# ghnmqdtg/VM-ASR

Measured on AMD Instinct MI355X. Metric: audio clips/sec (train step) 48kHz n_fft=1024, higher is better.
Workload: dtype bf16 (autocast over G; scan/STFT f32; MPD f32/bf16x3 MFMA); 1 GPU; vm_asr_48k_MPD.yaml full train step, DIMS 16 d_state 1 n_fft 1024 clip 122640@48k; per_gpu_batch=4, global_batch=4, parallelism=dp1, execution=hipGraph replay, 2 streams, generator_streams=2

## Files before the change

include/vmasr_hip.h:

```cpp
#ifndef VMASR_HIP_H
#define VMASR_HIP_H

#include <stddef.h>
#include <stdint.h>

#ifdef __cplusplus
extern "C" {
#endif

#define VMASR_ABI_VERSION 1

typedef void *vmasr_stream_t;

enum { VMASR_F32 = 0, VMASR_F16 = 1, VMASR_BF16 = 2 };

enum {
    VMASR_OK = 0,
    VMASR_EINVAL = -1,
    VMASR_EALIGN = -2,
    VMASR_ENOSPACE = -3
};

int vmasr_abi_version(void);
const char *vmasr_last_error(void);
// ... 95 lines not shown
    const float *h_down, *h_up;
    int64_t n_mid, mid_off;
    int32_t up, down, half_len, half_len_up;
} vmasr_degrade_item;
size_t vmasr_degrade_batch_workspace(const vmasr_degrade_item *items, int32_t B);
int vmasr_degrade_batch(const float *x, float *y, const vmasr_degrade_item *items, const vmasr_degrade_item *items_dev, int32_t B,
                        int64_t T, void *ws, size_t ws_bytes, vmasr_stream_t stream);

int vmasr_layer_norm_fwd(const void *x, const float *gamma, const float *beta, void *y, float *mean,
                         float *rstd, int32_t rows, int32_t C, float eps, int32_t dtype, int32_t y_dtype,
                         vmasr_stream_t stream);
size_t vmasr_layer_norm_bwd_workspace(int32_t rows, int32_t C);
int vmasr_layer_norm_bwd(const void *x, const void *gy, const float *gamma, const float *mean,
                         const float *rstd, void *dx, float *dgamma, float *dbeta, float *ws, int32_t rows,
                         int32_t C, int32_t dtype, int32_t gy_dtype, vmasr_stream_t stream);
int vmasr_layer_norm_bwd_res(const void *x, const void *gy, const float *gamma, const float *mean,
                             const float *rstd, const void *residual, void *dx, float *dgamma, float *dbeta, float *ws,
                             int32_t rows, int32_t C, int32_t dtype, int32_t gy_dtype, vmasr_stream_t stream);
int32_t vmasr_layer_norm_bwd_blocks(int32_t rows, int32_t C);
int vmasr_layer_norm_bwd_reduce_multi(const float *const *parts, float *const *dgammas, float *const *dbetas, const int32_t *nblks,
                                      const int32_t *Cs, int32_t n, vmasr_stream_t stream);

int vmasr_small_linear_supported(int32_t in_features, int32_t out_features);
int vmasr_small_linear_fwd(const void *x, const float *w, const float *bias, void *y, int64_t rows,
                           int32_t in_features, int32_t out_features, int32_t x_dtype, int32_t y_dtype,
                           vmasr_stream_t stream);
size_t vmasr_small_linear_bwd_workspace(int64_t rows, int32_t in_features, int32_t out_features);
int vmasr_small_linear_bwd(const void *x, const float *w, const void *gy, void *dx, float *dw, float *db,
                           float *ws, int64_t rows, int32_t in_features, int32_t out_features,
                           int32_t x_dtype, int32_t gy_dtype, vmasr_stream_t stream);

int vmasr_spectral_power_iter(const float *W, float *u, float *v, float *ws, int32_t R, int32_t C,
                              int32_t n_iter, float eps, vmasr_stream_t stream);

typedef struct vmasr_spectral_item {
    const float *W;
    float *u, *v, *t, *s;
    int32_t R, C, row_block_start, col_tile_start;
} vmasr_spectral_item;
int vmasr_spectral_power_iter_batched(const vmasr_spectral_item *items, int32_t n, int32_t total_row_blocks,
                                      int32_t total_col_tiles, int64_t weight_bytes, int32_t n_iter, float eps,
                                      float *sigma, vmasr_stream_t stream);

int vmasr_im2col_kx1(const void *x, void *cols, int64_t N, int32_t H, int32_t C, int32_t k, int32_t stride,
                     int32_t pad, int64_t rows_out, int32_t dtype, vmasr_stream_t stream);
int vmasr_im2col_kx1_split(const float *x, void *hi, void *lo, int64_t N, int32_t H, int32_t C, int32_t k, int32_t stride,
                           int32_t pad, int64_t rows_out, vmasr_stream_t stream);
int vmasr_col2im_kx1(const void *dcols, void *dx, int64_t N, int32_t H, int32_t C, int32_t k, int32_t stride,
                     int32_t pad, int32_t dtype, vmasr_stream_t stream);
int vmasr_im2col_kx1_split_multi(const float *const *xs, const int64_t *Ns, const int32_t *Hs, int32_t n, void *hi, void *lo,
                                 int32_t C, int32_t k, int32_t stride, int32_t pad, int64_t rows_out, vmasr_stream_t stream);
int vmasr_im2col_kx1_split3_multi(const float *const *xs, const int64_t *Ns, const int32_t *Hs, int32_t n, void *cat3, int32_t C,
                                  int32_t k, int32_t stride, int32_t pad, int64_t rows_out, vmasr_stream_t stream);
int vmasr_col2im_kx1_multi(const void *dcols, void *const *dxs, const int64_t *Ns, const int32_t *Hs, int32_t n, int32_t C,
                           int32_t k, int32_t stride, int32_t pad, int64_t rows, int32_t dtype, vmasr_stream_t stream);
int vmasr_col2im_kx1_stacked(const void *dcols, void *dx, const int64_t *Ns, const int32_t *Hs, int32_t n, int32_t C, int32_t k, int32_t stride,
                             int32_t pad, int64_t rows, int64_t dx_rows, int32_t dtype, vmasr_stream_t stream);
int vmasr_stack_rows(const void *const *srcs, const int64_t *Ms, int32_t n, void *full, int64_t rows, int64_t row_bytes,
                     vmasr_stream_t stream);


int vmasr_bias_gelu_fwd(float *acc, const float *bias, float *act, int32_t slots, int64_t M, int32_t N, int32_t parts,
                        vmasr_stream_t stream);
int vmasr_weight_prep_split(const float *w, void *out, int32_t n, int32_t N, int32_t K, vmasr_stream_t stream);
int vmasr_weight_transpose(const float *w, void *hi, void *lo, float *out32, int32_t n, int32_t N, int32_t Cin, int32_t k,
                           vmasr_stream_t stream);
int vmasr_sum_parts(const float *parts, float *out, int32_t P, int32_t n, int32_t S, int64_t NK, vmasr_stream_t stream);
int vmasr_gelu_bwd_split(const float *pre, const float *g, void *hi, void *lo, void *cat3, float *db, int32_t slots, int64_t M,
                         int32_t N, vmasr_stream_t stream);
int vmasr_gelu_bwd(const float *pre, const float *g, float *gx, float *db, int32_t slots, int64_t M, int32_t N, vmasr_stream_t stream);

typedef struct vmasr_cg_slot {
    const void *ah, *al;
    const void *bh, *bl;
    float *c0;
    float *c1;
    void *ch, *cl;
    const float *bias;
    int64_t nseq;
    int32_t H;
    int32_t reserved;
} vmasr_cg_slot;
int vmasr_conv_mfma_supported(int32_t Cin, int32_t Cout, int32_t k, int32_t stride);
int vmasr_conv_mfma_supported_launch(int32_t Cin, int32_t Cout, int32_t k, int32_t stride, int32_t n, int64_t rows);
int vmasr_conv_mfma_config(int32_t pass, int32_t Cin, int32_t Cout, int32_t ops, int32_t out[3]);
void vmasr_conv_set_cu_limit(int32_t cus);
int32_t vmasr_conv_get_cu_limit(void);
int vmasr_conv_mfma_fwd(const vmasr_cg_slot *slots, int32_t n, int32_t Cin, int32_t Cout, int32_t k, int32_t stride, int32_t pad,
                        int64_t rows_out, int32_t act, vmasr_stream_t stream);
int vmasr_conv_mfma_dgrad(const vmasr_cg_slot *slots, int32_t n, int32_t Cin, int32_t Cout, int32_t k, int32_t stride, int32_t pad,
                          int64_t rows_in, vmasr_stream_t stream);
int vmasr_conv_f32_fwd(const vmasr_cg_slot *slots, int32_t n, int32_t Cin, int32_t Cout, int32_t k, int32_t stride, int32_t pad,
                       int64_t rows_out, int32_t act, vmasr_stream_t stream);
int vmasr_conv_f32_dgrad(const vmasr_cg_slot *slots, int32_t n, int32_t Cin, int32_t Cout, int32_t k, int32_t stride, int32_t pad,
                         int64_t rows_in, vmasr_stream_t stream);
int vmasr_conv_mfma_wgrad(const vmasr_cg_slot *slots, int32_t n, int32_t Cin, int32_t Cout, int32_t k, int32_t stride, int32_t pad,
                          int32_t splits, vmasr_stream_t stream);
typedef struct vmasr_cg_gelu_bwd {
    const float *pre;
    const signed char *sgn;
    int64_t valid;
    float scale;
    int32_t reserved;
    float *db;
} vmasr_cg_gelu_bwd;
int vmasr_conv_mfma_dgrad_gelu(const vmasr_cg_slot *slots, const vmasr_cg_gelu_bwd *epi, const float *gtok, int32_t n, int32_t Cin, int32_t Cout,
                               int32_t k, int32_t stride, int32_t pad, int64_t rows_in, vmasr_stream_t stream);

int vmasr_wgrad_finish_multi(const float *const *parts, float *const *dws, float *const *dbs, float *const *e1s, float *const *e2s,
                             const int32_t *Ss, const int32_t *Ns, const int32_t *Ks, const int32_t *lds, int32_t n, vmasr_stream_t stream);

int vmasr_linear_f64acc(const float *x, const float *w, const float *bias, float *y, int64_t rows, int32_t out_features,
                        int32_t in_features, vmasr_stream_t stream);

typedef struct vmasr_adamw_item {
    float *p;
    const float *g;
    float *m;
    float *v;
    void *lp;
    int64_t n;
    float weight_decay;
    int32_t vec;
    void *lpt;
    int32_t rows, cols;
} vmasr_adamw_item;
int32_t vmasr_adamw_chunk(void);
int vmasr_adamw_step(const vmasr_adamw_item *items, const int32_t *chunks, int32_t nchunks, int64_t total_elems, const float *lr,
                     const float *step, float beta1, float beta2, float eps, vmasr_stream_t stream);

int32_t vmasr_sn_dot_blocks(void);
int vmasr_sn_stack_fwd(const void *const *weights, const void *const *sigmas, int32_t n, float *out, void *hi, void *lo, int32_t N, int32_t Cin,
                       int32_t k, vmasr_stream_t stream);
int vmasr_sn_stack_bwd(const float *dW, const float *Wn, void *const *gws, const void *const *sigmas, const void *const *us,
                       const void *const *vs, int32_t n, double *partials, int32_t N, int32_t Cin, int32_t k, vmasr_stream_t stream);

int vmasr_conv_post_supported(int32_t C, int32_t k);
int vmasr_conv_post_fwd(const float *x, const float *w, const float *b, float *y, const int64_t *Ms, const int32_t *Hs, int32_t n, int64_t rows,
                        int32_t C, int32_t k, vmasr_stream_t stream);
int vmasr_conv_post_bwd(const float *x, const float *w, const float *gy, float *dx, float *dw, float *db, const int64_t *Ms, const int32_t *Hs,
                        int32_t n, int64_t rows, int32_t C, int32_t k, vmasr_stream_t stream);
int vmasr_conv_post_bwd_gelu(const float *x, const float *w, const float *gy, const float *pre, const void *sgn, const float *gtok,
                             const int64_t *valid, const float *scale, void *gh, void *gl, float *g32, float *dw, float *db, float *dbcol,
                             const int64_t *Ms, const int32_t *Hs, int32_t n, int64_t rows, int32_t C, int32_t k, vmasr_stream_t stream);

int vmasr_conv_first_fwd(const void *const *xs, const int64_t *Ns, const int32_t *Hs, int32_t n, const float *w, const float *b, float *pre,
                         float *act, int64_t rows, vmasr_stream_t stream);
int vmasr_conv_first_bwd(const void *const *xs, const int64_t *Ns, const int32_t *Hs, int32_t n, const float *w, const float *pre,
                         const float *g, float *dcols, float *dw, float *db, int64_t rows, vmasr_stream_t stream);

int32_t vmasr_masked_l1_blocks(void);
int vmasr_masked_l1_fwd(const float *real, const float *gen, void *sgn, double *partials, const int64_t *valid, const float *scale,
                        int32_t n, int64_t rows_r, int64_t rows_g, int32_t N, vmasr_stream_t stream);
int vmasr_masked_l1_bwd(const void *sgn, const float *gout, float *dgen, const int64_t *valid, const float *scale, int32_t n,
                        int64_t rows_g, int32_t N, vmasr_stream_t stream);
int vmasr_masked_l1_bwd_add(const void *sgn, const float *gout, const float *add, float *dgen, const int64_t *valid, const float *scale,
                            int32_t n, int64_t rows_g, int32_t N, vmasr_stream_t stream);
int vmasr_lsgan_fwd(const void *const *xs, const int64_t *ns, const float *targets, int32_t count, float *out, vmasr_stream_t stream);
int vmasr_lsgan_bwd(const void *const *xs, void *const *ds, const int64_t *ns, const float *targets, int32_t count, const float *gout,
                    vmasr_stream_t stream);

#define VMASR_SS2D_PAIRS 1
typedef struct vmasr_ss2d_params {
    int32_t B, D, H, W, dtype, flags;
    const void *x;
    void *xT;
    const float *Wx, *Wdt, *dtb, *Alog, *Ds;
    float *state, *out02, *out13, *y;
    const float *dy;
    float *dyT, *adj, *part;
    void *dx;
    float *dWx, *dWdt, *ddtb, *dAlog, *dDs;
} vmasr_ss2d_params;
int vmasr_ss2d_supported(int32_t d_state, int32_t dt_rank, int32_t d_inner, int32_t H, int32_t W);
size_t vmasr_ss2d_part_floats(int32_t B, int32_t D, int32_t H, int32_t W);
int vmasr_ss2d_fwd(const vmasr_ss2d_params *p, vmasr_stream_t stream);
int vmasr_ss2d_bwd(const vmasr_ss2d_params *p, vmasr_stream_t stream);

typedef struct vmasr_ss2d_deep_params {
    int32_t B, D, H, W, R, dtype;
    const void *x;
    const float *WxT, *Wdt, *dtb, *Alog, *Ds;
    float *xdbl, *y;
    const float *dy;
    float *du;
    void *tp, *tb, *tc;
    float *pg, *g32;
    void *dx, *gpos;
} vmasr_ss2d_deep_params;
int vmasr_ss2d_deep_supported(int32_t d_state, int32_t dt_rank, int32_t d_inner, int32_t H, int32_t W);
int32_t vmasr_ss2d_deep_waves_per_row(int32_t H, int32_t W);
int vmasr_ss2d_deep_fwd(const vmasr_ss2d_deep_params *p, vmasr_stream_t stream);
int vmasr_ss2d_deep_bwd(const vmasr_ss2d_deep_params *p, vmasr_stream_t stream);

int vmasr_ss2d_glue_supported(int32_t D, int32_t L, int32_t dtype);
int vmasr_ss2d_pre_fwd(const void *xz, void *xT, void *sz, int32_t B, int32_t D, int32_t L, int32_t dtype, vmasr_stream_t stream);
int vmasr_ss2d_pre_bwd(const void *xz, const void *dxT, const void *dsz, void *dxz, int32_t B, int32_t D, int32_t L, int32_t dtype,
                       vmasr_stream_t stream);
int vmasr_ln_gate_fwd(const float *y, const void *sz, const float *gamma, const float *beta, void *out, float *mean, float *rstd,
                      int32_t B, int32_t D, int32_t L, float eps, int32_t dtype, vmasr_stream_t stream);
int vmasr_ln_gate_bwd(const float *y, const void *sz, const void *dout, const float *gamma, const float *beta, const float *mean,
                      const float *rstd, float *dy, void *dsz, float *dgamma, float *dbeta, int32_t B, int32_t D, int32_t L,
                      int32_t dtype, vmasr_stream_t stream);
int64_t vmasr_ln_gate_bwd_workspace(int32_t B, int32_t D, int32_t L, int32_t dtype);
int vmasr_ln_gate_bwd_ws(const float *y, const void *sz, const void *dout, const float *gamma, const float *beta, const float *mean,
                         const float *rstd, float *dy, void *dsz, float *dgamma, float *dbeta, float *ws, int32_t B, int32_t D,
                         int32_t L, int32_t dtype, vmasr_stream_t stream);
int vmasr_ln_gate_pair_supported(int32_t D, int32_t H, int32_t W);
int vmasr_ln_gate_pair_fwd(const float *y02, const float *y13, const void *sz, const float *gamma, const float *beta, void *out,
                           float *mean, float *rstd, int32_t B, int32_t D, int32_t H, int32_t W, float eps, int32_t dtype,
                           vmasr_stream_t stream);
int vmasr_ln_gate_pair_bwd(const float *y02, const float *y13, const void *sz, const void *dout, const float *gamma,
                           const float *beta, const float *mean, const float *rstd, float *dy02, float *dy13, void *dsz,
                           float *dgamma, float *dbeta, int32_t B, int32_t D, int32_t H, int32_t W, int32_t dtype,
                           vmasr_stream_t stream);

int vmasr_split_bf16(const float *x, void *hi, void *lo, int64_t n, vmasr_stream_t stream);

int vmasr_mlp_supported(int32_t d, int32_t hidden);
int vmasr_mlp_fwd(const void *x, const float *gamma, const float *beta, float eps, const void *w1, const float *b1,
                  const void *w2, const float *b2, const float *scale, int32_t rows_per_sample, void *y, int64_t rows,
                  int32_t d, int32_t x_dtype, vmasr_stream_t stream);
int vmasr_mlp_bwd(const void *x, const void *gy, const float *gamma, const float *beta, float eps, const void *w1,
                  const void *w1t, const float *b1, const void *w2t, const float *scale, int32_t rows_per_sample, void *dxn,
                  void *xn_aug, void *gys, void *act_aug, void *gpre, float *mean, float *rstd, int64_t rows, int32_t d,
                  int32_t x_dtype, vmasr_stream_t stream);

int vmasr_inproj_supported(int32_t d, int32_t d_proj, int64_t L);
int vmasr_inproj_fwd(const void *x, const float *gamma, const float *beta, float eps, const void *w, void *xT, void *sz, int64_t rows,
                     int32_t L, int32_t d, int32_t x_dtype, vmasr_stream_t stream);
int vmasr_inproj_bwd(const void *x, const float *gamma, const float *beta, float eps, const void *w, const void *wt, const void *dxT,
                     const void *dsz, void *dxn, void *xn, void *gpre, float *mean, float *rstd, int64_t rows, int32_t L, int32_t d,
                     int32_t x_dtype, vmasr_stream_t stream);

int vmasr_outproj_supported(int32_t d, int32_t d_inner);
int vmasr_outproj_fwd(const void *g, const void *w, const void *x, const float *scale, int32_t rows_per_sample, void *y, int64_t rows,
                      int32_t d, int32_t x_dtype, vmasr_stream_t stream);
int vmasr_outproj_bwd(const void *gy, const void *wt, const float *scale, int32_t rows_per_sample, void *dg, void *gys, int64_t rows,
                      int32_t d, int32_t x_dtype, vmasr_stream_t stream);

int32_t vmasr_stft_loss_blocks(void);
int vmasr_stft_loss_fwd(const float *re_x, const float *im_x, const float *re_y, const float *im_y, int64_t n, double *partials, float *out,
                        vmasr_stream_t stream);
int vmasr_stft_loss_bwd(const float *re_x, const float *im_x, const float *re_y, const float *im_y, int64_t n, const float *fin,
                        const float *g_sc, const float *g_ml, float *d_re, float *d_im, vmasr_stream_t stream);

int vmasr_gconv1d_supported(int32_t Cin, int32_t Cout, int32_t groups, int32_t k, int32_t stride);
int vmasr_gconv1d_supported_launch(int32_t Cin, int32_t Cout, int32_t groups, int32_t k, int32_t stride, int32_t pad, int32_t B, int64_t L);
size_t vmasr_gconv1d_wgrad_workspace(int32_t Cin, int32_t Cout, int32_t groups, int32_t k, int32_t stride, int32_t pad, int32_t B, int64_t L);
int vmasr_gconv1d_fwd(const float *x, const float *w, const float *bias, float *y, float *pre, int32_t B, int32_t Cin, int32_t Cout,
                      int32_t groups, int64_t L, int32_t k, int32_t stride, int32_t pad, int32_t act, vmasr_stream_t stream);
int vmasr_gconv1d_dgrad(const float *gy, const float *pre, const float *w, float *dx, int32_t B, int32_t Cin, int32_t Cout, int32_t groups,
                        int64_t L, int32_t k, int32_t stride, int32_t pad, vmasr_stream_t stream);
int vmasr_gconv1d_wgrad(const float *x, const float *gy, const float *pre, float *dw, float *db, void *ws, size_t ws_bytes, int32_t B,
                        int32_t Cin, int32_t Cout, int32_t groups, int64_t L, int32_t k, int32_t stride, int32_t pad, vmasr_stream_t stream);

int32_t vmasr_stem1d_time_tile(void);
int32_t vmasr_stem1d_channel_group(void);
int vmasr_stem1d_supported(int32_t Cout, int32_t k, int32_t stride, int32_t pad);
int vmasr_stem1d_supported_launch(int32_t Cout, int32_t k, int32_t stride, int32_t pad, int32_t B, int64_t L);
size_t vmasr_stem1d_bwd_workspace(int32_t Cout, int32_t k, int32_t stride, int32_t pad, int32_t B, int64_t L);
int vmasr_stem1d_fwd(const float *x, const float *w, const float *bias, float *y, int32_t B, int32_t Cout, int64_t L, int32_t k, int32_t stride,
                     int32_t pad, int32_t act, vmasr_stream_t stream);
int vmasr_stem1d_bwd(const float *gy, const float *x, const float *w, const float *bias, float *dx, float *dw, float *db, void *ws,
                     size_t ws_bytes, int32_t B, int32_t Cout, int64_t L, int32_t k, int32_t stride, int32_t pad, int32_t act,
                     vmasr_stream_t stream);

int vmasr_stem1d_fm_supported_launch(int32_t Cout, int32_t k, int32_t stride, int32_t pad, int32_t B, int64_t L);
size_t vmasr_stem1d_fm_workspace(int32_t Cout, int32_t k, int32_t stride, int32_t pad, int32_t B, int64_t L);
int vmasr_stem1d_fm_fwd(const float *x, const float *w, const float *bias, const float *y_real, float *y, double *partials, size_t ws_bytes,
                        int32_t B, int32_t Cout, int64_t L, int32_t k, int32_t stride, int32_t pad, vmasr_stream_t stream);
int vmasr_stem1d_fm_bwd(const float *gy, const float *x, const float *w, const float *bias, const float *y_real, const float *gterm, float coef,
                        float *dx, int32_t B, int32_t Cout, int64_t L, int32_t k, int32_t stride, int32_t pad, vmasr_stream_t stream);

enum {
    VMASR_K_SSCAN_FWD = 0,
    VMASR_K_SSCAN_FWD_AGG,
    VMASR_K_SSCAN_FWD_CARRY,
    VMASR_K_SSCAN_FWD_APPLY,
    VMASR_K_SSCAN_BWD,
    VMASR_K_SSCAN_BWD_AGG,
    VMASR_K_SSCAN_BWD_CARRY,
    VMASR_K_SSCAN_BWD_APPLY,
    VMASR_K_CROSS_SCAN,
    VMASR_K_CROSS_MERGE,
    VMASR_K_DWCONV_FWD,
    VMASR_K_DWCONV_BWD_A,
    VMASR_K_DWCONV_BWD_B,
    VMASR_K_STFT,
    VMASR_K_ISTFT_FRAMES,
    VMASR_K_ISTFT_OLA,
    VMASR_K_ISTFT_BWD,
    VMASR_K_LN_FWD,
    VMASR_K_LN_BWD,
    VMASR_K_LN_BWD_REDUCE,
    VMASR_K_SMALL_LINEAR_FWD,
    VMASR_K_SMALL_LINEAR_BWD,
    VMASR_K_SMALL_LINEAR_REDUCE,
    VMASR_K_XPROJ_FWD,
    VMASR_K_XPROJ_BWD_A,
    VMASR_K_XPROJ_BWD_B,
    VMASR_K_SPECTRAL,
    VMASR_K_IM2COL,
    VMASR_K_COL2IM,
    VMASR_K_SPLIT_BF16,
    VMASR_K_BIAS_GELU,
// ... 67 lines not shown
```

vm_asr_amd/_lib.py:

```python
import ctypes
import os

from . import knobs

_HERE = os.path.dirname(os.path.abspath(__file__))
LIB_PATH = knobs.get("VMASR_LIB") or os.path.join(_HERE, "libvmasr_hip.so")

c_i32, c_i64, c_vp, c_sz = ctypes.c_int32, ctypes.c_int64, ctypes.c_void_p, ctypes.c_size_t

F32, F16, BF16 = 0, 1, 2


class SScanParams(ctypes.Structure):
    _fields_ = (
        [(n, c_i32) for n in ("batch", "dim", "seqlen", "dstate", "n_groups", "n_chunks", "dtype",
                              "delta_softplus")]
        + [(n, c_i64) for n in ("A_d_stride", "A_dstate_stride",
                                "B_batch_stride", "B_group_stride", "B_dstate_stride",
                                "C_batch_stride", "C_group_stride", "C_dstate_stride",
                                "u_batch_stride", "u_d_stride", "delta_batch_stride", "delta_d_stride",
                                "out_batch_stride", "out_d_stride")]
        + [(n, c_vp) for n in ("A_ptr", "B_ptr", "C_ptr", "D_ptr", "u_ptr", "delta_ptr",
                               "delta_bias_ptr", "out_ptr", "x_ptr")]
    )


class SScanBwdParams(ctypes.Structure):
    _fields_ = (
        [("f", SScanParams)]
        + [(n, c_i64) for n in ("dout_batch_stride", "dout_d_stride", "du_batch_stride", "du_d_stride",
                                "ddelta_batch_stride", "ddelta_d_stride", "dA_d_stride", "dA_dstate_stride")]
        + [(n, c_vp) for n in ("dout_ptr", "du_ptr", "ddelta_ptr", "dA_ptr", "dB_ptr", "dC_ptr", "dD_ptr",
                               "ddelta_bias_ptr", "ws_ptr")]
        + [("ws_bytes", c_sz)]
    )


class SS2DParams(ctypes.Structure):
    _fields_ = ([(n, c_i32) for n in ("B", "D", "H", "W", "dtype", "flags")]
                + [(n, c_vp) for n in ("x", "xT", "Wx", "Wdt", "dtb", "Alog", "Ds", "state", "out02", "out13", "y",
                                       "dy", "dyT", "adj", "part", "dx", "dWx", "dWdt", "ddtb", "dAlog", "dDs")])


class CgSlot(ctypes.Structure):
    _fields_ = ([(n, c_vp) for n in ("ah", "al", "bh", "bl", "c0", "c1", "ch", "cl", "bias")]
                + [("nseq", c_i64), ("H", c_i32), ("reserved", c_i32)])


class CgGeluBwd(ctypes.Structure):
    _fields_ = [("pre", c_vp), ("sgn", c_vp), ("valid", c_i64), ("scale", ctypes.c_float), ("reserved", c_i32), ("db", c_vp)]


class SS2DDeepParams(ctypes.Structure):
    _fields_ = ([(n, c_i32) for n in ("B", "D", "H", "W", "R", "dtype")]
                + [(n, c_vp) for n in ("x", "WxT", "Wdt", "dtb", "Alog", "Ds", "xdbl", "y", "dy", "du", "tp", "tb", "tc", "pg",
                                       "g32", "dx", "gpos")])


SYMBOLS = {
    "vmasr_abi_version": (ctypes.c_int, []),
    "vmasr_last_error": (ctypes.c_char_p, []),
    "vmasr_sscan_chunk": (ctypes.c_int, []),
    "vmasr_sscan_fwd": (ctypes.c_int, [ctypes.POINTER(SScanParams), c_vp]),
    "vmasr_sscan_bwd_workspace": (c_sz, [ctypes.POINTER(SScanBwdParams)]),
    "vmasr_sscan_bwd": (ctypes.c_int, [ctypes.POINTER(SScanBwdParams), c_vp]),
    "vmasr_sscan_tune": (None, [ctypes.c_int, ctypes.c_int]),
    "vmasr_layer_norm_fwd": (ctypes.c_int, [c_vp, c_vp, c_vp, c_vp, c_vp, c_vp, c_i32, c_i32, ctypes.c_float, c_i32, c_i32, c_vp]),
    "vmasr_layer_norm_bwd_workspace": (c_sz, [c_i32, c_i32]),
    "vmasr_layer_norm_bwd": (ctypes.c_int, [c_vp, c_vp, c_vp, c_vp, c_vp, c_vp, c_vp, c_vp, c_vp, c_i32, c_i32, c_i32, c_i32, c_vp]),
    "vmasr_layer_norm_bwd_res": (ctypes.c_int, [c_vp, c_vp, c_vp, c_vp, c_vp, c_vp, c_vp, c_vp, c_vp, c_vp, c_i32, c_i32, c_i32, c_i32, c_vp]),
    "vmasr_layer_norm_bwd_blocks": (c_i32, [c_i32, c_i32]),
    "vmasr_layer_norm_bwd_reduce_multi": (ctypes.c_int, [c_vp, c_vp, c_vp, c_vp, c_vp, c_i32, c_vp]),
    "vmasr_mlp_supported": (ctypes.c_int, [c_i32, c_i32]),
    "vmasr_mlp_fwd": (ctypes.c_int, [c_vp, c_vp, c_vp, ctypes.c_float, c_vp, c_vp, c_vp, c_vp, c_vp, c_i32, c_vp, c_i64, c_i32, c_i32, c_vp]),
    "vmasr_mlp_bwd": (ctypes.c_int, [c_vp, c_vp, c_vp, c_vp, ctypes.c_float, c_vp, c_vp, c_vp, c_vp, c_vp, c_i32,
                                     c_vp, c_vp, c_vp, c_vp, c_vp, c_vp, c_vp, c_i64, c_i32, c_i32, c_vp]),
    "vmasr_stft_loss_blocks": (c_i32, []),
    "vmasr_stft_loss_fwd": (ctypes.c_int, [c_vp, c_vp, c_vp, c_vp, c_i64, c_vp, c_vp, c_vp]),
    "vmasr_stft_loss_bwd": (ctypes.c_int, [c_vp, c_vp, c_vp, c_vp, c_i64, c_vp, c_vp, c_vp, c_vp, c_vp, c_vp]),
    "vmasr_outproj_supported": (ctypes.c_int, [c_i32, c_i32]),
    "vmasr_outproj_fwd": (ctypes.c_int, [c_vp, c_vp, c_vp, c_vp, c_i32, c_vp, c_i64, c_i32, c_i32, c_vp]),
    "vmasr_outproj_bwd": (ctypes.c_int, [c_vp, c_vp, c_vp, c_i32, c_vp, c_vp, c_i64, c_i32, c_i32, c_vp]),
    "vmasr_inproj_supported": (ctypes.c_int, [c_i32, c_i32, c_i64]),
    "vmasr_inproj_fwd": (ctypes.c_int, [c_vp, c_vp, c_vp, ctypes.c_float, c_vp, c_vp, c_vp, c_i64, c_i32, c_i32, c_i32, c_vp]),
    "vmasr_inproj_bwd": (ctypes.c_int, [c_vp, c_vp, c_vp, ctypes.c_float, c_vp, c_vp, c_vp, c_vp, c_vp, c_vp, c_vp, c_vp, c_vp,
                                        c_i64, c_i32, c_i32, c_i32, c_vp]),
    "vmasr_small_linear_supported": (ctypes.c_int, [c_i32, c_i32]),
    "vmasr_small_linear_fwd": (ctypes.c_int, [c_vp, c_vp, c_vp, c_vp, c_i64, c_i32, c_i32, c_i32, c_i32, c_vp]),
    "vmasr_small_linear_bwd_workspace": (c_sz, [c_i64, c_i32, c_i32]),
    "vmasr_small_linear_bwd": (ctypes.c_int, [c_vp, c_vp, c_vp, c_vp, c_vp, c_vp, c_vp, c_i64, c_i32, c_i32, c_i32, c_i32, c_vp]),
    "vmasr_cross_scan_cvt": (ctypes.c_int, [c_vp, c_vp, c_i32, c_i32, c_i32, c_i32, c_i32, c_i32, c_vp]),
    "vmasr_cross_merge_cvt": (ctypes.c_int, [c_vp, c_vp, c_i32, c_i32, c_i32, c_i32, c_i32, c_i32, c_vp]),
    "vmasr_xproj_supported": (ctypes.c_int, [c_i32, c_i32, c_i32]),
    "vmasr_xproj_fwd": (ctypes.c_int, [c_vp] * 7 + [c_i32] * 7 + [c_vp]),
    "vmasr_xproj_bwd": (ctypes.c_int, [c_vp] * 12 + [c_i32] * 7 + [c_vp]),
    "vmasr_xproj_n_supported": (ctypes.c_int, [c_i32, c_i32, c_i32]),
    "vmasr_xproj_n_ws_floats": (c_sz, [c_i32, c_i32, c_i32, c_i32]),
    "vmasr_xproj_n_fwd": (ctypes.c_int, [c_vp] * 7 + [c_i32] * 7 + [c_vp]),
    "vmasr_xproj_n_bwd": (ctypes.c_int, [c_vp] * 12 + [c_i32] * 7 + [c_vp]),
    "vmasr_spectral_power_iter": (ctypes.c_int, [c_vp, c_vp, c_vp, c_vp, c_i32, c_i32, c_i32, ctypes.c_float, c_vp]),
    "vmasr_spectral_power_iter_batched": (ctypes.c_int, [c_vp, c_i32, c_i32, c_i32, c_i64, c_i32, ctypes.c_float, c_vp, c_vp]),
    "vmasr_im2col_kx1": (ctypes.c_int, [c_vp, c_vp, c_i64, c_i32, c_i32, c_i32, c_i32, c_i32, c_i64, c_i32, c_vp]),
    "vmasr_im2col_kx1_split": (ctypes.c_int, [c_vp, c_vp, c_vp, c_i64, c_i32, c_i32, c_i32, c_i32, c_i32, c_i64, c_vp]),
    "vmasr_im2col_kx1_split3_multi": (ctypes.c_int, [c_vp, c_vp, c_vp, c_i32, c_vp, c_i32, c_i32, c_i32, c_i32, c_i64, c_vp]),
    "vmasr_col2im_kx1": (ctypes.c_int, [c_vp, c_vp, c_i64, c_i32, c_i32, c_i32, c_i32, c_i32, c_i32, c_vp]),
    "vmasr_im2col_kx1_split_multi": (ctypes.c_int, [c_vp, c_vp, c_vp, c_i32, c_vp, c_vp, c_i32, c_i32, c_i32, c_i32, c_i64, c_vp]),
    "vmasr_col2im_kx1_multi": (ctypes.c_int, [c_vp, c_vp, c_vp, c_vp, c_i32, c_i32, c_i32, c_i32, c_i32, c_i64, c_i32, c_vp]),
    "vmasr_col2im_kx1_stacked": (ctypes.c_int, [c_vp, c_vp, c_vp, c_vp, c_i32, c_i32, c_i32, c_i32, c_i32, c_i64, c_i64, c_i32, c_vp]),
    "vmasr_stack_rows": (ctypes.c_int, [c_vp, c_vp, c_i32, c_vp, c_i64, c_i64, c_vp]),
    "vmasr_split_bf16": (ctypes.c_int, [c_vp, c_vp, c_vp, c_i64, c_vp]),
    "vmasr_bias_gelu_fwd": (ctypes.c_int, [c_vp, c_vp, c_vp, c_i32, c_i64, c_i32, c_i32, c_vp]),
    "vmasr_gelu_bwd": (ctypes.c_int, [c_vp, c_vp, c_vp, c_vp, c_i32, c_i64, c_i32, c_vp]),
    "vmasr_sn_dot_blocks": (c_i32, []),
    "vmasr_sn_stack_fwd": (ctypes.c_int, [c_vp, c_vp, c_i32, c_vp, c_vp, c_vp, c_i32, c_i32, c_i32, c_vp]),
    "vmasr_sn_stack_bwd": (ctypes.c_int, [c_vp, c_vp, c_vp, c_vp, c_vp, c_vp, c_i32, c_vp, c_i32, c_i32, c_i32, c_vp]),
    "vmasr_conv_post_supported": (ctypes.c_int, [c_i32, c_i32]),
    "vmasr_conv_post_fwd": (ctypes.c_int, [c_vp, c_vp, c_vp, c_vp, c_vp, c_vp, c_i32, c_i64, c_i32, c_i32, c_vp]),
    "vmasr_conv_post_bwd": (ctypes.c_int, [c_vp, c_vp, c_vp, c_vp, c_vp, c_vp, c_vp, c_vp, c_i32, c_i64, c_i32, c_i32, c_vp]),
    "vmasr_conv_post_bwd_gelu": (ctypes.c_int, [c_vp] * 16 + [c_i32, c_i64, c_i32, c_i32, c_vp]),
    "vmasr_conv_first_fwd": (ctypes.c_int, [c_vp, c_vp, c_vp, c_i32, c_vp, c_vp, c_vp, c_vp, c_i64, c_vp]),
    "vmasr_conv_first_bwd": (ctypes.c_int, [c_vp, c_vp, c_vp, c_i32, c_vp, c_vp, c_vp, c_vp, c_vp, c_vp, c_i64, c_vp]),
    "vmasr_adamw_chunk": (c_i32, []),
    "vmasr_adamw_step": (ctypes.c_int, [c_vp, c_vp, c_i32, c_i64, c_vp, c_vp, ctypes.c_float, ctypes.c_float, ctypes.c_float, c_vp]),
    "vmasr_masked_l1_blocks": (c_i32, []),
    "vmasr_masked_l1_fwd": (ctypes.c_int, [c_vp, c_vp, c_vp, c_vp, c_vp, c_vp, c_i32, c_i64, c_i64, c_i32, c_vp]),
    "vmasr_masked_l1_bwd": (ctypes.c_int, [c_vp, c_vp, c_vp, c_vp, c_vp, c_i32, c_i64, c_i32, c_vp]),
    "vmasr_lsgan_fwd": (ctypes.c_int, [c_vp, c_vp, c_vp, c_i32, c_vp, c_vp]),
    "vmasr_lsgan_bwd": (ctypes.c_int, [c_vp, c_vp, c_vp, c_vp, c_i32, c_vp, c_vp]),
    "vmasr_masked_l1_bwd_add": (ctypes.c_int, [c_vp, c_vp, c_vp, c_vp, c_vp, c_vp, c_i32, c_i64, c_i32, c_vp]),
    "vmasr_sum_parts": (ctypes.c_int, [c_vp, c_vp, c_i32, c_i32, c_i32, c_i64, c_vp]),
    "vmasr_weight_prep_split": (ctypes.c_int, [c_vp, c_vp, c_i32, c_i32, c_i32, c_vp]),
    "vmasr_weight_transpose": (ctypes.c_int, [c_vp, c_vp, c_vp, c_vp, c_i32, c_i32, c_i32, c_i32, c_vp]),
    "vmasr_gelu_bwd_split": (ctypes.c_int, [c_vp, c_vp, c_vp, c_vp, c_vp, c_vp, c_i32, c_i64, c_i32, c_vp]),
    "vmasr_conv_mfma_supported": (ctypes.c_int, [c_i32, c_i32, c_i32, c_i32]),
    "vmasr_conv_mfma_supported_launch": (ctypes.c_int, [c_i32, c_i32, c_i32, c_i32, c_i32, ctypes.c_int64]),
    "vmasr_conv_mfma_config": (ctypes.c_int, [c_i32, c_i32, c_i32, c_i32, ctypes.POINTER(c_i32)]),
    "vmasr_mark_time": (ctypes.c_int, [c_vp, c_vp]),
    "vmasr_im2col2d_rows": (ctypes.c_int, [c_vp, c_vp] + [c_i32] * 10 + [c_vp, c_i32, c_i32, c_vp]),
    "vmasr_col2im2d_rows": (ctypes.c_int, [c_vp, c_vp] + [c_i32] * 10 + [c_vp, c_i32, c_i32, c_vp]),
    "vmasr_skinny_linear_supported": (ctypes.c_int, [c_i64, c_i32, c_i32]),
    "vmasr_skinny_linear": (ctypes.c_int, [c_vp, c_vp, c_vp, c_vp, c_i64, c_i32, c_i32, c_i64, c_i64, c_i32, c_i32, c_vp]),
    "vmasr_conv_set_cu_limit": (None, [c_i32]),
    "vmasr_conv_get_cu_limit": (c_i32, []),
    "vmasr_conv_mfma_fwd": (ctypes.c_int, [ctypes.POINTER(CgSlot), c_i32, c_i32, c_i32, c_i32, c_i32, c_i32, c_i64, c_i32, c_vp]),
    "vmasr_conv_mfma_dgrad": (ctypes.c_int, [ctypes.POINTER(CgSlot), c_i32, c_i32, c_i32, c_i32, c_i32, c_i32, c_i64, c_vp]),
    "vmasr_conv_f32_fwd": (ctypes.c_int, [ctypes.POINTER(CgSlot), c_i32, c_i32, c_i32, c_i32, c_i32, c_i32, c_i64, c_i32, c_vp]),
    "vmasr_conv_f32_dgrad": (ctypes.c_int, [ctypes.POINTER(CgSlot), c_i32, c_i32, c_i32, c_i32, c_i32, c_i32, c_i64, c_vp]),
    "vmasr_conv_mfma_wgrad": (ctypes.c_int, [ctypes.POINTER(CgSlot), c_i32, c_i32, c_i32, c_i32, c_i32, c_i32, c_i32, c_vp]),
    "vmasr_conv_mfma_dgrad_gelu": (ctypes.c_int, [ctypes.POINTER(CgSlot), ctypes.POINTER(CgGeluBwd), c_vp, c_i32, c_i32, c_i32, c_i32, c_i32,
                                                  c_i32, c_i64, c_vp]),
    "vmasr_wgrad_finish_multi": (ctypes.c_int, [c_vp, c_vp, c_vp, c_vp, c_vp, c_vp, c_vp, c_vp, c_vp, c_i32, c_vp]),
    "vmasr_linear_f64acc": (ctypes.c_int, [c_vp, c_vp, c_vp, c_vp, c_i64, c_i32, c_i32, c_vp]),
    "vmasr_ss2d_glue_supported": (ctypes.c_int, [c_i32, c_i32, c_i32]),
    "vmasr_ss2d_pre_fwd": (ctypes.c_int, [c_vp, c_vp, c_vp, c_i32, c_i32, c_i32, c_i32, c_vp]),
    "vmasr_ss2d_pre_bwd": (ctypes.c_int, [c_vp, c_vp, c_vp, c_vp, c_i32, c_i32, c_i32, c_i32, c_vp]),
    "vmasr_ln_gate_fwd": (ctypes.c_int, [c_vp] * 7 + [c_i32, c_i32, c_i32, ctypes.c_float, c_i32, c_vp]),
    "vmasr_ln_gate_bwd": (ctypes.c_int, [c_vp] * 11 + [c_i32, c_i32, c_i32, c_i32, c_vp]),
    "vmasr_ln_gate_bwd_workspace": (c_i64, [c_i32, c_i32, c_i32, c_i32]),
    "vmasr_ln_gate_bwd_ws": (ctypes.c_int, [c_vp] * 12 + [c_i32, c_i32, c_i32, c_i32, c_vp]),
    "vmasr_ln_gate_pair_supported": (ctypes.c_int, [c_i32, c_i32, c_i32]),
    "vmasr_ln_gate_pair_fwd": (ctypes.c_int, [c_vp] * 8 + [c_i32, c_i32, c_i32, c_i32, ctypes.c_float, c_i32, c_vp]),
    "vmasr_ln_gate_pair_bwd": (ctypes.c_int, [c_vp] * 13 + [c_i32, c_i32, c_i32, c_i32, c_i32, c_vp]),
    "vmasr_ss2d_supported": (ctypes.c_int, [c_i32] * 5),
    "vmasr_ss2d_part_floats": (c_sz, [c_i32] * 4),
    "vmasr_ss2d_fwd": (ctypes.c_int, [ctypes.POINTER(SS2DParams), c_vp]),
    "vmasr_ss2d_bwd": (ctypes.c_int, [ctypes.POINTER(SS2DParams), c_vp]),
    "vmasr_ss2d_deep_supported": (ctypes.c_int, [c_i32] * 5),
    "vmasr_ss2d_deep_waves_per_row": (c_i32, [c_i32, c_i32]),
    "vmasr_ss2d_deep_fwd": (ctypes.c_int, [ctypes.POINTER(SS2DDeepParams), c_vp]),
    "vmasr_ss2d_deep_bwd": (ctypes.c_int, [ctypes.POINTER(SS2DDeepParams), c_vp]),
    "vmasr_set_deterministic": (None, [ctypes.c_int]),
    "vmasr_get_deterministic": (ctypes.c_int, []),
    "vmasr_det_timeouts": (ctypes.c_int64, []),
    "vmasr_prof_enable": (None, [ctypes.c_int]),
    "vmasr_prof_reset": (None, []),
    "vmasr_prof_name": (ctypes.c_char_p, [ctypes.c_int]),
    "vmasr_prof_collect": (ctypes.c_int, [ctypes.c_int, ctypes.POINTER(ctypes.c_int64),
                                          ctypes.POINTER(ctypes.c_double), ctypes.POINTER(ctypes.c_double)]),
    "vmasr_prof_collect_shapes": (ctypes.c_int, [ctypes.c_int, ctypes.c_int, ctypes.POINTER(ctypes.c_double), ctypes.POINTER(ctypes.c_int64),
                                                 ctypes.POINTER(ctypes.c_double)]),
    "vmasr_cross_scan": (ctypes.c_int, [c_vp, c_vp, c_i32, c_i32, c_i32, c_i32, c_i32, c_vp]),
    "vmasr_cross_merge": (ctypes.c_int, [c_vp, c_vp, c_i32, c_i32, c_i32, c_i32, c_i32, c_vp]),
    "vmasr_dwconv_silu_fwd": (ctypes.c_int, [c_vp, c_vp, c_vp, c_vp, c_i32, c_i32, c_i32, c_i32, c_i32, c_vp]),
    "vmasr_dwconv_silu_bwd": (ctypes.c_int, [c_vp, c_vp, c_vp, c_vp, c_vp, c_vp, c_vp, c_vp,
                                             c_i32, c_i32, c_i32, c_i32, c_i32, c_vp]),
    "vmasr_stft": (ctypes.c_int, [c_vp, c_vp, c_vp, c_i32, c_i32, c_i32, c_i32, c_i32, c_i32, c_i32, c_vp]),
    "vmasr_stft_bwd_workspace": (c_sz, [c_i32, c_i32, c_i32, c_i32]),
    "vmasr_stft_bwd": (ctypes.c_int, [c_vp, c_vp, c_vp, c_i32, c_i32, c_i32, c_i32, c_i32, c_i32, c_vp, c_sz, c_vp]),
    "vmasr_istft_workspace": (c_sz, [c_i32, c_i32, c_i32, c_i32]),
    "vmasr_istft": (ctypes.c_int, [c_vp, c_vp, c_vp, c_i32, c_i32, c_i32, c_i32, c_i32, c_vp, c_sz, c_vp]),
    "vmasr_istft_bwd": (ctypes.c_int, [c_vp, c_vp, c_vp, c_vp, c_vp, c_i32, c_i32, c_i32, c_i32, c_i32, c_vp]),
    "vmasr_metrics_workspace": (c_sz, [c_i32, c_i32, c_i32, c_i32]),
    "vmasr_metrics": (ctypes.c_int, [c_vp, c_vp, c_vp, c_vp, c_vp, c_i32, c_i32, c_i32, c_i32, c_vp, c_sz, c_vp]),
    "vmasr_gconv1d_supported": (ctypes.c_int, [c_i32] * 5),
    "vmasr_gconv1d_supported_launch": (ctypes.c_int, [c_i32] * 7 + [c_i64]),
    "vmasr_gconv1d_wgrad_workspace": (c_sz, [c_i32] * 7 + [c_i64]),
    "vmasr_gconv1d_fwd": (ctypes.c_int, [c_vp] * 5 + [c_i32] * 4 + [c_i64] + [c_i32] * 4 + [c_vp]),
    "vmasr_gconv1d_dgrad": (ctypes.c_int, [c_vp] * 4 + [c_i32] * 4 + [c_i64] + [c_i32] * 3 + [c_vp]),
    "vmasr_gconv1d_wgrad": (ctypes.c_int, [c_vp] * 6 + [c_sz] + [c_i32] * 4 + [c_i64] + [c_i32] * 3 + [c_vp]),
    "vmasr_stem1d_time_tile": (c_i32, []),
    "vmasr_stem1d_channel_group": (c_i32, []),
    "vmasr_stem1d_supported": (ctypes.c_int, [c_i32] * 4),
    "vmasr_stem1d_supported_launch": (ctypes.c_int, [c_i32] * 5 + [c_i64]),
    "vmasr_stem1d_bwd_workspace": (c_sz, [c_i32] * 5 + [c_i64]),
    "vmasr_stem1d_fwd": (ctypes.c_int, [c_vp] * 4 + [c_i32] * 2 + [c_i64] + [c_i32] * 4 + [c_vp]),
    "vmasr_stem1d_bwd": (ctypes.c_int, [c_vp] * 8 + [c_sz] + [c_i32] * 2 + [c_i64] + [c_i32] * 4 + [c_vp]),
    "vmasr_stem1d_fm_supported_launch": (ctypes.c_int, [c_i32] * 5 + [c_i64]),
    "vmasr_stem1d_fm_workspace": (c_sz, [c_i32] * 5 + [c_i64]),
    "vmasr_stem1d_fm_fwd": (ctypes.c_int, [c_vp] * 6 + [c_sz] + [c_i32] * 2 + [c_i64] + [c_i32] * 3 + [c_vp]),
    "vmasr_stem1d_fm_bwd": (ctypes.c_int, [c_vp] * 6 + [ctypes.c_float] + [c_vp] + [c_i32] * 2 + [c_i64] + [c_i32] * 3 + [c_vp]),
    "vmasr_resample_poly": (ctypes.c_int, [c_vp, c_vp, c_vp, c_i32, c_i64, c_i64, c_i32, c_i32, c_i32, c_vp]),
    "vmasr_resample_design_workspace": (c_sz, [c_i32]),
    "vmasr_resample_design": (ctypes.c_int, [c_vp, c_i32, c_i32, c_i32, c_vp, c_sz, c_vp]),
    "vmasr_degrade_batch_workspace": (c_sz, [c_vp, c_i32]),
    "vmasr_degrade_batch": (ctypes.c_int, [c_vp, c_vp, c_vp, c_vp, c_i32, c_i64, c_vp, c_sz, c_vp]),
}

_lib = None


def lib():
    global _lib
    if _lib is None:
        if not os.path.exists(LIB_PATH):
            raise RuntimeError(
                f"{LIB_PATH} is missing: build it with `make -C vm_asr_amd/csrc` "
                "(or __graft_entry__.build()). vm_asr_amd has no CPU fallback.")
        import torch
        l = ctypes.CDLL(LIB_PATH)
        for name, (res, args) in SYMBOLS.items():
            fn = getattr(l, name)
            fn.restype, fn.argtypes = res, args
        if l.vmasr_abi_version() != 1:
            raise RuntimeError("libvmasr_hip.so ABI version mismatch")
        if knobs.get("VMASR_DETERMINISTIC"):
            l.vmasr_set_deterministic(1)
        knobs.warn_undeclared()
        _lib = l
    return _lib


def check(code, what):
    if code != 0:
        msg = lib().vmasr_last_error().decode() or "unknown error"
        raise RuntimeError(f"{what} failed ({code}): {msg}")


def torch_dtype_code(dt):
    import torch
    try:
        return {torch.float32: F32, torch.float16: F16, torch.bfloat16: BF16}[dt]
    except KeyError:
        raise RuntimeError(f"unsupported dtype {dt}: expected float32 / float16 / bfloat16")


def det_mode():
    if knobs.get("VMASR_DETERMINISTIC"):
        return True
    try:
        return bool(lib().vmasr_get_deterministic())
    except (OSError, RuntimeError, AttributeError):
        return False


def current_stream(device):
    import torch
    return ctypes.c_void_p(torch.cuda.current_stream(device).cuda_stream)


def ptr(t):
    return None if t is None else ctypes.c_void_p(t.data_ptr())


def call(fn, *args, device=None):
    import torch
    what = fn.__name__[len("vmasr_"):]
    conv = list(args)
    for i, a in enumerate(conv):
# ... 85 lines not shown
```

vm_asr_amd/convgemm.py:

```python
import ctypes

import torch

from . import _lib
from .mpd_ops import need as _need, sum_parts


def supported(Cin, Cout, k, stride):
    return bool(_lib.lib().vmasr_conv_mfma_supported(int(Cin), int(Cout), int(k), int(stride)))


def config(what, Cin, Cout, f32=False):
    out = (ctypes.c_int32 * 3)()
    _lib.check(_lib.lib().vmasr_conv_mfma_config(("fwd", "dgrad", "wgrad").index(what), int(Cin), int(Cout), int(bool(f32)), out), "conv_mfma_config")
    return tuple(out)


_LIMIT = {"cus": 0, "min_channels": 0}


class cu_limit:

    def __init__(self, cus, min_channels=0):
        self.new = {"cus": int(cus or 0), "min_channels": int(min_channels or 0)}

    def __enter__(self):
        self.prev = dict(_LIMIT)
        _LIMIT.update(self.new)
        return self

    def __exit__(self, *exc):
        _LIMIT.update(self.prev)
        _lib.lib().vmasr_conv_set_cu_limit(0)
        return False


def _apply_limit(Cin, Cout):
    lim = _LIMIT["cus"] if max(Cin, Cout) >= _LIMIT["min_channels"] else 0
    _lib.lib().vmasr_conv_set_cu_limit(lim)


def _slots(geom, **operands):
    sl = (_lib.CgSlot * len(geom))()
    steps = [(f, t.data_ptr(), t.stride(0) * t.element_size()) for f, t in operands.items() if t is not None]
    for i, (nseq, H) in enumerate(geom):
        for f, base, step in steps:
            setattr(sl[i], f, base + i * step)
        sl[i].nseq, sl[i].H = int(nseq), int(H)
    return sl


def _ptr(t, i, step):
    return ctypes.c_void_p(t.data_ptr() + i * step) if t is not None else None


def out_positions(H, k, stride, pad):
    return (H + 2 * pad - k) // stride + 1


def _fwd(fn, xh, xl, wh, wl, bias, geom, k, stride, pad, rows_out, act, want_pair):
    _need(xh, xl, wh, wl, bias)
    (n, _, Cin), Cout, dev = xh.shape, wh.shape[1], xh.device
    pre = torch.empty((n, rows_out, Cout), dtype=torch.float32, device=dev)
    y = torch.empty_like(pre) if act else None
    yh = torch.empty((n, rows_out, Cout), dtype=torch.bfloat16, device=dev) if act and want_pair else None
    yl = torch.empty_like(yh) if yh is not None else None
    sl = _slots(geom, ah=xh, al=xl, bh=wh, bl=wl, c0=pre, c1=y, ch=yh, cl=yl, bias=bias)
    _apply_limit(Cin, Cout)
    _lib.call(fn, sl, n, Cin, Cout, k, stride, pad, rows_out, int(bool(act)), device=dev)
    return pre, y, yh, yl


def _dgrad(fn, gh, gl, wth, wtl, geom, k, stride, pad, rows_in):
    _need(gh, gl, wth, wtl)
    (n, _, Cout), Cin, dev = gh.shape, wth.shape[1], gh.device
    dx = torch.empty((n, rows_in, Cin), dtype=torch.float32, device=dev)
    sl = _slots(geom, ah=gh, al=gl, bh=wth, bl=wtl, c0=dx)
    _apply_limit(Cin, Cout)
    _lib.call(fn, sl, n, Cin, Cout, k, stride, pad, rows_in, device=dev)
    return dx


def conv_fwd(xh, xl, wh, wl, bias, geom, k, stride, pad, rows_out, act=True, want_pair=True):
    return _fwd(_lib.lib().vmasr_conv_mfma_fwd, xh, xl, wh, wl, bias, geom, k, stride, pad, rows_out, act, want_pair)


def conv_dgrad(gh, gl, wth, wtl, geom, k, stride, pad, rows_in):
    return _dgrad(_lib.lib().vmasr_conv_mfma_dgrad, gh, gl, wth, wtl, geom, k, stride, pad, rows_in)


def conv_fwd_f32(x, w, bias, geom, k, stride, pad, rows_out, act=True, want_pair=True):
    assert x.dtype == torch.float32 and w.dtype == torch.float32
    return _fwd(_lib.lib().vmasr_conv_f32_fwd, x, None, w, None, bias, geom, k, stride, pad, rows_out, act, want_pair)


def conv_dgrad_f32(g, wt, geom, k, stride, pad, rows_in):
    assert g.dtype == torch.float32 and wt.dtype == torch.float32
    return _dgrad(_lib.lib().vmasr_conv_f32_dgrad, g, None, wt, None, geom, k, stride, pad, rows_in)


def conv_dgrad_gelu(gh, gl, wth, wtl, geom, k, stride, pad, rows_in, pre, want_f32=False, want_pair=True, sgn=None, gtok=None,
                    scale=None, valid=None, db=None):
    _need(gh, gl, wth, wtl, pre, sgn, gtok, db)
    assert db is None or (db.shape == (gh.shape[0], wth.shape[1]) and db.dtype == torch.float32)
    (n, _, Cout), Cin, dev = gh.shape, wth.shape[1], gh.device
    assert pre.shape == (n, rows_in, Cin) and pre.dtype == torch.float32 and (want_f32 or want_pair)
    assert sgn is None or (sgn.shape == pre.shape and sgn.dtype == torch.int8 and gtok is not None and gtok.dtype == torch.float32)
    g32 = torch.empty((n, rows_in, Cin), dtype=torch.float32, device=dev) if want_f32 else None
    oh = torch.empty((n, rows_in, Cin), dtype=torch.bfloat16, device=dev) if want_pair else None
    ol = torch.empty_like(oh) if want_pair else None
    sl = _slots(geom, ah=gh, al=gl, bh=wth, bl=wtl, c0=g32, ch=oh, cl=ol)
    ep = (_lib.CgGeluBwd * n)()
    for i in range(n):
        ep[i].pre = _ptr(pre, i, rows_in * Cin * 4)
        ep[i].sgn = _ptr(sgn, i, rows_in * Cin)
        ep[i].valid = int(valid[i]) if (sgn is not None and valid is not None) else 0
        ep[i].scale = float(scale[i]) if (sgn is not None and scale is not None) else 0.0
        ep[i].db = _ptr(db, i, Cin * 4)
    _apply_limit(Cin, Cout)
    _lib.call(_lib.lib().vmasr_conv_mfma_dgrad_gelu, sl, ep, gtok if sgn is not None else None, n, Cin, Cout, k, stride, pad, rows_in,
              device=dev)
    return g32, ((oh, ol) if want_pair else None)


def wgrad_splits(n, Cin, Cout, k, M):
    if Cin % 256 == 0 and Cout % 256 == 0:
        return 1
    T = 128
    tiles = n * (Cout // T) * (k * Cin // T)
    s = 1
    while tiles * s < 768 and s < 16 and M // (2 * s) >= 1024:
        s *= 2
    return s


def conv_wgrad(gh, gl, xh, xl, geom, k, stride, pad, splits=None):
    _need(gh, gl, xh, xl)
    (n, _, Cout), Cin, dev = gh.shape, xh.shape[2], gh.device
    if splits is None:
        M = max(nseq * out_positions(H, k, stride, pad) for nseq, H in geom)
        splits = wgrad_splits(n, Cin, Cout, k, M)
    parts = torch.empty((n, splits, Cout, k * Cin), dtype=torch.float32, device=dev)
    sl = _slots(geom, ah=gh, al=gl, bh=xh, bl=xl, c0=parts)
    _apply_limit(Cin, Cout)
    _lib.call(_lib.lib().vmasr_conv_mfma_wgrad, sl, n, Cin, Cout, k, stride, pad, splits, device=dev)
    if splits == 1:
        return parts.view(n, Cout, k * Cin)
    return sum_parts(parts, 1, n, splits, (Cout, k * Cin))
```

vm_asr_amd/csrc/convgemm.hip:

```cpp
#include <algorithm>
#include <cstdlib>
#include <type_traits>

#include "common.h"

namespace vmasr {
namespace {

typedef __bf16 bf16x8 __attribute__((ext_vector_type(8)));
typedef float f32x16 __attribute__((ext_vector_type(16)));
typedef float f32x4 __attribute__((ext_vector_type(4)));
typedef unsigned u32x4 __attribute__((ext_vector_type(4)));
typedef __attribute__((address_space(1))) const void *cg_gptr;
typedef __attribute__((address_space(3))) void *cg_lptr;
__device__ uint4 cg_zero_page[4];

constexpr int CG_BM = 128, CG_BN = 128, CG_BK = 32;
constexpr int CG_TILE = CG_BM * CG_BK * 2;
constexpr int CG_STAGE = 4 * CG_TILE;
constexpr int CG_MAXP = 24;

struct CgProb {
    const bf16_t *ah, *al, *bh, *bl;
    float *c0, *c1;
    bf16_t *ch, *cl;
    const float *bias;
    int M, Q;
    int HA;
    int HC;
    int hq_mul, hq_add;
    int crow_mul, crow_add;
    int ntaps, tap0, tap_step, dstep;
    int tile_start, mtiles;
    int zero_rows;
    float fscale;
    int fvalid;
    float *db;
};

struct CgParams {
    CgProb prob[CG_MAXP];
    int nprob, ntiles_n, total_tiles;
    int CA;
    int NB;
    int KB;
    const float *gtok;
};
static_assert(sizeof(CgParams) <= 4096, "CgParams is passed by value as the kernel's argument block");

__device__ __forceinline__ int cg_swz(const int row) { return (0 - (row >> 2)) & 3; }
__device__ __forceinline__ int cg_off(const int row, const int chunk) { return row * 64 + ((chunk ^ cg_swz(row)) << 4); }

__device__ __forceinline__ float cg_gelu(float x) { return 0.5f * x * (1.f + erff(x * 0.70710678118654752f)); }
__device__ __forceinline__ float cg_gelu_grad(float x) {
    return 0.5f * (1.f + erff(x * 0.70710678118654752f)) + x * 0.3989422804014327f * __expf(-0.5f * x * x);
}

__device__ __forceinline__ f32x16 cg_mfma(const bf16x8 a, const bf16x8 b, const f32x16 c) {
    return __builtin_amdgcn_mfma_f32_32x32x16_bf16(a, b, c, 0, 0, 0);
}

template <int BM, int BN, int WM, int WN, int EPI, int MF, int OPS = 0>
__global__ __launch_bounds__(64 * WM * WN, 2) void conv_mfma_nt_kernel(const CgParams P) {
    static_assert(OPS == 0 || MF == 32, "the f32 form uses the 32-row fragment layout");
    constexpr bool ACT = EPI == 1;
    constexpr int NT = 64 * WM * WN;
    constexpr int WTM = BM / WM, WTN = BN / WN;
    constexpr int TI = WTM / MF, TJ = WTN / MF;
    constexpr int TILE_A = BM * 64, TILE_B = BN * 64;
    constexpr int STAGE = 2 * TILE_A + 2 * TILE_B;
    constexpr int RPP = NT / 4;
    constexpr int PA = BM / RPP, PB = (BN + RPP - 1) / RPP;
    constexpr bool B_PART = BN < RPP;
    static_assert(BM % RPP == 0 && (BN % RPP == 0 || (B_PART && BN % 16 == 0)) && BM % 128 == 0, "tile / thread geometry");
    extern __shared__ __attribute__((aligned(16))) unsigned char smem[];
    int *crow_tab = reinterpret_cast<int *>(smem + 2 * STAGE);

    const int tid = threadIdx.x, lane = tid & 63, wave = tid >> 6;
    const int wm = wave / WN, wn = wave % WN, lr = lane & 31, lh = lane >> 5;

#pragma unroll 1
    for (int tile = blockIdx.x; tile < P.total_tiles; tile += gridDim.x) {
    const int t = xcd_remap(tile, P.total_tiles);
    int pi = 0;
#pragma unroll 1
    for (int i = 1; i < P.nprob; ++i) pi = (t >= P.prob[i].tile_start) ? i : pi;
    const CgProb &pr = P.prob[pi];
    const int local = t - pr.tile_start;
    const int nt = local % P.ntiles_n, mt = local / P.ntiles_n;
    const int m0 = mt * BM, n0 = nt * BN;
    const int M = pr.M, Q = pr.Q, HA = pr.HA, CA = P.CA, NB = P.NB;
    constexpr int UPK = OPS ? 64 : 32;
    const int LDA = OPS ? 2 * CA : CA;
    const int KB = OPS ? 2 * P.KB : P.KB;

    if (tid < BM) {
        const int m = m0 + tid;
        int cr = -1;
        if (m < M) {
            const int seq = m / Q, q = m - seq * Q;
            cr = seq * pr.HC + q * pr.crow_mul + pr.crow_add;
        } else if (m < pr.zero_rows) {
            cr = m;
        }
        crow_tab[tid] = cr;
    }

    const int srow = tid >> 2, chunk = (tid & 3) ^ cg_swz(srow);
    int a_base[PA], a_hq[PA];
    bool a_ok[PA];
#pragma unroll
    for (int i = 0; i < PA; ++i) {
        const int m = m0 + srow + RPP * i;
        a_ok[i] = m < M;
        const int mm = a_ok[i] ? m : 0;
        const int seq = mm / Q, q = mm - seq * Q;
        a_base[i] = seq * HA;
        a_hq[i] = q * pr.hq_mul + pr.hq_add;
    }
    const bf16_t *bsrc_h[PB], *bsrc_l[PB];
#pragma unroll
    for (int i = 0; i < PB; ++i) {
        const size_t o = (size_t)(n0 + ((B_PART && srow >= BN) ? 0 : srow + RPP * i)) * KB + chunk * 8;
        bsrc_h[i] = pr.bh + o;
        bsrc_l[i] = pr.bl + o;
    }
    const int cpk = CA / CG_BK;
    const int nk = (m0 < M) ? pr.ntaps * cpk : 0;
    const int wbase = wave * 16 * 64;
    const bf16_t *zp = reinterpret_cast<const bf16_t *>(cg_zero_page);

#define CG_DMA(src, dst) __builtin_amdgcn_global_load_lds((cg_gptr)(src), (cg_lptr)(dst), 16, 0, 0)
    auto stage_tile = [&](const int kt, const int buf) {
        const int j = kt / cpk, c0 = (kt - j * cpk) * UPK;
        const int koff = (pr.tap0 + j * pr.tap_step) * LDA + c0;
        unsigned char *d = smem + buf * STAGE + wbase;
#pragma unroll
        for (int i = 0; i < PA; ++i) {
            const int pos = a_hq[i] + j * pr.dstep;
            const bool ok = a_ok[i] && pos >= 0 && pos < HA;
            const size_t o = (size_t)(a_base[i] + pos) * LDA + c0 + chunk * 8;
            CG_DMA(ok ? pr.ah + o : zp, d + i * RPP * 64);
            CG_DMA(ok ? (OPS ? pr.ah + o + 32 : pr.al + o) : zp, d + TILE_A + i * RPP * 64);
        }
#pragma unroll
        for (int i = 0; i < PB; ++i) {
            if (B_PART && srow >= BN) break;
            CG_DMA(bsrc_h[i] + koff, d + 2 * TILE_A + i * RPP * 64);
            CG_DMA((OPS ? bsrc_h[i] + 32 : bsrc_l[i]) + koff, d + 2 * TILE_A + TILE_B + i * RPP * 64);
        }
    };

    using acc_t = typename std::conditional<MF == 32, f32x16, f32x4>::type;
    constexpr int NR = MF == 32 ? 16 : 4;
    acc_t acc[TI][TJ];
#pragma unroll
    for (int i = 0; i < TI; ++i)
#pragma unroll
        for (int j = 0; j < TJ; ++j)
#pragma unroll
            for (int r = 0; r < NR; ++r) acc[i][j][r] = 0.f;

    if (nk > 0) stage_tile(0, 0);
    asm volatile("s_waitcnt vmcnt(0)" ::: "memory");
    __syncthreads();

    for (int kt = 0; kt < nk; ++kt) {
        const int buf = kt & 1;
        if (kt + 1 < nk) stage_tile(kt + 1, buf ^ 1);
        const unsigned char *s = smem + buf * STAGE;
        if constexpr (OPS == 1) {
#pragma unroll
            for (int ks = 0; ks < 2; ++ks) {
                f32x4 a0[TI], a1[TI], b0[TJ], b1[TJ];
#pragma unroll
                for (int i = 0; i < TI; ++i) {
                    const int oa = cg_off(wm * WTM + i * 32 + lr, ks * 2 + lh);
                    a0[i] = *reinterpret_cast<const f32x4 *>(s + oa);
                    a1[i] = *reinterpret_cast<const f32x4 *>(s + TILE_A + oa);
                }
#pragma unroll
                for (int j = 0; j < TJ; ++j) {
                    const int ob = cg_off(wn * WTN + j * 32 + lr, ks * 2 + lh);
                    b0[j] = *reinterpret_cast<const f32x4 *>(s + 2 * TILE_A + ob);
                    b1[j] = *reinterpret_cast<const f32x4 *>(s + 2 * TILE_A + TILE_B + ob);
                }
#pragma unroll
                for (int i = 0; i < TI; ++i)
#pragma unroll
                    for (int j = 0; j < TJ; ++j) {
#pragma unroll
                        for (int e = 0; e < 4; ++e) acc[i][j] = __builtin_amdgcn_mfma_f32_32x32x2f32(a0[i][e], b0[j][e], acc[i][j], 0, 0, 0);
#pragma unroll
                        for (int e = 0; e < 4; ++e) acc[i][j] = __builtin_amdgcn_mfma_f32_32x32x2f32(a1[i][e], b1[j][e], acc[i][j], 0, 0, 0);
                    }
            }
        } else if constexpr (MF == 32) {
#pragma unroll
            for (int ks = 0; ks < 2; ++ks) {
                bf16x8 ah[TI], al[TI], bh[TJ], bl[TJ];
#pragma unroll
                for (int i = 0; i < TI; ++i) {
                    const int oa = cg_off(wm * WTM + i * 32 + lr, ks * 2 + lh);
                    ah[i] = *reinterpret_cast<const bf16x8 *>(s + oa);
                    al[i] = *reinterpret_cast<const bf16x8 *>(s + TILE_A + oa);
                }
// ... 358 lines not shown
int cg_grid(int tiles, size_t smem) {
    if (g_cg_cu_limit <= 0) return tiles;
    const int per_cu = std::max(1, (int)((160 * 1024) / std::max<size_t>(smem, 1)));
    static const int slack = [] { const char *e = getenv("VMASR_CONV_CU_SLACK"); return e ? atoi(e) : 24; }();
    const int cap = std::min(256, g_cg_cu_limit + slack) * per_cu;
    const int rounds = (tiles + cap - 1) / cap;
    const int g = ((tiles + rounds - 1) / rounds + 7) / 8 * 8;
    return std::min(tiles, std::min(g, cap));
}

template <int BM, int BN, int WM, int WN, int MF, int OPS = 0>
int cg_launch_cfg(CgParams &P, int epi, hipStream_t st, int kid, double bytes) {
    int tiles = 0;
    P.ntiles_n = P.NB / BN;
    for (int i = 0; i < P.nprob; ++i) {
        P.prob[i].tile_start = tiles;
        P.prob[i].mtiles = (std::max(P.prob[i].M, P.prob[i].zero_rows) + BM - 1) / BM;
        tiles += P.prob[i].mtiles * P.ntiles_n;
    }
    P.total_tiles = tiles;
    if (tiles == 0) return 0;
    constexpr size_t smem = 2 * (2 * BM * 64 + 2 * BN * 64) + BM * sizeof(int);
    constexpr bool HAS_EPI2 = BN >= 128 && OPS == 0;
    static bool attr_done = false;
    if (!attr_done && smem > 65536) {
        (void)hipFuncSetAttribute(reinterpret_cast<const void *>(&conv_mfma_nt_kernel<BM, BN, WM, WN, 1, MF, OPS>), hipFuncAttributeMaxDynamicSharedMemorySize, (int)smem);
        (void)hipFuncSetAttribute(reinterpret_cast<const void *>(&conv_mfma_nt_kernel<BM, BN, WM, WN, 0, MF, OPS>), hipFuncAttributeMaxDynamicSharedMemorySize, (int)smem);
        if constexpr (HAS_EPI2)
            (void)hipFuncSetAttribute(reinterpret_cast<const void *>(&conv_mfma_nt_kernel<BM, BN, WM, WN, 2, MF, OPS>), hipFuncAttributeMaxDynamicSharedMemorySize, (int)smem);
        attr_done = true;
    }
    if (epi == 1) {
        VMASR_LAUNCH(kid, bytes, (conv_mfma_nt_kernel<BM, BN, WM, WN, 1, MF, OPS>), dim3(cg_grid(tiles, smem)), dim3(64 * WM * WN), smem, st, P);
    } else if (epi == 2) {
        if constexpr (HAS_EPI2) {
            VMASR_LAUNCH(kid, bytes, (conv_mfma_nt_kernel<BM, BN, WM, WN, 2, MF, OPS>), dim3(cg_grid(tiles, smem)), dim3(64 * WM * WN), smem, st, P);
        } else {
            set_error("conv_mfma: no fused activation backward for this tile");
            return VMASR_EINVAL;
        }
    } else {
        VMASR_LAUNCH(kid, bytes, (conv_mfma_nt_kernel<BM, BN, WM, WN, 0, MF, OPS>), dim3(cg_grid(tiles, smem)), dim3(64 * WM * WN), smem, st, P);
    }
    return check_launch("conv_mfma");
}

int env_conv_tile() {
    static const int v = [] { const char *e = getenv("VMASR_CONV_TILE"); return e ? atoi(e) : 0; }();
    return v;
}
int env_conv_mfma() {
    static const int v = [] { const char *e = getenv("VMASR_CONV_MFMA"); return e ? atoi(e) : 16; }();
    return v;
}

struct CgConfig {
    int BM, BN, MF;
};
enum { CG_PASS_FWD = 0, CG_PASS_DGRAD = 1, CG_PASS_WGRAD = 2 };

CgConfig cg_config_nt(int NB, int CA, int ops, bool fwd) {
    if (ops) {
        static const int tile = [] { const char *e = getenv("VMASR_CONV_F32_TILE"); return e ? atoi(e) : 128; }();
        if (!fwd) return {256, 32, 32};
        return tile == 256 ? CgConfig{256, 128, 32} : CgConfig{128, 128, 32};
    }
    const int forced = env_conv_tile();
    const int mf = env_conv_mfma() == 16 ? 16 : 32;
    if (NB % 256 == 0 && forced != 128) return {256, 256, mf};
    if (NB % 128 == 0 && CA == 32 && forced != 128) return {256, 128, 16};
    if (NB == 32) return {256, 32, 16};
    return {128, 128, mf};
}

CgConfig cg_config_wgrad(int Cin, int Cout) {
    if (Cout % 256 == 0 && Cin % 256 == 0 && env_conv_tile() != 128) return {256, 256, 16};
    if (Cin == 32) return {128, 32, 16};
    return {128, 128, env_conv_mfma() == 32 ? 32 : 16};
}

CgConfig cg_config(int pass, int Cin, int Cout, int ops) {
    if (pass == CG_PASS_WGRAD) return cg_config_wgrad(Cin, Cout);
    return pass == CG_PASS_FWD ? cg_config_nt(Cout, Cin, ops, true) : cg_config_nt(Cin, Cout, ops, false);
}

int cg_launch(CgParams &P, int epi, hipStream_t st, int kid, double bytes, int ops = 0, bool fwd = true) {
    const CgConfig c = cg_config_nt(P.NB, P.CA, ops, fwd);
    const int key = c.BM * 1000000 + c.BN * 1000 + c.MF;
    if (ops) {
        switch (key) {
            case 256128032: return cg_launch_cfg<256, 128, 4, 2, 32, 1>(P, epi, st, kid, bytes);
            case 256032032: return cg_launch_cfg<256, 32, 8, 1, 32, 1>(P, epi, st, kid, bytes);
            default: return cg_launch_cfg<128, 128, 2, 2, 32, 1>(P, epi, st, kid, bytes);
        }
    }
    switch (key) {
        case 256256016: return cg_launch_cfg<256, 256, 2, 4, 16>(P, epi, st, kid, bytes);
        case 256256032: return cg_launch_cfg<256, 256, 2, 4, 32>(P, epi, st, kid, bytes);
        case 256128016: return cg_launch_cfg<256, 128, 4, 2, 16>(P, epi, st, kid, bytes);
        case 256032016: return cg_launch_cfg<256, 32, 8, 1, 16>(P, epi, st, kid, bytes);
        case 128128032: return cg_launch_cfg<128, 128, 2, 2, 32>(P, epi, st, kid, bytes);
        default: return cg_launch_cfg<128, 128, 2, 2, 16>(P, epi, st, kid, bytes);
    }
}

int64_t cg_fwd_row_bound(int Cin, int Cout, int k, int ops) { return ((int64_t)1 << (ops ? 30 : 31)) / std::max(Cout, k * Cin); }
int64_t cg_dgrad_row_bound(int Cin, int Cout, int k) { return ((int64_t)1 << 31) / std::max(Cin, k * Cout); }
int64_t cg_wgrad_grow_bound(int Cin, int Cout) { return ((int64_t)1 << 31) / std::max(Cout, Cin); }
int64_t cg_wgrad_xrow_bound(int Cin) { return ((int64_t)1 << 31) / Cin; }

}

VMASR_EXPORT void vmasr_conv_set_cu_limit(int32_t cus) { g_cg_cu_limit = cus < 0 ? 0 : cus; }
VMASR_EXPORT int32_t vmasr_conv_get_cu_limit(void) { return g_cg_cu_limit; }

VMASR_EXPORT int vmasr_conv_mfma_supported(int32_t Cin, int32_t Cout, int32_t k, int32_t stride) {
    const bool in_ok = Cin > 0 && (Cin % 128 == 0 || Cin == 32), out_ok = Cout > 0 && Cout % 128 == 0;
    return in_ok && out_ok && k >= 1 && k <= 8 && stride >= 1 && stride <= 3;
}

VMASR_EXPORT int vmasr_conv_mfma_supported_launch(int32_t Cin, int32_t Cout, int32_t k, int32_t stride, int32_t n, int64_t rows) {
    if (!vmasr_conv_mfma_supported(Cin, Cout, k, stride)) return 0;
    if (n < 1 || n > 8 || n * (stride + 1) > CG_MAXP) return 0;
    int64_t bound = std::min(cg_fwd_row_bound(Cin, Cout, k, 0), cg_dgrad_row_bound(Cin, Cout, k));
    bound = std::min(bound, std::min(cg_wgrad_grow_bound(Cin, Cout), cg_wgrad_xrow_bound(Cin)));
    if (Cin == 32) bound = std::min(bound, cg_fwd_row_bound(Cin, Cout, k, 1));
    return rows >= 1 && rows < bound ? 1 : 0;
}

VMASR_EXPORT int vmasr_conv_mfma_config(int32_t pass, int32_t Cin, int32_t Cout, int32_t ops, int32_t out[3]) {
    VMASR_REQUIRE(out && pass >= CG_PASS_FWD && pass <= CG_PASS_WGRAD && (ops == 0 || (ops == 1 && Cin == 32 && pass != CG_PASS_WGRAD)), VMASR_EINVAL,
                  "conv_mfma_config: pass 0..2, ops 0 or 1 (Cin 32, forward / input gradient), out");
    VMASR_REQUIRE(vmasr_conv_mfma_supported(Cin, Cout, 1, 1), VMASR_EINVAL, "conv_mfma_config: unsupported channel counts (Cin %d, Cout %d)", Cin, Cout);
    const CgConfig c = cg_config(pass, Cin, Cout, ops);
    out[0] = c.BM; out[1] = c.BN; out[2] = c.MF;
    return VMASR_OK;
}

namespace {
int cg_fwd(const vmasr_cg_slot *slots, int32_t n, int32_t Cin, int32_t Cout, int32_t k, int32_t stride, int32_t pad, int64_t rows_out,
           int32_t act, vmasr_stream_t stream, int ops) {
    const char *what = ops ? "conv_f32_fwd" : "conv_mfma_fwd";
    VMASR_REQUIRE(slots && n >= 1 && n <= CG_MAXP, VMASR_EINVAL, "%s: 1..%d slots", what, CG_MAXP);
    VMASR_REQUIRE(vmasr_conv_mfma_supported(Cin, Cout, k, stride) && (!ops || Cin == 32), VMASR_EINVAL,
                  "%s: unsupported shape (Cin %d, Cout %d, k %d, stride %d)", what, Cin, Cout, k, stride);
    VMASR_REQUIRE(rows_out % 256 == 0, VMASR_EINVAL, "%s: rows_out must be a multiple of 256", what);
    CgParams P = {};
    P.nprob = n;
    P.CA = Cin; P.NB = Cout; P.KB = k * Cin;
    double bytes = 0;
    for (int i = 0; i < n; ++i) {
        const vmasr_cg_slot &s = slots[i];
        VMASR_REQUIRE(s.ah && s.bh && s.c0 && (ops || (s.al && s.bl)), VMASR_EINVAL, "%s: null tensor in slot %d", what, i);
        VMASR_REQUIRE(!ops || (aligned_to(s.ah, 16) && aligned_to(s.bh, 16)), VMASR_EALIGN, "%s: slot %d: operands must be 16-byte aligned", what, i);
        const int64_t H1 = ((int64_t)s.H + 2 * pad - k) / stride + 1;
        const int64_t M = s.nseq * H1;
        VMASR_REQUIRE(H1 >= 1 && M <= rows_out && rows_out < cg_fwd_row_bound(Cin, Cout, k, ops), VMASR_EINVAL,
                      "%s: slot %d: %lld rows do not fit rows_out %lld (or 32-bit offsets)", what, i, (long long)M, (long long)rows_out);
        CgProb &p = P.prob[i];
        p.ah = (const bf16_t *)s.ah; p.al = (const bf16_t *)s.al; p.bh = (const bf16_t *)s.bh; p.bl = (const bf16_t *)s.bl;
        p.c0 = s.c0; p.c1 = s.c1; p.ch = (bf16_t *)s.ch; p.cl = (bf16_t *)s.cl; p.bias = s.bias;
        p.M = (int)M; p.Q = (int)H1; p.HA = s.H; p.HC = (int)H1;
        p.hq_mul = stride; p.hq_add = -pad; p.crow_mul = 1; p.crow_add = 0;
        p.ntaps = k; p.tap0 = 0; p.tap_step = 1; p.dstep = 1;
        p.zero_rows = (int)rows_out;
        bytes += (double)s.nseq * s.H * Cin * 4 + (double)Cout * k * Cin * 4 + (double)M * Cout * (act ? 12 : 4);
    }
    hipStream_t st = static_cast<hipStream_t>(stream);
    if (ops) VMASR_REQUIRE(Cout % 128 == 0, VMASR_EINVAL, "%s: Cout %% 128", what);
    return cg_launch(P, act != 0 ? 1 : 0, st, VMASR_K_CONV_MFMA_FWD, bytes, ops, true);
}
}

VMASR_EXPORT int vmasr_conv_mfma_fwd(const vmasr_cg_slot *slots, int32_t n, int32_t Cin, int32_t Cout, int32_t k, int32_t stride,
                                     int32_t pad, int64_t rows_out, int32_t act, vmasr_stream_t stream) {
    return cg_fwd(slots, n, Cin, Cout, k, stride, pad, rows_out, act, stream, 0);
}

VMASR_EXPORT int vmasr_conv_f32_fwd(const vmasr_cg_slot *slots, int32_t n, int32_t Cin, int32_t Cout, int32_t k, int32_t stride,
                                    int32_t pad, int64_t rows_out, int32_t act, vmasr_stream_t stream) {
    return cg_fwd(slots, n, Cin, Cout, k, stride, pad, rows_out, act, stream, 1);
}

namespace {

int cg_dgrad(const vmasr_cg_slot *slots, const vmasr_cg_gelu_bwd *epi, const float *gtok, int32_t n, int32_t Cin, int32_t Cout, int32_t k,
             int32_t stride, int32_t pad, int64_t rows_in, vmasr_stream_t stream, int ops = 0) {
    const char *what = ops ? "conv_f32_dgrad" : epi ? "conv_mfma_dgrad_gelu" : "conv_mfma_dgrad";
    VMASR_REQUIRE(!ops || (!epi && Cin == 32), VMASR_EINVAL, "%s: the f32 form serves Cin = 32 without a fused activation backward", what);
    VMASR_REQUIRE(slots && n >= 1 && n * (stride + 1) <= CG_MAXP, VMASR_EINVAL, "%s: too many slots", what);
    VMASR_REQUIRE(vmasr_conv_mfma_supported(Cin, Cout, k, stride), VMASR_EINVAL, "%s: unsupported shape (Cin %d, Cout %d, k %d, stride %d)", what,
                  Cin, Cout, k, stride);
    VMASR_REQUIRE(!epi || Cin % 128 == 0, VMASR_EINVAL, "%s: the fused activation backward needs Cin %% 128 == 0", what);
    CgParams P = {};
    P.CA = Cout; P.NB = Cin; P.KB = k * Cout;
    P.gtok = gtok;
    double bytes = 0;
    int np = 0;
    for (int i = 0; i < n; ++i) {
        const vmasr_cg_slot &s = slots[i];
        VMASR_REQUIRE(s.ah && s.bh && (ops || (s.al && s.bl)) && (epi ? (s.c0 || (s.ch && s.cl)) && (!s.ch == !s.cl) : s.c0 != nullptr), VMASR_EINVAL,
                      "%s: null tensor in slot %d", what, i);
        VMASR_REQUIRE(!ops || (aligned_to(s.ah, 16) && aligned_to(s.bh, 16)), VMASR_EALIGN, "%s: slot %d: operands must be 16-byte aligned", what, i);
        VMASR_REQUIRE(!epi || (epi[i].pre && epi[i].valid >= 0 && (!epi[i].sgn || gtok)), VMASR_EINVAL,
                      "%s: slot %d: pre-activation missing (or a sign map without the loss gradient)", what, i);
        const int64_t H = s.H, H1 = (H + 2 * pad - k) / stride + 1;
        VMASR_REQUIRE(H1 >= 1 && s.nseq * H <= rows_in && rows_in < cg_dgrad_row_bound(Cin, Cout, k), VMASR_EINVAL,
                      "%s: slot %d: %lld rows do not fit rows_in %lld (or 32-bit offsets)", what, i, (long long)(s.nseq * H), (long long)rows_in);
        auto outputs = [&](CgProb &p) {
            p.c0 = s.c0; p.c1 = nullptr; p.ch = nullptr; p.cl = nullptr; p.bias = nullptr;
            if (epi) {
                p.ch = (bf16_t *)s.ch; p.cl = (bf16_t *)s.cl;
                p.bias = epi[i].pre;
                p.c1 = reinterpret_cast<float *>(const_cast<signed char *>(epi[i].sgn));
                p.fscale = epi[i].scale;
                p.fvalid = (int)std::min<int64_t>(epi[i].valid, rows_in);
                p.db = epi[i].db;
            }
        };
        for (int r = 0; r < stride; ++r) {
            const int r0 = ((r - pad) % stride + stride) % stride;
            const int64_t Q = H > r0 ? (H - r0 + stride - 1) / stride : 0;
            if (Q == 0) continue;
            CgProb &p = P.prob[np++];
            p.ah = (const bf16_t *)s.ah; p.al = (const bf16_t *)s.al; p.bh = (const bf16_t *)s.bh; p.bl = (const bf16_t *)s.bl;
            outputs(p);
            p.M = (int)(s.nseq * Q); p.Q = (int)Q; p.HA = (int)H1; p.HC = (int)H;
            p.hq_mul = 1; p.hq_add = (r0 + pad - r) / stride;
            p.crow_mul = stride; p.crow_add = r0;
            p.ntaps = r < k ? (k - r + stride - 1) / stride : 0;
            p.tap0 = r; p.tap_step = stride; p.dstep = -1;
            p.zero_rows = 0;
        }
        if (s.nseq * H < rows_in) {
            CgProb &p = P.prob[np++];
            p.ah = (const bf16_t *)s.ah; p.al = (const bf16_t *)s.al; p.bh = (const bf16_t *)s.bh; p.bl = (const bf16_t *)s.bl;
            outputs(p);
            p.M = (int)(rows_in - s.nseq * H); p.Q = p.M; p.HA = 1; p.HC = 0;
            p.hq_mul = 0; p.hq_add = 0; p.crow_mul = 1; p.crow_add = (int)(s.nseq * H);
            p.ntaps = 0; p.tap0 = 0; p.tap_step = 1; p.dstep = 0;
            p.zero_rows = 0;
            p.db = nullptr;
        }
        bytes += (double)s.nseq * H1 * Cout * 4 + (double)Cout * k * Cin * 4 + (double)s.nseq * H * Cin * 4;
        if (epi) bytes += (double)s.nseq * H * Cin * ((s.c0 && s.ch ? 4.0 : 0.0) + 4.0 + (epi[i].sgn ? 1.0 : 0.0));
    }
    P.nprob = np;
    return cg_launch(P, epi ? 2 : 0, static_cast<hipStream_t>(stream), VMASR_K_CONV_MFMA_DGRAD, bytes, ops, false);
}

}

VMASR_EXPORT int vmasr_conv_mfma_dgrad(const vmasr_cg_slot *slots, int32_t n, int32_t Cin, int32_t Cout, int32_t k, int32_t stride,
                                       int32_t pad, int64_t rows_in, vmasr_stream_t stream) {
    return cg_dgrad(slots, nullptr, nullptr, n, Cin, Cout, k, stride, pad, rows_in, stream);
}

VMASR_EXPORT int vmasr_conv_f32_dgrad(const vmasr_cg_slot *slots, int32_t n, int32_t Cin, int32_t Cout, int32_t k, int32_t stride,
                                      int32_t pad, int64_t rows_in, vmasr_stream_t stream) {
    return cg_dgrad(slots, nullptr, nullptr, n, Cin, Cout, k, stride, pad, rows_in, stream, 1);
}

VMASR_EXPORT int vmasr_conv_mfma_dgrad_gelu(const vmasr_cg_slot *slots, const vmasr_cg_gelu_bwd *epi, const float *gtok, int32_t n, int32_t Cin,
                                            int32_t Cout, int32_t k, int32_t stride, int32_t pad, int64_t rows_in, vmasr_stream_t stream) {
    VMASR_REQUIRE(epi, VMASR_EINVAL, "conv_mfma_dgrad_gelu: epi is required");
    return cg_dgrad(slots, epi, gtok, n, Cin, Cout, k, stride, pad, rows_in, stream);
}

VMASR_EXPORT int vmasr_conv_mfma_wgrad(const vmasr_cg_slot *slots, int32_t n, int32_t Cin, int32_t Cout, int32_t k, int32_t stride,
                                       int32_t pad, int32_t splits, vmasr_stream_t stream) {
    VMASR_REQUIRE(slots && n >= 1 && n <= 8, VMASR_EINVAL, "conv_mfma_wgrad: 1..8 slots");
    VMASR_REQUIRE(vmasr_conv_mfma_supported(Cin, Cout, k, stride) && splits >= 1 && splits <= 64, VMASR_EINVAL,
                  "conv_mfma_wgrad: unsupported shape (Cin %d, Cout %d, k %d, stride %d, splits %d)", Cin, Cout, k, stride, splits);
    CwParams P = {};
    const CgConfig cfg = cg_config_wgrad(Cin, Cout);
    const bool big = cfg.BM == 256, narrow = cfg.BN == 32;
    const int T = cfg.BM, TK = cfg.BN;
    P.nslots = n; P.splits = splits; P.tiles_co = Cout / T; P.tiles_kc = k * Cin / TK;
    P.Cin = Cin; P.Cout = Cout; P.k = k; P.stride = stride; P.pad = pad;
    double bytes = 0;
    for (int i = 0; i < n; ++i) {
        const vmasr_cg_slot &s = slots[i];
        VMASR_REQUIRE(s.ah && s.al && s.bh && s.bl && s.c0, VMASR_EINVAL, "conv_mfma_wgrad: null tensor in slot %d", i);
        const int64_t H1 = ((int64_t)s.H + 2 * pad - k) / stride + 1, M = s.nseq * H1;
        VMASR_REQUIRE(H1 >= 1 && M < cg_wgrad_grow_bound(Cin, Cout) && s.nseq * (int64_t)s.H < cg_wgrad_xrow_bound(Cin), VMASR_EINVAL,
                      "conv_mfma_wgrad: slot %d too large for 32-bit row offsets", i);
        CwProb &p = P.prob[i];
        p.gh = (const bf16_t *)s.ah; p.gl = (const bf16_t *)s.al; p.xh = (const bf16_t *)s.bh; p.xl = (const bf16_t *)s.bl;
        p.dw = s.c0; p.M = (int)M; p.Q = (int)H1; p.H = s.H;
        const int64_t per = (M + splits - 1) / splits;
        p.mchunk = (int)((per + CW_BR - 1) / CW_BR * CW_BR);
        bytes += (double)M * Cout * 4 + (double)s.nseq * s.H * Cin * 4 + (double)splits * Cout * k * Cin * 4;
    }
    const int tiles = n * splits * P.tiles_co * P.tiles_kc;
    hipStream_t st = static_cast<hipStream_t>(stream);
    if (big) {
        constexpr size_t smem = 2 * 4 * CW_BR * 512;
        static bool attr_done = false;
        if (!attr_done) {
            (void)hipFuncSetAttribute(reinterpret_cast<const void *>(&conv_mfma_wgrad_kernel<256, 256, 2, 4, 16>), hipFuncAttributeMaxDynamicSharedMemorySize, (int)smem);
            attr_done = true;
        }
        VMASR_LAUNCH(VMASR_K_CONV_MFMA_WGRAD, bytes, (conv_mfma_wgrad_kernel<256, 256, 2, 4, 16>), dim3(cg_grid(tiles, smem)), dim3(512), smem, st, P);
    } else if (narrow) {
        VMASR_LAUNCH(VMASR_K_CONV_MFMA_WGRAD, bytes, (conv_mfma_wgrad_kernel<128, 32, 4, 1, 16>), dim3(cg_grid(tiles, 2 * (2 * CW_BR * 256 + 2 * CW_BR * 64))), dim3(256), 2 * (2 * CW_BR * 256 + 2 * CW_BR * 64), st, P);
    } else if (cfg.MF == 32) {
        VMASR_LAUNCH(VMASR_K_CONV_MFMA_WGRAD, bytes, (conv_mfma_wgrad_kernel<128, 128, 2, 2, 32>), dim3(cg_grid(tiles, 2 * 4 * CW_BR * 256)), dim3(256), 2 * 4 * CW_BR * 256, st, P);
    } else {
        VMASR_LAUNCH(VMASR_K_CONV_MFMA_WGRAD, bytes, (conv_mfma_wgrad_kernel<128, 128, 2, 2, 16>), dim3(cg_grid(tiles, 2 * 4 * CW_BR * 256)), dim3(256), 2 * 4 * CW_BR * 256, st, P);
    }
    return check_launch("conv_mfma_wgrad");
}
```

vm_asr_amd/csrc/featloss.hip:

```cpp
#include <algorithm>

#include "common.h"

namespace vmasr {
namespace {

constexpr int kMaxSlots = 8;

struct L1Slots {
    long valid_elems[kMaxSlots];
    float scale[kMaxSlots];
};

__device__ __forceinline__ signed char sgn1(float d) { return (signed char)((d > 0.f) - (d < 0.f)); }

__global__ __launch_bounds__(256) void masked_l1_fwd_kernel(const float *__restrict__ real, const float *__restrict__ gen,
                                                            signed char *__restrict__ sgn, double *__restrict__ partials,
                                                            const L1Slots t, const size_t stride_r, const size_t stride_g) {
    const int s = blockIdx.y;
    const float *__restrict__ r = real + (size_t)s * stride_r;
    const float *__restrict__ g = gen + (size_t)s * stride_g;
    signed char *__restrict__ o = sgn ? sgn + (size_t)s * stride_g : nullptr;
    const long n = t.valid_elems[s], n4 = n / 4;
    double acc = 0.0;
    for (long i = (long)blockIdx.x * blockDim.x + threadIdx.x; i < n4; i += (long)gridDim.x * blockDim.x) {
        const float4 a = reinterpret_cast<const float4 *>(g)[i], b = reinterpret_cast<const float4 *>(r)[i];
        const float d0 = a.x - b.x, d1 = a.y - b.y, d2 = a.z - b.z, d3 = a.w - b.w;
        acc += (double)((fabsf(d0) + fabsf(d1)) + (fabsf(d2) + fabsf(d3)));
        if (o) {
            char4 q;
            q.x = sgn1(d0); q.y = sgn1(d1); q.z = sgn1(d2); q.w = sgn1(d3);
            reinterpret_cast<char4 *>(o)[i] = q;
        }
    }
    if (blockIdx.x == 0 && (int)threadIdx.x < (int)(n - n4 * 4)) {
        const long i = n4 * 4 + threadIdx.x;
        const float d = g[i] - r[i];
        acc += (double)fabsf(d);
        if (o) o[i] = sgn1(d);
    }
    for (int off = 32; off > 0; off >>= 1) acc += __shfl_down(acc, off, 64);
    __shared__ double wsum[4];
    if ((threadIdx.x & 63) == 0) wsum[threadIdx.x >> 6] = acc;
    __syncthreads();
    if (threadIdx.x == 0) partials[(size_t)s * gridDim.x + blockIdx.x] = (wsum[0] + wsum[1] + wsum[2] + wsum[3]) * (double)t.scale[s];
}

__global__ __launch_bounds__(256) void masked_l1_bwd_kernel(const signed char *__restrict__ sgn, const float *__restrict__ gout,
                                                            const float *__restrict__ add, float *__restrict__ dgen, const L1Slots t,
                                                            const size_t stride_g) {
    const int s = blockIdx.y;
    const signed char *__restrict__ q = sgn + (size_t)s * stride_g;
    const float *__restrict__ a = add ? add + (size_t)s * stride_g : nullptr;
    float *__restrict__ o = dgen + (size_t)s * stride_g;
    const float k = gout[0] * t.scale[s];
    const long n = t.valid_elems[s], total4 = (long)(stride_g / 4);
    for (long i = (long)blockIdx.x * blockDim.x + threadIdx.x; i < total4; i += (long)gridDim.x * blockDim.x) {
        float4 v = a ? reinterpret_cast<const float4 *>(a)[i] : make_float4(0.f, 0.f, 0.f, 0.f);
        const long e = i * 4;
        if (e + 3 < n) {
            const char4 c = reinterpret_cast<const char4 *>(q)[i];
            v.x = fmaf(k, (float)c.x, v.x); v.y = fmaf(k, (float)c.y, v.y); v.z = fmaf(k, (float)c.z, v.z); v.w = fmaf(k, (float)c.w, v.w);
        } else if (e < n) {
            float w[4] = {v.x, v.y, v.z, v.w};
            for (int j = 0; j < 4 && e + j < n; ++j) w[j] = fmaf(k, (float)q[e + j], w[j]);
            v = make_float4(w[0], w[1], w[2], w[3]);
        }
        reinterpret_cast<float4 *>(o)[i] = v;
    }
}

int fill_slots(L1Slots &t, const int64_t *valid, const float *scale, int n, int N, int64_t rows_g, int64_t rows_r, const char *what) {
    for (int s = 0; s < n; ++s) {
        if (valid[s] < 0 || valid[s] > rows_g || valid[s] > rows_r) {
            set_error("%s: slot %d has %ld valid rows of %ld / %ld", what, s, (long)valid[s], (long)rows_g, (long)rows_r);
            return VMASR_EINVAL;
        }
        t.valid_elems[s] = (long)valid[s] * N;
        t.scale[s] = scale[s];
    }
    return 0;
}

}
}

using namespace vmasr;

VMASR_EXPORT int32_t vmasr_masked_l1_blocks(void) { return 256 * 4; }

VMASR_EXPORT int vmasr_masked_l1_fwd(const float *real, const float *gen, void *sgn, double *partials, const int64_t *valid,
                                     const float *scale, int32_t n, int64_t rows_r, int64_t rows_g, int32_t N, vmasr_stream_t stream) {
    VMASR_REQUIRE(real && gen && partials && valid && scale, VMASR_EINVAL, "masked_l1_fwd: null argument");
    VMASR_REQUIRE(n > 0 && n <= kMaxSlots && rows_r > 0 && rows_g > 0 && N > 0, VMASR_EINVAL, "masked_l1_fwd: bad shape");
    VMASR_REQUIRE(((size_t)rows_r * N) % 4 == 0 && ((size_t)rows_g * N) % 4 == 0 && aligned_to(real, 16) && aligned_to(gen, 16) &&
                      (!sgn || aligned_to(sgn, 4)),
                  VMASR_EINVAL, "masked_l1_fwd: slots must be 16-byte aligned (rows * N %% 4 == 0)");
    L1Slots t{};
    if (int e = fill_slots(t, valid, scale, n, N, rows_g, rows_r, "masked_l1_fwd")) return e;
    double bytes = 0;
    for (int s = 0; s < n; ++s) bytes += (double)t.valid_elems[s] * (sgn ? 9.0 : 8.0);
    hipStream_t st = static_cast<hipStream_t>(stream);
    VMASR_LAUNCH(VMASR_K_FEAT_L1, bytes, masked_l1_fwd_kernel, dim3(vmasr_masked_l1_blocks(), n), dim3(256), 0, st, real, gen,
                 static_cast<signed char *>(sgn), partials, t, (size_t)rows_r * N, (size_t)rows_g * N);
    return check_launch("masked_l1_fwd");
}

VMASR_EXPORT int vmasr_masked_l1_bwd_add(const void *sgn, const float *gout, const float *add, float *dgen, const int64_t *valid,
                                         const float *scale, int32_t n, int64_t rows_g, int32_t N, vmasr_stream_t stream) {
    VMASR_REQUIRE(sgn && gout && dgen && valid && scale, VMASR_EINVAL, "masked_l1_bwd: null argument");
    VMASR_REQUIRE(n > 0 && n <= kMaxSlots && rows_g > 0 && N > 0, VMASR_EINVAL, "masked_l1_bwd: bad shape");
    VMASR_REQUIRE(((size_t)rows_g * N) % 4 == 0 && aligned_to(dgen, 16) && aligned_to(sgn, 4) && (!add || aligned_to(add, 16)), VMASR_EINVAL,
                  "masked_l1_bwd: slots must be 16-byte aligned (rows * N %% 4 == 0)");
    L1Slots t{};
    if (int e = fill_slots(t, valid, scale, n, N, rows_g, rows_g, "masked_l1_bwd")) return e;
    const long total4 = (long)rows_g * N / 4;
    const int blocks = (int)std::min<long>((total4 + 255) / 256, 256L * 8);
    hipStream_t st = static_cast<hipStream_t>(stream);
    VMASR_LAUNCH(VMASR_K_FEAT_L1, (add ? 9.0 : 5.0) * n * (double)rows_g * N, masked_l1_bwd_kernel, dim3(blocks, n), dim3(256), 0, st,
                 static_cast<const signed char *>(sgn), gout, add, dgen, t, (size_t)rows_g * N);
    return check_launch("masked_l1_bwd");
}

VMASR_EXPORT int vmasr_masked_l1_bwd(const void *sgn, const float *gout, float *dgen, const int64_t *valid, const float *scale, int32_t n,
                                     int64_t rows_g, int32_t N, vmasr_stream_t stream) {
    return vmasr_masked_l1_bwd_add(sgn, gout, nullptr, dgen, valid, scale, n, rows_g, N, stream);
}

namespace vmasr {
namespace {

constexpr int kGanMax = 16;
struct GanItems {
    const float *x[kGanMax];
    float *d[kGanMax];
    long n[kGanMax];
    float c[kGanMax];
    int count;
};

__global__ __launch_bounds__(1024) void lsgan_fwd_kernel(const GanItems t, float *__restrict__ out) {
    __shared__ double ws[16];
    double total = 0.0;
    for (int it = 0; it < t.count; ++it) {
        const float *__restrict__ x = t.x[it];
        const float c = t.c[it];
        double acc = 0.0;
        for (long i = threadIdx.x; i < t.n[it]; i += blockDim.x) {
            const float d = x[i] - c;
            acc += (double)(d * d);
        }
        for (int off = 32; off > 0; off >>= 1) acc += __shfl_down(acc, off, 64);
        if ((threadIdx.x & 63) == 0) ws[threadIdx.x >> 6] = acc;
        __syncthreads();
        if (threadIdx.x == 0) {
            double s = 0.0;
            for (int w = 0; w < 16; ++w) s += ws[w];
            total += s / (double)t.n[it];
        }
        __syncthreads();
    }
    if (threadIdx.x == 0) out[0] = (float)total;
}

__global__ __launch_bounds__(256) void lsgan_bwd_kernel(const GanItems t, const float *__restrict__ gout) {
    const int it = blockIdx.y;
    const float *__restrict__ x = t.x[it];
    float *__restrict__ d = t.d[it];
    const float c = t.c[it], k = 2.f * gout[0] / (float)t.n[it];
    for (long i = (long)blockIdx.x * blockDim.x + threadIdx.x; i < t.n[it]; i += (long)gridDim.x * blockDim.x) d[i] = k * (x[i] - c);
}

int gan_fill(GanItems &t, const void *const *xs, void *const *ds, const int64_t *ns, const float *cs, int count, const char *what) {
    VMASR_REQUIRE(xs && ns && cs && count > 0 && count <= kGanMax, VMASR_EINVAL, "%s: 1..%d tensors", what, kGanMax);
    t.count = count;
    for (int i = 0; i < count; ++i) {
        VMASR_REQUIRE(xs[i] && ns[i] > 0 && (!ds || ds[i]), VMASR_EINVAL, "%s: tensor %d null / empty", what, i);
        t.x[i] = static_cast<const float *>(xs[i]);
        t.d[i] = ds ? static_cast<float *>(ds[i]) : nullptr;
        t.n[i] = ns[i];
        t.c[i] = cs[i];
    }
    return 0;
}

}
}

VMASR_EXPORT int vmasr_lsgan_fwd(const void *const *xs, const int64_t *ns, const float *targets, int32_t count, float *out,
                                 vmasr_stream_t stream) {
    VMASR_REQUIRE(out, VMASR_EINVAL, "lsgan_fwd: null output");
    GanItems t{};
    if (int e = gan_fill(t, xs, nullptr, ns, targets, count, "lsgan_fwd")) return e;
    double bytes = 0;
    for (int i = 0; i < count; ++i) bytes += 4.0 * ns[i];
    VMASR_LAUNCH(VMASR_K_FEAT_L1, bytes, lsgan_fwd_kernel, dim3(1), dim3(1024), 0, static_cast<hipStream_t>(stream), t, out);
    return check_launch("lsgan_fwd");
}

VMASR_EXPORT int vmasr_lsgan_bwd(const void *const *xs, void *const *ds, const int64_t *ns, const float *targets, int32_t count,
                                 const float *gout, vmasr_stream_t stream) {
    VMASR_REQUIRE(gout && ds, VMASR_EINVAL, "lsgan_bwd: null argument");
    GanItems t{};
    if (int e = gan_fill(t, xs, ds, ns, targets, count, "lsgan_bwd")) return e;
    long nmax = 0;
    double bytes = 0;
    for (int i = 0; i < count; ++i) { nmax = std::max<long>(nmax, ns[i]); bytes += 8.0 * ns[i]; }
    const int blocks = (int)std::min<long>((nmax + 255) / 256, 64);
    VMASR_LAUNCH(VMASR_K_FEAT_L1, bytes, lsgan_bwd_kernel, dim3(blocks, count), dim3(256), 0, static_cast<hipStream_t>(stream), t, gout);
    return check_launch("lsgan_bwd");
}
```

vm_asr_amd/discriminator.py:

```python

import torch
import torch.nn as nn
import torch.nn.functional as F
from torch.nn.utils import parametrize
from torch.nn.utils.parametrizations import weight_norm

from . import _lib, knobs, mpd_ops as bind
from .linear import linear as _linear, weight_grad as _weight_grad
from .mpd_featloss import StackedFeatures, _FeatTapFn, _MaskedL1Fn, _masked_l1_ok, feature_loss_stacked
from .mpd_layers import (_BatchedLinearFn, _BatchedLinearSplitFn, _StackedConvFirstFn, _StackedConvMfmaFn, _StackedConvPostFn,
                         _StackedConvSplitFn, _StackedIm2ColFn, _UnstackRowsFn, _bmm3, _dw3, _l1_mode, _poison, _round_up, _split_k,
                         _split_mode, scores_only, skip_weight_grads)
from .mpd_link import _Link, _Tap
from .mpd_ops import SpectralBatch, _slot_arrays, geom_of as _geom, split_bf16

__all__ = ["PeriodDiscriminator", "MultiPeriodDiscriminator", "spectral_norm", "plain_torch_ops"]

_PLAIN_OPS = [False]


class plain_torch_ops:

    def __enter__(self):
        self._saved = _PLAIN_OPS[0]
        _PLAIN_OPS[0] = True
        return self

    def __exit__(self, *exc):
        _PLAIN_OPS[0] = self._saved
        return False


class _SpectralNorm(nn.Module):

    def __init__(self, weight, n_power_iterations=1, eps=1e-12):
        super().__init__()
        self.n_power_iterations, self.eps = n_power_iterations, eps
        w = weight.detach().flatten(1)
        u = F.normalize(w.new_empty(w.size(0)).normal_(0, 1), dim=0, eps=eps)
        v = F.normalize(w.new_empty(w.size(1)).normal_(0, 1), dim=0, eps=eps)
        self.register_buffer("_u", u)
        self.register_buffer("_v", v)
        self._power_method(w, 15)

    @torch.autograd.no_grad()
    def _power_method(self, w, n):
        if w.is_cuda and n > 0 and w.dtype == torch.float32:
            bind.spectral_power_iter(w.contiguous(), self._u, self._v, n, self.eps)
            return
        for _ in range(n):
            self._u = F.normalize((w @ self._v.unsqueeze(1)).squeeze(1), dim=0, eps=self.eps, out=self._u)
            self._v = F.normalize((w.t() @ self._u.unsqueeze(1)).squeeze(1), dim=0, eps=self.eps, out=self._v)

    def forward(self, weight):
        with torch.autocast(device_type=weight.device.type, enabled=False):
            pre = getattr(self, "_sigma_pre", None)
            if pre is not None and self.training and self.n_power_iterations == 0 and weight.dtype == torch.float32:
                return _SNDivFn.apply(weight, self._u, self._v, pre)
            w = (weight if weight.dtype == torch.float64 else weight.float()).flatten(1)
            if self.training:
                self._power_method(w, self.n_power_iterations)
            u, v = self._u.clone(), self._v.clone()
            sigma = (u * (w @ v.unsqueeze(1)).squeeze(1)).sum()
            return weight / sigma


class _SNDivFn(torch.autograd.Function):

    @staticmethod
    def forward(ctx, weight, u, v, sigma):
        out = weight / sigma
        ctx.save_for_backward(out, u, v, sigma)
        return out

    @staticmethod
    def backward(ctx, g):
        out, u, v, sigma = ctx.saved_tensors
        g2, o2 = g.reshape(u.numel(), -1), out.reshape(u.numel(), -1)
        s = torch.dot(g2.reshape(-1), o2.reshape(-1))
        gw = torch.addcmul(g2, (u * (-s)).unsqueeze(1), v.unsqueeze(0)) / sigma
        return gw.view_as(out), None, None, None


class _SNStackFn(torch.autograd.Function):

    @staticmethod
    def forward(ctx, n, *args):
        sig, us, vs, ws = args[:n], args[n:2 * n], args[2 * n:3 * n], args[3 * n:4 * n]
        pair_out = args[4 * n] if len(args) > 4 * n else None
        out = bind.sn_stack_fwd([w.detach().contiguous() for w in ws], sig, want_pair=pair_out is not None)
        if pair_out is not None:
            out, pair_out["w"] = out
        ctx.save_for_backward(out, *sig, *us, *vs)
        ctx.geom = (n, [w.shape for w in ws], len(args) - 4 * n)
        return out

    @staticmethod
    def backward(ctx, dW):
        n, shapes, extra = ctx.geom
        out, *rest = ctx.saved_tensors
        gws = bind.sn_stack_bwd(dW.float().contiguous(), out, rest[:n], rest[n:2 * n], rest[2 * n:3 * n], shapes)
        return (None, *([None] * (3 * n)), *gws, *([None] * extra))


def _sn_stack(layers, pair_out=None):
    sns, origs = [], []
    for l in layers:
        if not (isinstance(l, nn.Conv2d) and parametrize.is_parametrized(l, "weight")):
            return None
        sn, w = l.parametrizations.weight[0], l.parametrizations.weight.original
        if not (isinstance(sn, _SpectralNorm) and getattr(sn, "_sigma_pre", None) is not None and sn.training and sn.n_power_iterations == 0
                and w.is_cuda and w.dtype == torch.float32 and w.dim() == 4 and w.shape[3] == 1):
            return None
        sns.append(sn); origs.append(w)
    n = len(layers)
    if n > 8 or any(w.shape != origs[0].shape for w in origs) or origs[0].shape[1] * origs[0].shape[2] * 4 > 60 * 1024:
        return None
    if n > 1 and (origs[0].numel() % 4):
        return None
    return _SNStackFn.apply(n, *[sn._sigma_pre for sn in sns], *[sn._u for sn in sns], *[sn._v for sn in sns], *origs,
                            *([pair_out] if pair_out is not None else []))


def spectral_norm(module, name="weight", n_power_iterations=1, eps=1e-12):
    parametrize.register_parametrization(module, name, _SpectralNorm(getattr(module, name), n_power_iterations, eps))
    return module


class _Im2ColFn(torch.autograd.Function):

    @staticmethod
    def forward(ctx, x, k, stride, pad):
        B, P, H, C = x.shape
        cols = bind.im2col_kx1([x.contiguous()], _geom([x]), C, k, stride, pad)
        ctx.geom = (tuple(x.shape), k, stride, pad)
        return cols.view(B, P, -1, k * C)

    @staticmethod
    def backward(ctx, g):
        shape, k, stride, pad = ctx.geom
        return bind.col2im_kx1(g.contiguous(), shape, k, stride, pad), None, None, None


def _conv_kx1_cl(x, weight, bias, stride, pad):
    k = weight.shape[2]
    if x.is_cuda and x.dtype in (torch.float32, torch.float16, torch.bfloat16) and x.shape[2] + 2 * pad >= k:
        cols = _Im2ColFn.apply(x, k, stride, pad)
        w = weight[:, :, :, 0].permute(0, 2, 1).reshape(weight.shape[0], -1)
        return _linear(cols, w, bias)
    if pad:
        x = F.pad(x, (0, 0, pad, pad))
    cols = x.unfold(2, k, stride)
    Bn, P, To, Cin, _ = cols.shape
    w = weight[:, :, :, 0].reshape(weight.shape[0], Cin * k)
    y = _linear(cols.reshape(Bn, P, To, Cin * k), w, bias)
    return y


class _ConvKx1Fn(torch.autograd.Function):

    @staticmethod
    def forward(ctx, x, weight, bias, stride, pad, cdt):
        B, P, H, C = x.shape
        Cout, _, k, _ = weight.shape
        N = B * P
        H1 = (H + 2 * pad - k) // stride + 1
# ... 26 lines not shown
            ctx.save_for_backward(xp, Wt)
            rows = Hp
        ctx.meta = (x.shape, x.dtype, weight.dtype, None if bias is None else bias.dtype, stride, pad, k, H1, rows)
        return Y.view(B, P, rows, Cout)[:, :, :H1]

    @staticmethod
    def backward(ctx, gy):
        (B, P, H, C), xdt, wdt, bdt, stride, pad, k, H1, rows = ctx.meta
        N = B * P
        Cout = gy.shape[-1]
        cdt = ctx.saved_tensors[0].dtype
        g = F.pad(gy.reshape(N, H1, Cout).to(cdt), (0, 0, 0, rows - H1)).view(N * rows, Cout)
        need_x, need_w, need_b = ctx.needs_input_grad[0], ctx.needs_input_grad[1], ctx.needs_input_grad[2]
        dx = dw = db = None
        if stride == 3:
            xp, Wa, Wb = ctx.saved_tensors
            V = xp.view(N * rows, 3 * C)
            if need_x:
                dV = g @ Wa
                dV[1:, :2 * C].addmm_(g[:-1], Wb)
                dxp = dV.view(N, 3 * rows, C)
            if need_w:
                dWa = _weight_grad(g, V).view(Cout, 3, C)
                dWb = _weight_grad(g[:-1], V[1:, :2 * C]).view(Cout, 2, C)
                dw = torch.cat((dWa, dWb), dim=1).permute(0, 2, 1).unsqueeze(-1).to(wdt)
            Hp = 3 * rows
        else:
            xp, Wt = ctx.saved_tensors
            Hp = rows
            R = N * Hp - (k - 1)
            if need_x:
                dX = torch.zeros((N * Hp, C), dtype=cdt, device=gy.device)
                for j in range(k):
                    dX[j:j + R].addmm_(g[:R], Wt[j])
                dxp = dX.view(N, Hp, C)
            if need_w:
                dw = torch.stack([_weight_grad(g[:R], xp[j:j + R]) for j in range(k)], dim=2).unsqueeze(-1).to(wdt)
        if need_x:
            avail = min(H, Hp - pad)
            dx = dxp[:, pad:pad + avail]
            if avail < H:
                dx = F.pad(dx, (0, 0, 0, H - avail))
            dx = dx.reshape(B, P, H, C).to(xdt)
        if need_b and bdt is not None:
            db = g.sum(0, dtype=torch.float32 if cdt in (torch.float16, torch.bfloat16) else None).to(bdt)
        return dx, dw, db, None, None, None


def _kx1_mode():
    return knobs.get("VMASR_MPD_CONV") or "unfold"


def _batched_conv_mode():
    return knobs.get("VMASR_MPD_CONV") or "mfma"


def conv_kx1(x, weight, bias, stride, pad):
    k = weight.shape[2]
    mode = _kx1_mode()
    ok = (stride == 3 and k == 5 and mode in ("gemm", "s3")) or (stride == 1 and mode == "gemm")
    if x.is_cuda and ok and x.shape[2] + 2 * pad >= k:
        cdt = _lib.autocast_dtype(x)
        return _ConvKx1Fn.apply(x, weight, bias, stride, pad, cdt)
    return _conv_kx1_cl(x, weight, bias, stride, pad)


def _layer_path(li, act, cdt, prev_dt, stacked, k, stride, pad, Cin, Cout, n, rows_out, rows_in):
    f32 = cdt == torch.float32
    if (not act and prev_dt is not None and f32 and k == 3 and stride == 1 and pad == 1 and Cout == 1
            and prev_dt == torch.float32 and knobs.get("VMASR_CONV_POST") and bind.conv_post_supported(Cin, k)):
        return "post"
    if (act and li == 0 and f32 and k == 5 and stride == 3 and pad == 2 and Cout == 32 and k * Cin == 5 and Cin == 1
            and knobs.get("VMASR_CONV_FIRST")):
        return "first"
    if (f32 and knobs.get("VMASR_MPD_GEMM") == "bf16x3" and act and stacked
            and _batched_conv_mode() == "mfma"
            and (Cin >= 128 or _l1_mode() != "0")
            and bind.conv_mfma_supported_launch(Cin, Cout, k, stride, n, max(_round_up(rows_out, 256), rows_in))):
        return "mfma"
    if _split_mode(k * Cin, Cout, cdt) and Cin % 4 == 0:
        return "split"
    return "gemm"


class PeriodDiscriminator(nn.Module):
    def __init__(self, period, kernel_size=5, stride=3, use_spectral_norm=False, hidden=32):
        super().__init__()
        self.period = period
        norm = weight_norm if use_spectral_norm else spectral_norm
        pad = (kernel_size - 1) // 2
        chans = [1, hidden, hidden * 4, hidden * 16, hidden * 32]
        layers = [norm(nn.Conv2d(chans[i], chans[i + 1], (kernel_size, 1), (stride, 1), padding=(pad, 0)))
                  for i in range(4)]
        layers.append(norm(nn.Conv2d(hidden * 32, hidden * 32, (kernel_size, 1), 1, padding=(2, 0))))
        self.layers = nn.ModuleList(layers)
        self.conv_post = norm(nn.Conv2d(hidden * 32, 1, (3, 1), 1, padding=(1, 0)))

    def forward(self, x, detach_weights=False):
        fmap = []
        b, c, t = x.shape
        if t % self.period != 0:
            n_pad = self.period - (t % self.period)
            x = F.pad(x, (0, n_pad), "reflect")
            t = t + n_pad
        wb = (lambda l: (l.weight.detach(), l.bias.detach())) if detach_weights else (lambda l: (l.weight, l.bias))
        if not x.is_cuda or _PLAIN_OPS[0]:
            x = x.view(b, c, t // self.period, self.period)
            for layer in list(self.layers) + [self.conv_post]:
                w, bias = wb(layer)
                x = F.conv2d(x, w, bias, layer.stride, layer.padding)
                if layer is not self.conv_post:
                    x = F.gelu(x)
                fmap.append(x)
            return torch.flatten(x, 1, -1), fmap
        x = x.view(b, c, t // self.period, self.period).permute(0, 3, 2, 1)
        for layer in self.layers:
            w, bias = wb(layer)
            x = F.gelu(conv_kx1(x, w, bias, layer.stride[0], layer.padding[0]))
            fmap.append(x)
        w, bias = wb(self.conv_post)
        x = conv_kx1(x, w, bias, 1, self.conv_post.padding[0])
        fmap.append(x)
        return torch.flatten(x, 1, -1), fmap


class MultiPeriodDiscriminator(nn.Module):
    def __init__(self, hidden=32, periods=(2, 3, 5, 7, 11)):
        super().__init__()
        self.discriminators = nn.ModuleList([PeriodDiscriminator(p, hidden=hidden) for p in periods])
        self._frozen = None

    def frozen_weights(self):
        import contextlib

        @contextlib.contextmanager
        def ctx():
            object.__setattr__(self, "_frozen", {})
            try:
                yield
            finally:
                object.__setattr__(self, "_frozen", None)
        return ctx()

    def _forward_batched(self, x, detach_weights=False):
        discs = list(self.discriminators)
        n, (B, _, T) = len(discs), x.shape
        cdt = _lib.autocast_dtype(x)
        cur = []
        for d in discs:
            xp, p = x, d.period
            if T % p:
                xp = F.pad(xp, (0, p - T % p), "reflect")
            cur.append(xp.view(B, 1, -1, p).permute(0, 3, 2, 1).to(cdt))
        fmaps, stacks, valid, taps = [[] for _ in discs], [], [], []
        next_pair = this_link = None
        for li in range(len(discs[0].layers) + 1):
            layers = [d.layers[li] if li < len(d.layers) else d.conv_post for d in discs]
            k, stride, pad = layers[0].kernel_size[0], layers[0].stride[0], layers[0].padding[0]
            P = [c.shape[1] for c in cur]
            H1 = [(c.shape[2] + 2 * pad - k) // stride + 1 for c in cur]
            Ms = [B * p * h for p, h in zip(P, H1)]
            act = li < len(discs[0].layers)
            sgeom, src = None, cur
            pair, next_pair = next_pair, None
            prev_link, this_link = this_link, None
            if stacks and stacks[-1].dtype == cdt and knobs.get("VMASR_STACK_INPUT"):
                sgeom, src = tuple((B * p, c.shape[2]) for c, p in zip(cur, P)), (stacks[-1],)
            rows = _round_up(max(Ms), 256)
            Cin = cur[0].shape[3]
            path = _layer_path(li, act, cdt, stacks[-1].dtype if stacks else None, sgeom is not None, k, stride, pad, Cin,
                               layers[0].out_channels, n, max(Ms), max(B * p * c.shape[2] for c, p in zip(cur, P)))
            wcache = wpair = None
            if path == "mfma" and self._frozen is not None:
                wcache = self._frozen.setdefault(("mfma_ops", li), {})
            W = None
            if knobs.get("VMASR_SN_STACK"):
                key = (li, bool(detach_weights))
                W = self._frozen.get(key) if self._frozen is not None else None
                if W is None:
                    got = {} if (path == "mfma" and not (Cin < 128 and _l1_mode() == "f32")
                                 and (wcache is None or "ops" not in wcache)) else None
                    W = _sn_stack(layers, got)
                    wpair = got.get("w") if got is not None else None
                    if W is not None and detach_weights:
                        W = W.detach()
                    if W is not None and self._frozen is not None:
                        self._frozen[key] = W
            if W is not None:
                ws = [(None, l.bias.detach() if detach_weights else l.bias) for l in layers]
            else:
                ws = [(l.weight.detach(), l.bias.detach()) if detach_weights else (l.weight, l.bias) for l in layers]
                W = torch.stack([w.squeeze(3).transpose(1, 2) for w, _ in ws])
                W = W.reshape(n, W.shape[1], -1)
            bstack = torch.stack([b for _, b in ws])
            if path == "post":
                y = _StackedConvPostFn.apply(tuple(valid[-1]), tuple(c.shape[2] for c in cur), W, bstack, stacks[-1], prev_link)
            elif path == "first":
                y = _StackedConvFirstFn.apply(rows, W, bstack, *cur)
            elif path == "mfma":
                xh, xl = pair if pair is not None else (None, None)
                this_link = _Link()
                y = _StackedConvMfmaFn.apply(k, stride, pad, rows, sgeom, wcache, W, bstack, src[0], xh, xl, this_link, prev_link, wpair)
                next_pair, this_link.pair = this_link.pair, None
            elif path == "split":
                y = _StackedConvSplitFn.apply(k, stride, pad, rows, act, sgeom, W, bstack, *src)
            else:
                cols = _StackedIm2ColFn.apply(k, stride, pad, rows, sgeom, *src)
                y = _BatchedLinearFn.apply(cols, W, bstack, cdt, act)
            tap = None
            if (act and y.requires_grad and y.dtype == torch.float32 and x.requires_grad
                    and knobs.get("VMASR_FEAT_TAP")):
                t = _Tap()
                y, token = _FeatTapFn.apply(y, t)
                tap = (token, t)
                if this_link is not None:
                    this_link.tap = t
            outs = _UnstackRowsFn.apply(y, *Ms)
            cur = [o.view(B, p, h, -1) for o, p, h in zip(outs, P, H1)]
            for f, c in zip(fmaps, cur):
                f.append(c)
            stacks.append(y)
            valid.append(tuple(Ms))
            taps.append(tap)
        return [torch.flatten(c, 1, -1) for c in cur], StackedFeatures(fmaps, stacks, valid, taps)

    def _use_batched(self, x):
        return (x.is_cuda and not _PLAIN_OPS[0] and knobs.get("VMASR_MPD_BATCHED")
                and len(self.discriminators) > 1)

    def forward_single(self, x, detach_weights=False):
        if self._use_batched(x):
            return self._forward_batched(x, detach_weights)
        res = [d(x, detach_weights) for d in self.discriminators]
        return [r[0] for r in res], [r[1] for r in res]

    def forward_pair(self, y, y_hat):
        n = y.shape[0]
        y_real, y_gen, fmap_real, fmap_gen = [], [], [], []
        both = torch.cat((y, y_hat), dim=0)
        if self._use_batched(both):
            scores, feats = self._forward_batched(both)
            y_real, y_gen = [s[:n] for s in scores], [s[n:] for s in scores]
            fmap_real = StackedFeatures([[t[:n] for t in f] for f in feats], feats.stacks, [tuple(m // 2 for m in v) for v in feats.valid])
            return y_real, y_gen, fmap_real, [[t[n:] for t in f] for f in feats]
        else:
            res = [d(both) for d in self.discriminators]
        for s, f in res:
            y_real.append(s[:n]); y_gen.append(s[n:])
            fmap_real.append([t[:n] for t in f]); fmap_gen.append([t[n:] for t in f])
        return y_real, y_gen, fmap_real, fmap_gen

    def spectral_norms(self):
        return [m for m in self.modules() if isinstance(m, _SpectralNorm)]

    def power_iterate_all(self, n_iter, with_sigma=False):
        pairs = [(mod.parametrizations.weight[0], mod.parametrizations.weight.original)
                 for mod in self.modules() if isinstance(mod, nn.Conv2d) and parametrize.is_parametrized(mod, "weight")
                 and isinstance(mod.parametrizations.weight[0], _SpectralNorm)]
        if not pairs or not all(w.is_cuda and w.dtype == torch.float32 for _, w in pairs) or len(pairs) > 64:
            return False
        weights = [w.detach() for _, w in pairs]
        batch = getattr(self, "_sn_batch", None)
        if batch is None or not batch.matches(weights):
            batch = SpectralBatch([m for m, _ in pairs], weights)
            object.__setattr__(self, "_sn_batch", batch)
        batch.run(n_iter, with_sigma)
        return True

    def clear_sigmas(self):
        batch = getattr(self, "_sn_batch", None)
        if batch is not None:
            batch.clear_sigma()

    def forward(self, y, y_hat):
        y_real, y_gen, fmap_real, fmap_gen = [], [], [], []
        for disc in self.discriminators:
            r, fr = disc(y)
            y_real.append(r)
            fmap_real.append(fr)
            if y_hat is not None:
                g, fg = disc(y_hat)
                y_gen.append(g)
                fmap_gen.append(fg)
            else:
                y_gen.append(0)
                fmap_gen.append(0)
        return y_real, y_gen, fmap_real, fmap_gen
```

vm_asr_amd/knobs.py:

```python
import os
import warnings
from collections import namedtuple

Knob = namedtuple("Knob", "name kind default values reader doc parse")


def _bad(k, raw, allowed):
    return ValueError(f"{k.name}={raw!r}: expected {allowed}")


def _flag(k, raw):
    if raw == "1":
        return True
    if raw == "0":
        return False
    raise _bad(k, raw, "0 or 1")


def _choice(k, raw):
    if raw in k.values:
        return raw
    raise _bad(k, raw, "one of " + " | ".join(k.values))


def _int(k, raw):
    try:
        return int(raw)
    except ValueError:
        raise _bad(k, raw, "an integer") from None


def _float(k, raw):
    try:
        return float(raw)
    except ValueError:
        raise _bad(k, raw, "a number") from None


def _str(k, raw):
    return raw or k.default


def _comma_list(k, raw):
    return tuple(raw.split(","))


def _step_variant(k, raw):
    if raw == "":
        return None
    if raw == "one":
        return (False, None)
    if raw == "lane":
        return (True, None)
    if raw.startswith("lane:"):
        try:
            share = float(raw[5:])
        except ValueError:
            share = 0.0
        if 0.0 < share < 1.0:
            return (True, share)
    raise _bad(k, raw, "one | lane | lane:<share> with 0 < share < 1")


_PARSE = {"flag": _flag, "choice": _choice, "int": _int, "float": _float, "str": _str}
_FLAG_VALUES = ("0", "1")


def _k(name, kind, default, doc, values=None, reader="python", parse=None):
    if kind == "flag":
        values, default = _FLAG_VALUES, bool(default)
    return Knob(name, kind, default, values, reader, doc, parse or _PARSE.get(kind))


def _csrc(name, default, doc):
    return Knob(name, "csrc", default, None, "csrc", doc, None)


def _external(name, doc):
    return Knob(name, "external", None, None, "external", doc, None)


KNOBS = {k.name: k for k in (
    _k("VMASR_LIB", "str", None, "path of the HIP library instead of vm_asr_amd/libvmasr_hip.so (A/B and sanitizer builds); read at import"),
    _k("VMASR_DETERMINISTIC", "flag", 0, "ordered fp32 accumulation everywhere; every stream-layout decision then keeps one stream (_lib.det_mode())"),
    _k("VMASR_LINEAR_F64ACC", "choice", "auto", "fp32 Linear with float64 accumulation: 1 always, 0 never, auto only where no gradient is recorded",
       values=("auto", "0", "1")),
    _k("VMASR_SKINNY", "choice", "1", "streaming kernel for Linear layers of many rows and few features: 1 where it beats the GEMM library, 0 off, "
       "all every supported shape", values=("1", "0", "all")),
    _k("VMASR_SPLITK_CHUNK", "int", 2048, "fewest rows of one K-split of a weight-gradient GEMM; read at import"),
    _k("VMASR_XPROJ_MAX_D", "int", 512, "largest d_inner that takes the x_proj row kernels instead of einsums; read at import"),
    _k("VMASR_FUSED_MLP", "flag", 1, "LayerNorm + Mlp + residual of a VSS block as one operator (mlp.py)"),
    _k("VMASR_FUSED_INPROJ", "flag", 1, "LayerNorm + in_proj + split + SiLU as one operator (inproj.py)"),
    _k("VMASR_FUSED_OUTPROJ", "flag", 1, "out_proj + DropPath + residual as one operator (outproj.py)"),
    _k("VMASR_SS2D_FUSED", "flag", 1, "the d_state-1 SS2D core (x_proj, dt_proj, four-direction scan, merge) as one operator (ss2d_core.py)"),
    _k("VMASR_SS2D_DEEP", "flag", 1, "the deep stages' SS2D core on the row-parallel kernels (ss2d_deep.py)"),
    _k("VMASR_SS2D_GLUE", "flag", 1, "the pre-scan and gated-LayerNorm glue kernels (ss2d_glue.py)"),
    _k("VMASR_SS2D_PAIRS", "flag", 1, "magnitude and phase blocks of equal shape through one gated-LayerNorm launch (ss2d_glue.py)"),
    _k("VMASR_IM2COL2D", "flag", 1, "the generator's 2-D convolutions through the row-major im2col kernel (model.py)"),
    _k("VMASR_STFT_LOSS", "flag", 1, "the multi-resolution STFT loss kernel (loss.py)"),
    _k("VMASR_LSGAN", "flag", 1, "the least-squares GAN loss kernel (loss.py)"),
    _k("VMASR_MPD_BATCHED", "flag", 1, "all period discriminators layer by layer on stacked operands"),
    _k("VMASR_MPD_GEMM", "choice", "bf16x3", "fp32 discriminator GEMMs as bf16x3 MFMA triples, or fp32 library GEMMs", values=("bf16x3", "fp32")),
    _k("VMASR_MPD_CONV", "choice", None, "ONE variable read at two sites.  conv_kx1 (one discriminator at a time; unset = unfold): gemm = the "
       "im2col-free GEMM form for stride 3 and stride 1, s3 = that form for the stride-3 layers only, unfold or mfma = unfold + GEMM.  "
       "Batched path (unset = mfma): mfma = the implicit-GEMM MFMA kernels for the compute-bound layers, gemm / s3 / unfold = not those",
       values=("mfma", "gemm", "s3", "unfold")),
    _k("VMASR_MPD_CONV_L1", "choice", "f32", "the 32 -> 128 layer: f32 exact-fp32 MFMA implicit GEMM, 1 bf16x3 pairs, 0 library GEMMs",
       values=("f32", "1", "0")),
    _k("VMASR_MPD_SPLIT_MIN", "int", 1 << 18, "smallest K * N of a stacked layer that takes the split (hi, lo) GEMM path"),
    _k("VMASR_MPD_KCAT", "flag", 0, "the split GEMM's three products as one GEMM over a concatenated K"),
    _k("VMASR_MPD_FUSE_GELU_BWD", "flag", 1, "the activation backward inside the input-gradient epilogue"),
    _k("VMASR_SN_STACK", "flag", 1, "spectral normalisation, stack and permutation of a layer's weights in one launch"),
    _k("VMASR_STACK_INPUT", "flag", 1, "a layer reads the previous layer's stacked output directly"),
    _k("VMASR_CONV_POST", "flag", 1, "the 1-channel output convolution straight on the stacked maps"),
    _k("VMASR_CONV_FIRST", "flag", 1, "the 1 -> 32 channel input convolution + GELU straight from the folded signals"),
    _k("VMASR_FEAT_TAP", "flag", 1, "a feature map's gradient (next layer's + feature-matching loss's) formed in one pass"),
    _k("VMASR_FEAT_L1", "flag", 1, "the feature-matching loss on the stacked maps in one kernel"),
    _k("VMASR_MSD_CONV", "choice", "hip", "the MSD's strided grouped 1-D convolutions: hip = the exact-fp32 MFMA kernels (csrc/gconv1d.hip), "
       "torch = F.conv1d (A/B measurements, double backward)", values=("hip", "torch"), reader="python:msd"),
    _k("VMASR_MSD_STEM", "choice", "hip", "the MSD's 1 -> hidden stem convolution + GELU: hip = one fused pass that keeps no pre-activation "
       "(csrc/stem1d.hip), torch = F.conv1d + F.gelu (A/B measurements, double backward)", values=("hip", "torch"), reader="python:msd"),
    _k("VMASR_MSD_FEAT", "choice", "hip", "the MSD's feature-matching loss in the generator's pass: hip = formed on the way (the stem's share inside "
       "the stem kernels, the other maps in the one-pass L1 kernel; msd_featmatch.py), torch = forward_single + the loop of sub, abs, mean",
       values=("hip", "torch"), reader="python:msd"),
    _k("VMASR_TWO_STREAM", "choice", "1", "the discriminator on a side stream: 1 on, 0 one stream, force also in deterministic mode (test hook)",
       values=("1", "0", "force")),
    _k("VMASR_SHARE_FAKE_PASS", "flag", 1, "one discriminator pass over the fake batch serves both phases of the step"),
    _k("VMASR_GEN_STREAMS", "choice", "auto", "the generator's phase branch on a stream of its own in captured steps: auto where the trainer says so, "
       "1 off, 2 on, 2eager on in eager steps too (debugging aid)", values=("auto", "1", "2", "2eager")),
    _k("VMASR_GEN_LANES", "list", None, "comma list of the segments that leave the main stream (pe,e0..e3,d0..d3,out,ia); unset = all (dev aid)",
       parse=_comma_list),
    _k("VMASR_STEP_VARIANT", "variant", None, "pins the captured step layout: one | lane | lane:<share of the CUs for the discriminator's backward>",
       values=("one", "lane", "lane:0.75"), parse=_step_variant),
    _k("VMASR_SIDE_CUS", "int", None, "CU limit of the discriminator's convolutions beside the generator's backward (and forward unless "
       "VMASR_SIDE_CUS_FWD is set); 0 = no limit; unset = Trainer.side_cu_limits()"),
    _k("VMASR_SIDE_CUS_FWD", "int", None, "the same beside the generator's forward"),
    _k("VMASR_SIDE_CUS_MINC", "int", 0, "the backward limit only for layers at least this wide"),
    _k("VMASR_GRAPH_GC_GUARD", "flag", 1, "no cyclic garbage collection between a graph capture and its first replays"),
    _k("VMASR_PHASE_EVENTS", "flag", 0, "device-clock marks at the step's phase boundaries (tools/phase_probe.py)"),
    _k("VMASR_LN_DEFER", "flag", 1, "LayerNorm's dgamma / dbeta of a whole backward pass reduced in one launch"),
    _k("VMASR_HIP_ADAMW", "flag", 1, "the multi-tensor AdamW kernel on the flat gradient buffers"),
    _k("VMASR_FUSED_ADAMW", "flag", 1, "torch's fused AdamW where the HIP kernel does not apply"),
    _k("VMASR_LP_SHADOWS", "flag", 1, "bf16 shadow copies of the parameters, refreshed by the optimiser kernel"),
    _k("VMASR_LP_SHADOWS_T", "flag", 1, "transposed bf16 shadows of the 2-D weights too"),
    _k("VMASR_RESUME_CONFIG_MISMATCH", "choice", "raise", "a checkpoint written under another configuration: raise or warn", values=("raise", "warn")),
    _k("VMASR_DIST_BACKEND", "str", None, "torch.distributed backend; unset = nccl on a GPU, else gloo"),
    _k("VMASR_DIST_TIMEOUT_S", "int", 600, "process-group timeout in seconds"),
    _k("VMASR_RCCL_TIMEOUT_S", "float", 300.0, "watchdog of a captured collective in seconds (rccl.py)"),
    _k("VMASR_RCCL_DIRECT", "flag", 0, "the trainer's own RCCL communicator outside captures too"),
    _k("VMASR_GRAPH_COLLECTIVES", "flag", 0, "capture the gradient all-reduces into the step's graph"),
    _k("VMASR_OVERLAP_REDUCE", "flag", 1, "asynchronous gradient all-reduces; 0 = strictly between the graphs"),
    _k("VMASR_GRAD_COMM", "choice", "fp32", "wire dtype of the gradient all-reduce: fp32, mpd-bf16 the discriminator's as bf16, bf16 both",
       values=("fp32", "mpd-bf16", "bf16")),
    _k("VMASR_GRAD_COMM_EMULATE", "choice", None, "one rank: the 16-bit wire's rounding applied to this rank's own gradient", values=("mpd-bf16", "bf16")),
    _csrc("VMASR_CONV_CU_SLACK", 24, "convgemm.hip: CUs by which the convolution CU limit is soft"),
    _csrc("VMASR_CONV_TILE", 0, "convgemm.hip: 128 forces the small tile"),
    _csrc("VMASR_CONV_MFMA", 16, "convgemm.hip: 16 = the 16x16x32 MFMA form, 32 = 32x32x16"),
    _csrc("VMASR_CONV_F32_TILE", 128, "convgemm.hip: tile of the exact-fp32 form, 128 or 256"),
    _csrc("VMASR_XPROJ_MFMA", 0, "xproj.hip: 1 = the MFMA kernels (measured slower)"),
    _csrc("VMASR_SSCAN_N_RB", 0, "sscan_n.hip: rows per workgroup; 0 = planned"),
    _csrc("VMASR_SSCAN_N_PP", 0, "sscan_n.hip: state pairs per wave; 0 = planned"),
    _csrc("VMASR_BWD_WAVES", 0, "sscan.hip: waves of the d_state-1 backward; 0 = 8"),
    _csrc("VMASR_SSCAN_N_LEGACY", 0, "sscan.hip: non-zero = the one-state-at-a-time kernels for general d_state (A/B)"),
    _external("VMASR_BENCH_WATCHDOG", "bench.py: seconds after which a wedged run dumps its stacks and exits"),
    _external("VMASR_PARITY_TABLE", "tests/conftest.py: path of the achieved-error table the session writes"),
    _external("VMASR_TEST_CLIPS", "tests/test_fullsize.py: clips of the full-size accuracy test"),
    _external("VMASR_ORACLE_LIB", "oracle/oracle.py: path of the oracle library (sanitizer build)"),
    _external("VMASR_REFERENCE", "tests/golden/_refload.py: checkout of the reference project that regenerates the goldens"),
)}


def get(name):
    k = KNOBS[name]
    raw = os.environ.get(name)
    return k.default if raw is None else k.parse(k, raw)


def undeclared():
    return sorted(n for n in os.environ if n.startswith("VMASR_") and n not in KNOBS)


def warn_undeclared():
    names = undeclared()
    if names:
        warnings.warn(f"unknown VMASR_* variables in the environment (ignored): {', '.join(names)}; vm_asr_amd/knobs.py lists the switches",
                      stacklevel=2)
```

vm_asr_amd/mpd_featloss.py:

```python
import torch

from . import knobs, mpd_ops as bind


class StackedFeatures(list):

    def __init__(self, per_disc, stacks, valid, taps=None):
        super().__init__(per_disc)
        self.stacks, self.valid = stacks, valid
        self.taps = taps if taps is not None else [None] * len(stacks)

    def detach(self):
        return StackedFeatures([[f.detach() for f in fs] for fs in self], [y.detach() for y in self.stacks], self.valid)


class _FeatTapFn(torch.autograd.Function):

    @staticmethod
    def forward(ctx, y, tap):
        ctx.tap = tap
        ctx.set_materialize_grads(False)
        return y.view_as(y), y.new_zeros(1)

    @staticmethod
    def backward(ctx, gy, gtok):
        t = ctx.tap
        sgn = t.sgn
        t.gtok = None
        consumed, t.consumed = t.consumed, False
        if consumed:
            return gy, None
        if gtok is None or sgn is None:
            return gy, None
        add = None if gy is None else gy.float().contiguous()
        return bind.masked_l1_bwd(sgn, gtok.float().contiguous(), t.valid, t.scale, add, tap=True), None


_FEAT_MASKS = {}


class _MaskedL1Fn(torch.autograd.Function):

    @staticmethod
    def forward(ctx, real, gen, valid, scale, token, tap):
        tapped = token is not None and ctx.needs_input_grad[4]
        partials, sgn = bind.masked_l1_fwd(real, gen, valid, scale, ctx.needs_input_grad[1] or tapped)
        ctx.meta = (valid, scale, gen.shape)
        ctx.tapped = tapped
        ctx.tap = tap if tapped else None
        if tapped:
            tap.offer(sgn, valid, scale)
        elif sgn is not None:
            ctx.save_for_backward(sgn)
        return partials.sum().float()

    @staticmethod
    def backward(ctx, g):
        if ctx.tapped:
            ctx.tap.gtok = g.detach().reshape(1).float().contiguous()
            return None, None, None, None, g.reshape(1), None
        (sgn,) = ctx.saved_tensors
        valid, scale, _ = ctx.meta
        return None, bind.masked_l1_bwd(sgn, g.float().contiguous(), valid, scale), None, None, None, None


def _masked_l1_ok(yr, yg):
    return (yg.is_cuda and yr.is_cuda and yg.dtype == torch.float32 and yr.dtype == torch.float32 and yg.is_contiguous()
            and yr.is_contiguous() and not yr.requires_grad and yg.shape[0] <= 8 and yg.shape[0] == yr.shape[0]
            and (yg.shape[1] * yg.shape[2]) % 4 == 0 and (yr.shape[1] * yr.shape[2]) % 4 == 0
            and knobs.get("VMASR_FEAT_L1"))


def feature_loss_stacked(real, gen):
    if not (isinstance(real, StackedFeatures) and isinstance(gen, StackedFeatures)) or real.valid != gen.valid:
        return None
    n_maps = sum(len(fs) for fs in gen)
    total = None
    for yr, yg, valid, tap in zip(real.stacks, gen.stacks, real.valid, gen.taps):
        R, N = min(yr.shape[1], yg.shape[1]), yg.shape[2]
        if max(valid) > R:
            return None
        if _masked_l1_ok(yr, yg):
            scale = tuple(1.0 / (m * N * n_maps) for m in valid)
            if tap is not None and tap[0].requires_grad and not tap[1].fed:
                term = _MaskedL1Fn.apply(yr, yg.detach(), tuple(valid), scale, *tap)
            else:
                term = _MaskedL1Fn.apply(yr, yg, tuple(valid), scale, None, None)
            total = term if total is None else total + term
            continue
        key = (yg.device, valid, R, N, n_maps)
        mask = _FEAT_MASKS.get(key)
        if mask is None:
            rows = torch.arange(R, device=yg.device).unsqueeze(0)
            m = torch.tensor(valid, device=yg.device).unsqueeze(1)
            mask = ((rows < m).float() / (m.float() * N * n_maps)).unsqueeze(2)
            _FEAT_MASKS[key] = mask
        term = ((yg[:, :R] - yr[:, :R]).abs() * mask).sum()
        total = term if total is None else total + term
    return total
```

vm_asr_amd/mpd_layers.py:

```python
import torch
import torch.nn.functional as F

from . import _lib, knobs, mpd_ops as bind
from .linear import _mm_acc
from .mpd_ops import geom_of as _geom, split_bf16



def _round_up(v, m):
    return -(-v // m) * m


class _StackedIm2ColFn(torch.autograd.Function):

    @staticmethod
    def forward(ctx, k, stride, pad, rows, geom, *xs):
        if geom is not None:
            src = xs[0].contiguous()
            ctx.geom = (k, stride, pad, None, tuple(geom), tuple(src.shape))
        else:
            src, geom = [x.contiguous() for x in xs], _geom(xs)
            ctx.geom = (k, stride, pad, [tuple(x.shape) for x in xs], None, None)
        return bind.im2col_kx1(src, geom, src[0].shape[-1], k, stride, pad, rows)

# ... 104 lines not shown
        return 1
    return max(d for d in range(1, want + 1) if blocks % d == 0)


def _dw3(gh, gl, ch, cl, wdt):
    n, M, N = gh.shape
    K = ch.shape[2]
    S = _split_k(n, N, K, M)
    v = (lambda t: t.view(n * S, M // S, t.shape[2])) if S > 1 else (lambda t: t)
    ght, glt = v(gh).transpose(1, 2), v(gl).transpose(1, 2)
    parts = torch.empty((3, n * S, N, K), dtype=torch.float32, device=gh.device)
    torch.bmm(ght, v(ch), out_dtype=torch.float32, out=parts[0])
    torch.bmm(glt, v(ch), out_dtype=torch.float32, out=parts[1])
    torch.bmm(ght, v(cl), out_dtype=torch.float32, out=parts[2])
    if (N * K) % 4 == 0 and n <= 65535:
        return bind.sum_parts(parts, 3, n, S, (N, K)).to(wdt)
    return parts.view(3, n, S, N, K).sum((0, 2)).to(wdt)


def _split_mode(K, N, cdt):
    return (cdt == torch.float32 and K * N >= knobs.get("VMASR_MPD_SPLIT_MIN")
            and knobs.get("VMASR_MPD_GEMM") == "bf16x3")


class _BatchedLinearSplitFn(torch.autograd.Function):

    @staticmethod
    def forward(ctx, cols, weight, bias):
        ch, cl = split_bf16(cols)
        w = weight.detach().float()
        wh, wl = split_bf16(w)
        wth, wtl = split_bf16(w.transpose(1, 2).contiguous())
        y = _bmm3(ch, cl, wth, wtl).add_(bias.detach().float().unsqueeze(1))
        ctx.save_for_backward(ch, cl, wh, wl)
        ctx.meta = (weight.dtype, bias.dtype)
        return y

    @staticmethod
    def backward(ctx, gy):
        ch, cl, wh, wl = ctx.saved_tensors
        wdt, bdt = ctx.meta
        gy = gy.float().contiguous()
        n, M, N = gy.shape
        K = ch.shape[2]
        gh, gl = split_bf16(gy)
        dcols = _bmm3(gh, gl, wh, wl) if ctx.needs_input_grad[0] else None
        if skip_weight_grads.on:
            return dcols, None, None
        dw = db = None
        if ctx.needs_input_grad[1]:
            dw = _dw3(gh, gl, ch, cl, wdt)
        if ctx.needs_input_grad[2]:
            db = gy.sum(1).to(bdt)
        return dcols, dw, db


class _StackedConvSplitFn(torch.autograd.Function):

    @staticmethod
    def forward(ctx, k, stride, pad, rows, act, geom, weight, bias, *xs):
        sgeom = tuple(geom) if geom is not None else None
        if geom is not None:
            src = xs[0].float().contiguous()
        else:
            src, geom = [x.float().contiguous() for x in xs], _geom(xs)
        C, dev = xs[0].shape[-1], xs[0].device
        n, K = len(geom), k * C
        w = weight.detach().float().contiguous()
        N = w.shape[1]
        fused = act and N % 4 == 0 and N <= 1024
        kcat = fused and knobs.get("VMASR_MPD_KCAT")
        if kcat:
            acat = bind.im2col_kx1_split(src, geom, C, k, stride, pad, rows, cat3=True)
            ch, cl = acat[:, :, :K], acat[:, :, K:2 * K]
        else:
            ch, cl = bind.im2col_kx1_split(src, geom, C, k, stride, pad, rows)
        wcat = bind.weight_prep_split(w)
        wth, wtl = wcat[:, :, :N], wcat[:, :, 2 * N:]
        b32 = bias.detach().float().contiguous()
        pre = None
        if kcat:
            f32 = torch.float32
            wk = torch.cat((wth, wth, wtl), dim=1)
            pre = torch.bmm(acat, wk, out_dtype=f32)
            y = bind.bias_gelu_fwd(pre, b32)
        elif fused:
            f32 = torch.float32
            parts = torch.empty((3, n, rows, N), dtype=f32, device=dev)
            torch.bmm(ch, wth, out_dtype=f32, out=parts[0])
            torch.bmm(cl, wth, out_dtype=f32, out=parts[1])
            torch.bmm(ch, wtl, out_dtype=f32, out=parts[2])
            pre = parts[0]
            y = bind.bias_gelu_fwd(parts, b32, 3)
        else:
            y = _bmm3(ch, cl, wth, wtl)
            y.add_(b32.unsqueeze(1))
            if act:
                pre = y
                y = F.gelu(pre)
        ctx.save_for_backward(ch, cl, wcat, *([pre] if pre is not None else []))
        ctx.geom = (k, stride, pad, [tuple(x.shape) for x in xs], weight.dtype, bias.dtype, [x.dtype for x in xs], act, fused, sgeom)
        return y

    @staticmethod
    def backward(ctx, gy):
        ch, cl, wcat, *rest = ctx.saved_tensors
        k, stride, pad, shapes, wdt, bdt, xdts, act, fused, sgeom = ctx.geom
        gy = gy.float().contiguous()
        n, M, N = gy.shape
        K = ch.shape[2]
        want_db = ctx.needs_input_grad[7] and not skip_weight_grads.on
        want_dx = any(ctx.needs_input_grad[8:])
        db32 = gcat = None
        if N % 4 == 0 and N <= 1024:
            db32, = _lib.zeros_f32(gy.device, (n, N) if want_db else None)
            gh, gl, gcat = bind.gelu_bwd_split(rest[0] if act else None, gy, db32, cat=want_dx)
        else:
            if act:
                gy = torch.ops.aten.gelu_backward(gy, rest[0])
            gh, gl = split_bf16(gy)
            db32 = gy.sum(1) if want_db else None
        dxs = [None] * len(shapes)
        if want_dx:
            if gcat is None:
                gcat = torch.cat((gh, gl, gh), dim=2)
            dcols = torch.bmm(gcat, wcat.transpose(1, 2), out_dtype=torch.float32)
            if sgeom is not None:
                dxs = [bind.col2im_kx1_stacked(dcols, sgeom, shapes[0], k, stride, pad).to(xdts[0])]
            else:
                outs = bind.col2im_kx1_multi(dcols, shapes, k, stride, pad, ctx.needs_input_grad[8:])
                dxs = [o.to(xdts[i]) if o is not None else None for i, o in enumerate(outs)]
        dw = db = None
        if not skip_weight_grads.on:
            if ctx.needs_input_grad[6]:
                dw = _dw3(gh, gl, ch, cl, wdt)
            if ctx.needs_input_grad[7]:
                db = db32.to(bdt)
        return (None, None, None, None, None, None, dw, db, *dxs)


def _dgrad_operand(ops, key, pair, w, k, n, N, C):
    if key not in ops:
        if bind.weight_transpose_supported(N, C):
            ops[key] = bind.weight_transpose(w, k, pair=pair)
        else:
            wt = w.view(n, N, k, C).permute(0, 3, 2, 1).reshape(n, C, k * N).contiguous()
            ops[key] = split_bf16(wt) if pair else wt
    return ops[key]


class _StackedConvMfmaFn(torch.autograd.Function):

    @staticmethod
    def forward(ctx, k, stride, pad, rows, geom, wcache, weight, bias, x, xh, xl, link, below=None, wpair=None):
        from . import convgemm as cg
        x_req = x.requires_grad
        x = x.float().contiguous()
        w = weight.detach().float().contiguous()
        f32 = x.shape[2] < 128 and _l1_mode() == "f32"
        ops = wcache.get("ops") if wcache is not None else None
        if ops is None:
            ops = {} if f32 else {"w": wpair if wpair is not None else split_bf16(w)}
            if wcache is not None:
                wcache["ops"] = ops
        if f32:
            pre, y, yh, yl = cg.conv_fwd_f32(x, w, bias.detach().float().contiguous(), geom, k, stride, pad, rows, act=True)
            xh = xl = x
        else:
            if xh is None:
                xh, xl = split_bf16(x)
            wh, wl = ops["w"]
            pre, y, yh, yl = cg.conv_fwd(xh, xl, wh, wl, bias.detach().float().contiguous(), geom, k, stride, pad, rows, act=True)
        ctx.save_for_backward(xh, xl, pre, w)
        ctx.f32 = f32
        ctx.meta = (k, stride, pad, tuple(geom), ops, weight.dtype, bias.dtype, x.shape)
        ctx.link, ctx.below = link, below
        link.fill(pre, x.shape[2], x_req, weight.requires_grad, bias.requires_grad, pair=(yh, yl))
        return y

    @staticmethod
    def _fuse_below(ctx, gh, gl, wth, wtl, geom, k, stride, pad, rows_in, skip_w):
        from . import convgemm as cg
        plan = ctx.below.plan(skip_w, scores_only.on) if ctx.below is not None else None
        if plan is None:
            return False
        db32 = _lib.zeros_f32(gh.device, (gh.shape[0], wth.shape[1]))[0] if plan.want_db else None
        g32, pair = cg.conv_dgrad_gelu(gh, gl, wth, wtl, geom, k, stride, pad, rows_in, ctx.below.pre, want_f32=plan.want_f32,
                                       want_pair=plan.want_pair, db=db32, **(plan.loss or {}))
        ctx.below.put(g32, pair, db32)
        return True

    @staticmethod
    def backward(ctx, gy):
        from . import convgemm as cg
        xh, xl, pre, w = ctx.saved_tensors
        k, stride, pad, geom, ops, wdt, bdt, xshape = ctx.meta
        n, M, N = gy.shape
        C = xshape[2]
        skip_w = skip_weight_grads.on
        want_db = ctx.needs_input_grad[7] and not skip_w
        fp32_dgrad = C < 128 and ctx.needs_input_grad[8]
        need_pair = (not fp32_dgrad and ctx.needs_input_grad[8]) or (ctx.needs_input_grad[6] and not skip_w)
        gh = gl = gx = None
        stash = ctx.link.take()
        if stash is not None:
            gx, pair_, db32 = stash
            gh, gl = pair_ if pair_ is not None else (None, None)
            if (want_db and db32 is None) or (need_pair and gh is None) or (fp32_dgrad and gx is None):
                raise RuntimeError("MPD: the fused activation backward left less than this layer's backward needs")
        if stash is None:
            gy = gy.float().contiguous()
            db32, = _lib.zeros_f32(gy.device, (n, N) if want_db else None)
            if need_pair:
                gh, gl, _ = bind.gelu_bwd_split(pre, gy, db32)
            if fp32_dgrad:
                gx, _ = bind.gelu_bwd(pre, gy, None if need_pair else db32)
        dx = dw = db = None
        if fp32_dgrad and ctx.f32:
            dx = cg.conv_dgrad_f32(gx, _dgrad_operand(ops, "wt32", False, w, k, n, N, C), geom, k, stride, pad, xshape[1])
        elif fp32_dgrad:
            dx = bind.col2im_kx1_stacked(torch.bmm(gx, w), geom, xshape, k, stride, pad)
        elif ctx.needs_input_grad[8]:
            wth, wtl = _dgrad_operand(ops, "wt", True, w, k, n, N, C)
            if _StackedConvMfmaFn._fuse_below(ctx, gh, gl, wth, wtl, geom, k, stride, pad, xshape[1], skip_w):
                dx = _poison(gy.device).expand(xshape)
            else:
                dx = cg.conv_dgrad(gh, gl, wth, wtl, geom, k, stride, pad, xshape[1])
        if not skip_w:
            if ctx.needs_input_grad[6]:
                if ctx.f32:
                    xh, xl = split_bf16(xh)
                dw = cg.conv_wgrad(gh, gl, xh, xl, geom, k, stride, pad).to(wdt)
            if want_db:
                db = db32.to(bdt)
        return (None, None, None, None, None, None, dw, db, dx, None, None, None, None, None)


_POISON = {}


def _poison(device):
    t = _POISON.get(device)
    if t is None:
        t = _POISON[device] = torch.full((), float("nan"), dtype=torch.float32, device=device)
    return t


def _l1_mode():
    return knobs.get("VMASR_MPD_CONV_L1")


class _StackedConvFirstFn(torch.autograd.Function):

    @staticmethod
    def forward(ctx, rows, W, bias, *xs):
        xcs = [x.float().contiguous() for x in xs]
        w32, b32 = W.detach().float().contiguous(), bias.detach().float().contiguous()
        pre, act = bind.conv_first_fwd(xcs, _geom(xcs), w32, b32, rows)
        ctx.save_for_backward(pre, w32, *xcs)
        ctx.meta = (W.dtype, bias.dtype, [x.dtype for x in xs], [tuple(x.shape) for x in xs])
        return act

    @staticmethod
    def backward(ctx, gy):
        pre, w32, *xcs = ctx.saved_tensors
        wdt, bdt, xdts, shapes = ctx.meta
        gy = gy.float().contiguous()
        skip_w = skip_weight_grads.on
        want_dw, want_db = ctx.needs_input_grad[1] and not skip_w, ctx.needs_input_grad[2] and not skip_w
        want_dx = any(ctx.needs_input_grad[3:])
        dxs = [None] * len(xcs)
        dcols, dw, db = bind.conv_first_bwd(xcs, _geom(shapes), w32, pre, gy, want_dx, want_dw, want_db)
        if want_dx:
            outs = bind.col2im_kx1_multi(dcols, shapes, 5, 3, 2, ctx.needs_input_grad[3:])
            dxs = [o.to(xdts[i]) if o is not None else None for i, o in enumerate(outs)]
        return (None, dw.to(wdt) if want_dw else None, db.to(bdt) if want_db else None, *dxs)


class _StackedConvPostFn(torch.autograd.Function):

    @staticmethod
    def forward(ctx, Ms, Hs, W, bias, x, below=None):
        xc, w32, b32 = x.contiguous(), W.detach().float().contiguous(), bias.detach().float().contiguous()
        y = bind.conv_post_fwd(xc, w32, b32, Ms, Hs)
        ctx.save_for_backward(xc, w32)
        ctx.meta = (tuple(Ms), tuple(Hs), W.dtype, bias.dtype, tuple(bias.shape))
        ctx.below = below
        return y

    @staticmethod
    def _fuse_below(ctx, xc, w32, gy, Ms, Hs, want_dw, want_db, skip_w):
        plan = ctx.below.plan(skip_w, scores_only.on, map_shape=xc.shape) if ctx.below is not None else None
        if plan is None:
            return None
        g32, pair, dbcol, dw, db = bind.conv_post_bwd_gelu(xc, w32, gy, ctx.below.pre, Ms, Hs, plan.want_pair, plan.want_f32, want_dw, want_db,
                                                           plan.want_db, **(plan.loss or {}))
        ctx.below.put(g32, pair, dbcol)
        return dw, db

    @staticmethod
    def backward(ctx, gy):
        xc, w32 = ctx.saved_tensors
        Ms, Hs, wdt, bdt, bshape = ctx.meta
        gy = gy.float().contiguous()
        skip_w = skip_weight_grads.on
        want_dx, want_dw, want_db = ctx.needs_input_grad[4], ctx.needs_input_grad[2] and not skip_w, ctx.needs_input_grad[3] and not skip_w
        fused = _StackedConvPostFn._fuse_below(ctx, xc, w32, gy, Ms, Hs, want_dw, want_db, skip_w) if want_dx else None
        if fused is not None:
            (dw, db), dx = fused, _poison(gy.device).expand(xc.shape)
        else:
            dx, dw, db = bind.conv_post_bwd(xc, w32, gy, Ms, Hs, want_dx, want_dw, want_db)
        return (None, None, dw.to(wdt) if want_dw else None, db.view(bshape).to(bdt) if want_db else None, dx, None)


class _UnstackRowsFn(torch.autograd.Function):

    @staticmethod
    def forward(ctx, y, *Ms):
        ctx.shape = tuple(y.shape)
        ctx.Ms = Ms
        return tuple(y[i, :m] for i, m in enumerate(Ms))

    @staticmethod
    def backward(ctx, *gs):
        ref = next(g for g in gs if g is not None)
        if ref.is_cuda and len(gs) <= 8:
            return (bind.stack_rows(gs, ctx.Ms, ctx.shape, ref), *([None] * len(ctx.Ms)))
        full = torch.empty(ctx.shape, dtype=ref.dtype, device=ref.device)
        for i, (g, m) in enumerate(zip(gs, ctx.Ms)):
            if g is None:
                full[i].zero_()
            else:
                full[i, :m].copy_(g)
                if m < ctx.shape[1]:
                    full[i, m:].zero_()
        return (full, *([None] * len(ctx.Ms)))
```

vm_asr_amd/mpd_link.py:

```python
from collections import namedtuple

Plan = namedtuple("Plan", "want_f32 want_pair want_db loss")


class _Tap:
    __slots__ = ("sgn", "valid", "scale", "gtok", "consumed")

    def __init__(self):
        self.sgn = self.valid = self.scale = self.gtok = None
        self.consumed = False

    def offer(self, sgn, valid, scale):
        self.sgn, self.valid, self.scale = sgn, valid, scale

    @property
    def fed(self):
        return self.sgn is not None

    def loss_term(self):
        if self.sgn is None or self.gtok is None:
            return None
        return dict(sgn=self.sgn, gtok=self.gtok, scale=self.scale, valid=self.valid)


class _Link:
    __slots__ = ("pre", "C", "x_req", "w_req", "b_req", "tap", "pair", "_stash")

    def __init__(self):
        self.pre = self.C = self.tap = self.pair = self._stash = None
        self.x_req = self.w_req = self.b_req = False

    def fill(self, pre, C, x_req, w_req, b_req, pair):
        self.pre, self.C, self.x_req, self.w_req, self.b_req, self.pair = pre, C, x_req, w_req, b_req, pair

    def put(self, g32, pair, db):
        if self._stash is not None:
            raise RuntimeError("MPD: the fused activation backward of an earlier pass was never taken by the layer below")
        self._stash = (g32, pair, db)

    def take(self):
        stash, self._stash = self._stash, None
        return stash

    def plan(self, skip_w, scores_only, map_shape=None):
        from . import _lib, knobs
        if (self.pre is None or not knobs.get("VMASR_MPD_FUSE_GELU_BWD") or _lib.det_mode()
                or (map_shape is not None and self.pre.shape != map_shape)):
            return None
        want_db = bool(self.b_req and not skip_w)
        want_f32 = bool(self.C < 128 and self.x_req)
        want_pair = bool((not want_f32 and self.x_req) or (self.w_req and not skip_w))
        if not (want_f32 or want_pair):
            return None
        loss = self.tap.loss_term() if self.tap is not None else None
        if loss is not None and map_shape is not None and self.tap.sgn.shape != map_shape:
            loss = None
        if loss is not None:
            self.tap.consumed = True
        elif not scores_only:
            return None
        return Plan(want_f32, want_pair, want_db, loss)
```

vm_asr_amd/mpd_ops.py:

```python
import ctypes

import torch

from . import _lib
from ._lib import ptr as _p

_F32, _BF16 = torch.float32, torch.bfloat16


def need(*ts):
    for t in ts:
        if t is not None and not (t.is_cuda and t.is_contiguous()):
            raise RuntimeError("vm_asr_amd: tensors must be contiguous CUDA tensors (there is no CPU path)")


def _call(fn, *args):
    need(*[a for a in args if torch.is_tensor(a)])
    _lib.call(fn, *args)


def _new(like, shape, dtype=None):
    return torch.empty(shape, dtype=dtype or like.dtype, device=like.device)


# ... 28 lines not shown
    x0, (nseq0, H0), src = xs[0], geom[0], _ptrs(xs, len(geom))
    cols = _new(x0, (len(geom), rows or nseq0 * ((H0 + 2 * pad - k) // stride + 1), k * C))
    for i, (nseq, H) in enumerate(geom):
        _lib.call(_lib.lib().vmasr_im2col_kx1, src[i], cols[i], nseq, H, C, k, stride, pad, rows, _lib.torch_dtype_code(x0.dtype))
    return cols


def col2im_kx1(g, shape, k, stride, pad):
    B, P, H, C = shape
    dx = _new(g, shape)
    _call(_lib.lib().vmasr_col2im_kx1, g, dx, B * P, H, C, k, stride, pad, _lib.torch_dtype_code(g.dtype))
    return dx


def im2col_kx1_split(xs, geom, C, k, stride, pad, rows, cat3=False):
    n, x0 = len(geom), xs[0]
    ptrs, Ns, Hs = _slots(xs, geom)
    if cat3:
        acat = _new(x0, (n, rows, 3 * k * C), _BF16)
        _call(_lib.lib().vmasr_im2col_kx1_split3_multi, ptrs, Ns, Hs, n, acat, C, k, stride, pad, rows)
        return acat
    ch, cl = _new(x0, (n, rows, k * C), _BF16), _new(x0, (n, rows, k * C), _BF16)
    _call(_lib.lib().vmasr_im2col_kx1_split_multi, ptrs, Ns, Hs, n, ch, cl, C, k, stride, pad, rows)
    return ch, cl


def col2im_kx1_multi(dcols, shapes, k, stride, pad, want=None):
    dxs = [_new(dcols, shp) if want is None or want[i] else None for i, shp in enumerate(shapes)]
    ptrs, Ns, Hs = _slots(dxs, geom_of(shapes))
    _call(_lib.lib().vmasr_col2im_kx1_multi, dcols, ptrs, Ns, Hs, len(shapes), shapes[0][3], k, stride, pad, dcols.shape[1],
          _lib.torch_dtype_code(dcols.dtype))
    return dxs


def col2im_kx1_stacked(dcols, geom, shape, k, stride, pad):
    n, rows_in, C = shape
    dx = _new(dcols, shape)
    _, Ns, Hs = _slot_arrays([0] * n, [g[0] for g in geom], [g[1] for g in geom])
    _call(_lib.lib().vmasr_col2im_kx1_stacked, dcols, dx, Ns, Hs, n, C, k, stride, pad, dcols.shape[1], rows_in,
          _lib.torch_dtype_code(dcols.dtype))
    return dx


def stack_rows(gs, Ms, shape, like):
    full = _new(like, shape)
    gc = [g.contiguous() if g is not None else None for g in gs]
    ptrs, Ms, _ = _slot_arrays([g.data_ptr() if g is not None else 0 for g in gc], list(Ms))
    _call(_lib.lib().vmasr_stack_rows, ptrs, Ms, len(gs), full, shape[1], shape[2] * like.element_size())
    return full


def split_bf16(x):
    x = x.contiguous()
    hi, lo = _new(x, x.shape, _BF16), _new(x, x.shape, _BF16)
    _call(_lib.lib().vmasr_split_bf16, x, hi, lo, x.numel())
    return hi, lo


def weight_prep_split(w):
    n, N, K = w.shape
    wcat = _new(w, (n, K, 3 * N), _BF16)
    _call(_lib.lib().vmasr_weight_prep_split, w, wcat, n, N, K)
    return wcat


def bias_gelu_fwd(pre, bias, nparts=1):
    n, M, N = pre.shape[-3:]
    y = _new(pre, (n, M, N))
    _call(_lib.lib().vmasr_bias_gelu_fwd, pre, bias, y, n, M, N, nparts)
    return y


def gelu_bwd(pre, gy, db=None, want_db=None):
    gx = torch.empty_like(gy)
    if want_db is not None:
        db, = _lib.zeros_f32(gy.device, (gy.shape[0], gy.shape[2]) if want_db else None)
    _call(_lib.lib().vmasr_gelu_bwd, pre, gy, gx, db, *gy.shape)
    return gx, db


def gelu_bwd_split(pre, gy, db=None, cat=False):
    n, M, N = gy.shape
    gcat = _new(gy, (n, M, 3 * N), _BF16) if cat else None
    gh, gl = (gcat[:, :, :N], gcat[:, :, N:2 * N]) if cat else (_new(gy, (n, M, N), _BF16), _new(gy, (n, M, N), _BF16))
    _call(_lib.lib().vmasr_gelu_bwd_split, pre, gy, None if cat else gh, None if cat else gl, gcat, db, n, M, N)
    return gh, gl, gcat


def sum_parts(parts, nparts, n, S, shape):
    out = _new(parts, (n, *shape))
    _call(_lib.lib().vmasr_sum_parts, parts, out, nparts, n, S, parts.numel() // (nparts * n * S))
    return out


def conv_first_fwd(xs, geom, w, bias, rows):
    n, (ptrs, Ns, Hs) = len(xs), _slots(xs, geom)
    pre, act = _new(w, (n, rows, 32)), _new(w, (n, rows, 32))
    _call(_lib.lib().vmasr_conv_first_fwd, ptrs, Ns, Hs, n, w, bias, pre, act, rows)
    return pre, act


def conv_first_bwd(xs, geom, w, pre, gy, want_dx, want_dw, want_db):
    n, rows, _ = pre.shape
    ptrs, Ns, Hs = _slots(xs, geom)
    dcols = _new(pre, (n, rows, 5)) if want_dx else None
    dw, db = _lib.zeros_f32(pre.device, (n, 32, 5) if want_dw else None, (n, 32) if want_db else None)
    _call(_lib.lib().vmasr_conv_first_bwd, ptrs, Ns, Hs, n, w, pre, gy, dcols, dw, db, rows)
    return dcols, dw, db


def conv_post_supported(C, k):
    return bool(_lib.lib().vmasr_conv_post_supported(int(C), int(k)))


def conv_post_fwd(x, w, bias, Ms, Hs):
    n, rows, C = x.shape
    ms, hs = (ctypes.c_int64 * n)(*Ms), (ctypes.c_int32 * n)(*Hs)
    y = _new(x, (n, rows, 1), _F32)
    _call(_lib.lib().vmasr_conv_post_fwd, x, w, bias, y, ms, hs, n, rows, C, 3)
    return y


def conv_post_bwd(x, w, gy, Ms, Hs, want_dx, want_dw, want_db):
    n, rows, C = x.shape
    ms, hs = (ctypes.c_int64 * n)(*Ms), (ctypes.c_int32 * n)(*Hs)
    dx = torch.empty_like(x) if want_dx else None
    dw, db = _lib.zeros_f32(x.device, (n, 1, 3 * C) if want_dw else None, (n,) if want_db else None)
    _call(_lib.lib().vmasr_conv_post_bwd, x, w, gy, dx, dw, db, ms, hs, n, rows, C, 3)
    return dx, dw, db


def conv_post_bwd_gelu(x, w, gy, pre, Ms, Hs, want_pair, want_f32, want_dw, want_db, want_dbcol, sgn=None, gtok=None, valid=None, scale=None):
    n, rows, C = x.shape
    ms, hs = (ctypes.c_int64 * n)(*Ms), (ctypes.c_int32 * n)(*Hs)
    v, sc = _valid_scale(valid, scale) if sgn is not None else (None, None)
    g32 = torch.empty_like(x) if want_f32 else None
    gh = _new(x, x.shape, _BF16) if want_pair else None
    gl = _new(x, x.shape, _BF16) if want_pair else None
    dw, db, dbcol = _lib.zeros_f32(x.device, (n, 1, 3 * C) if want_dw else None, (n,) if want_db else None, (n, C) if want_dbcol else None)
    _call(_lib.lib().vmasr_conv_post_bwd_gelu, x if want_dw else None, w, gy, pre, sgn, gtok if sgn is not None else None, v, sc, gh, gl, g32,
          dw, db, dbcol, ms, hs, n, rows, C, 3)
    return g32, ((gh, gl) if want_pair else None), dbcol, dw, db


def conv_mfma_supported_launch(Cin, Cout, k, stride, n, rows):
    return bool(_lib.lib().vmasr_conv_mfma_supported_launch(int(Cin), int(Cout), int(k), int(stride), int(n), int(rows)))


def _valid_scale(valid, scale):
    n = len(valid)
    return (ctypes.c_int64 * n)(*valid), (ctypes.c_float * n)(*scale)


def masked_l1_fwd(real, gen, valid, scale, want_sgn):
    n, rows_g, N = gen.shape
    v, sc = _valid_scale(valid, scale)
    partials = _new(gen, n * _lib.lib().vmasr_masked_l1_blocks(), torch.float64)
    sgn = _new(gen, (n, rows_g, N), torch.int8) if want_sgn else None
    _call(_lib.lib().vmasr_masked_l1_fwd, real, gen, sgn, partials, v, sc, n, real.shape[1], rows_g, N)
    return partials, sgn


def masked_l1_bwd(sgn, g, valid, scale, add=None, tap=False):
    v, sc = _valid_scale(valid, scale)
    out = _new(sgn, sgn.shape, _F32)
    if tap:
        _call(_lib.lib().vmasr_masked_l1_bwd_add, sgn, g, add, out, v, sc, *sgn.shape)
    else:
        _call(_lib.lib().vmasr_masked_l1_bwd, sgn, g, out, v, sc, *sgn.shape)
    return out


def sn_stack_fwd(ws, sig, want_pair=False):
    n, (N, Cin, k) = len(ws), ws[0].shape[:3]
    out = _new(ws[0], (n, N, k * Cin), _F32)
    hi, lo = (_new(out, out.shape, _BF16), _new(out, out.shape, _BF16)) if want_pair else (None, None)
    _call(_lib.lib().vmasr_sn_stack_fwd, _ptr_array(ws), _ptr_array(sig), n, out, hi, lo, N, Cin, k)
    return (out, (hi, lo)) if want_pair else out


def weight_transpose_supported(N, Cin):
    return Cin % 4 == 0 and N % 8 == 0


def weight_transpose(w, k, pair):
    n, N, K = w.shape
    Cin = K // k
    if pair:
        hi, lo = _new(w, (n, Cin, k * N), _BF16), _new(w, (n, Cin, k * N), _BF16)
        _call(_lib.lib().vmasr_weight_transpose, w, hi, lo, None, n, N, Cin, k)
        return hi, lo
    out = _new(w, (n, Cin, k * N), _F32)
    _call(_lib.lib().vmasr_weight_transpose, w, None, None, out, n, N, Cin, k)
    return out


def sn_stack_bwd(dW, out, sig, us, vs, shapes):
    n, (N, Cin, k) = len(shapes), shapes[0][:3]
    gws = [_new(dW, shp, _F32) for shp in shapes]
    partials = _new(dW, n * _lib.lib().vmasr_sn_dot_blocks(), torch.float64)
    _call(_lib.lib().vmasr_sn_stack_bwd, dW, out, _ptr_array(gws), _ptr_array(sig), _ptr_array(us), _ptr_array(vs), n,
          partials, N, Cin, k)
    return gws


def spectral_power_iter(w, u, v, n_iter, eps):
    R, C = w.shape
    ws = _new(w, R + C)
    _call(_lib.lib().vmasr_spectral_power_iter, w, u, v, ws, R, C, int(n_iter), float(eps))


class SpectralBatch:

    def __init__(self, modules, weights):
        import numpy as np
        assert 0 < len(modules) <= 64
        dev = weights[0].device
        self.modules, self.eps = list(modules), float(modules[0].eps)
        mats = [w.detach() for w in weights]
        assert all(w.is_cuda and w.dtype == torch.float32 and w.is_contiguous() for w in mats)
        shapes = [(w.shape[0], w[0].numel()) for w in mats]
        self.ws = torch.zeros(sum(r + c for r, c in shapes), dtype=torch.float32, device=dev)
        item = np.dtype([("W", "u8"), ("u", "u8"), ("v", "u8"), ("t", "u8"), ("s", "u8"), ("R", "i4"), ("C", "i4"), ("rb", "i4"), ("ct", "i4")])
        tab = np.zeros(len(mats), dtype=item)
        off = rb = ct = 0
        for i, (m, w, (r, c)) in enumerate(zip(self.modules, mats, shapes)):
            tab[i] = (w.data_ptr(), m._u.data_ptr(), m._v.data_ptr(), self.ws.data_ptr() + 4 * off,
                      self.ws.data_ptr() + 4 * (off + r), r, c, rb, ct)
            off += r + c
            rb += -(-r // 4)
            ct += -(-c // 1024) * -(-r // 32)
        self.n, self.row_blocks, self.col_tiles = len(mats), rb, ct
        self.weight_bytes = sum(4 * r * c for r, c in shapes)
        self.ptrs = [(w.data_ptr(), m._u.data_ptr(), m._v.data_ptr()) for m, w in zip(self.modules, mats)]
        self.sigma = torch.ones(len(mats), dtype=torch.float32, device=dev)
        self.table = torch.from_numpy(tab.view(np.uint8).copy()).to(dev)

    def matches(self, weights):
        return len(weights) == self.n and all(
            (w.data_ptr(), m._u.data_ptr(), m._v.data_ptr()) == p for m, w, p in zip(self.modules, weights, self.ptrs))

    @torch.no_grad()
    def run(self, n_iter, with_sigma=False):
        _call(_lib.lib().vmasr_spectral_power_iter_batched, self.table, self.n, self.row_blocks, self.col_tiles, self.weight_bytes,
              int(n_iter), self.eps, self.sigma if with_sigma else None)
        if with_sigma:
            for i, m in enumerate(self.modules):
                object.__setattr__(m, "_sigma_pre", self.sigma[i])

    def clear_sigma(self):
        for m in self.modules:
            object.__setattr__(m, "_sigma_pre", None)
```

Measured before the change: 200.2 clips/s.

## Skip storing unused MPD forward outputs; form feature loss from pre-activations

Stacked MFMA discriminator layers now store only the outputs the next layer reads. The fp32 GELU map is dropped when the next layer is also MFMA, since it consumes the bf16 pair instead, and the bf16 pair is dropped under conv_post. The feature-matching L1 loss instead recomputes GELU from the stored pre-activations inside a templated kernel. This cuts write bandwidth in the forward pass, at the cost of recomputing erf-based GELU in the loss and some added complexity: lazy materialisation of the maps and poison placeholder tensors.

```diff
diff --git a/include/vmasr_hip.h b/include/vmasr_hip.h
--- a/include/vmasr_hip.h
+++ b/include/vmasr_hip.h
@@ -271,6 +271,9 @@
 int32_t vmasr_masked_l1_blocks(void);
 int vmasr_masked_l1_fwd(const float *real, const float *gen, void *sgn, double *partials, const int64_t *valid, const float *scale,
                         int32_t n, int64_t rows_r, int64_t rows_g, int32_t N, vmasr_stream_t stream);
+int vmasr_masked_l1_fwd_pre(const float *real_pre, const float *gen_pre, void *sgn, double *partials, const int64_t *valid, const float *scale,
+                            int32_t n, int64_t rows_r, int64_t rows_g, int32_t N, vmasr_stream_t stream);
+int vmasr_mpd_gelu_fwd(const float *pre, float *y, int64_t count, vmasr_stream_t stream);
 int vmasr_masked_l1_bwd(const void *sgn, const float *gout, float *dgen, const int64_t *valid, const float *scale, int32_t n,
                         int64_t rows_g, int32_t N, vmasr_stream_t stream);
 int vmasr_masked_l1_bwd_add(const void *sgn, const float *gout, const float *add, float *dgen, const int64_t *valid, const float *scale,
diff --git a/vm_asr_amd/_lib.py b/vm_asr_amd/_lib.py
--- a/vm_asr_amd/_lib.py
+++ b/vm_asr_amd/_lib.py
@@ -124,6 +124,8 @@
     "vmasr_adamw_step": (ctypes.c_int, [c_vp, c_vp, c_i32, c_i64, c_vp, c_vp, ctypes.c_float, ctypes.c_float, ctypes.c_float, c_vp]),
     "vmasr_masked_l1_blocks": (c_i32, []),
     "vmasr_masked_l1_fwd": (ctypes.c_int, [c_vp, c_vp, c_vp, c_vp, c_vp, c_vp, c_i32, c_i64, c_i64, c_i32, c_vp]),
+    "vmasr_masked_l1_fwd_pre": (ctypes.c_int, [c_vp, c_vp, c_vp, c_vp, c_vp, c_vp, c_i32, c_i64, c_i64, c_i32, c_vp]),
+    "vmasr_mpd_gelu_fwd": (ctypes.c_int, [c_vp, c_vp, c_i64, c_vp]),
     "vmasr_masked_l1_bwd": (ctypes.c_int, [c_vp, c_vp, c_vp, c_vp, c_vp, c_i32, c_i64, c_i32, c_vp]),
     "vmasr_lsgan_fwd": (ctypes.c_int, [c_vp, c_vp, c_vp, c_i32, c_vp, c_vp]),
     "vmasr_lsgan_bwd": (ctypes.c_int, [c_vp, c_vp, c_vp, c_vp, c_i32, c_vp, c_vp]),
diff --git a/vm_asr_amd/convgemm.py b/vm_asr_amd/convgemm.py
--- a/vm_asr_amd/convgemm.py
+++ b/vm_asr_amd/convgemm.py
@@ -58,11 +58,11 @@
     return (H + 2 * pad - k) // stride + 1
 
 
-def _fwd(fn, xh, xl, wh, wl, bias, geom, k, stride, pad, rows_out, act, want_pair):
+def _fwd(fn, xh, xl, wh, wl, bias, geom, k, stride, pad, rows_out, act, want_pair, want_act=True):
     _need(xh, xl, wh, wl, bias)
     (n, _, Cin), Cout, dev = xh.shape, wh.shape[1], xh.device
     pre = torch.empty((n, rows_out, Cout), dtype=torch.float32, device=dev)
-    y = torch.empty_like(pre) if act else None
+    y = torch.empty_like(pre) if act and want_act else None
     yh = torch.empty((n, rows_out, Cout), dtype=torch.bfloat16, device=dev) if act and want_pair else None
     yl = torch.empty_like(yh) if yh is not None else None
     sl = _slots(geom, ah=xh, al=xl, bh=wh, bl=wl, c0=pre, c1=y, ch=yh, cl=yl, bias=bias)
@@ -81,17 +81,17 @@
     return dx
 
 
-def conv_fwd(xh, xl, wh, wl, bias, geom, k, stride, pad, rows_out, act=True, want_pair=True):
-    return _fwd(_lib.lib().vmasr_conv_mfma_fwd, xh, xl, wh, wl, bias, geom, k, stride, pad, rows_out, act, want_pair)
+def conv_fwd(xh, xl, wh, wl, bias, geom, k, stride, pad, rows_out, act=True, want_pair=True, want_act=True):
+    return _fwd(_lib.lib().vmasr_conv_mfma_fwd, xh, xl, wh, wl, bias, geom, k, stride, pad, rows_out, act, want_pair, want_act)
 
 
 def conv_dgrad(gh, gl, wth, wtl, geom, k, stride, pad, rows_in):
     return _dgrad(_lib.lib().vmasr_conv_mfma_dgrad, gh, gl, wth, wtl, geom, k, stride, pad, rows_in)
 
 
-def conv_fwd_f32(x, w, bias, geom, k, stride, pad, rows_out, act=True, want_pair=True):
+def conv_fwd_f32(x, w, bias, geom, k, stride, pad, rows_out, act=True, want_pair=True, want_act=True):
     assert x.dtype == torch.float32 and w.dtype == torch.float32
-    return _fwd(_lib.lib().vmasr_conv_f32_fwd, x, None, w, None, bias, geom, k, stride, pad, rows_out, act, want_pair)
+    return _fwd(_lib.lib().vmasr_conv_f32_fwd, x, None, w, None, bias, geom, k, stride, pad, rows_out, act, want_pair, want_act)
 
 
 def conv_dgrad_f32(g, wt, geom, k, stride, pad, rows_in):
diff --git a/vm_asr_amd/csrc/convgemm.hip b/vm_asr_amd/csrc/convgemm.hip
--- a/vm_asr_amd/csrc/convgemm.hip
+++ b/vm_asr_amd/csrc/convgemm.hip
@@ -3,6 +3,7 @@
 #include <type_traits>
 
 #include "common.h"
+#include "gelu.h"
 
 namespace vmasr {
 namespace {
@@ -51,7 +52,6 @@
 __device__ __forceinline__ int cg_swz(const int row) { return (0 - (row >> 2)) & 3; }
 __device__ __forceinline__ int cg_off(const int row, const int chunk) { return row * 64 + ((chunk ^ cg_swz(row)) << 4); }
 
-__device__ __forceinline__ float cg_gelu(float x) { return 0.5f * x * (1.f + erff(x * 0.70710678118654752f)); }
 __device__ __forceinline__ float cg_gelu_grad(float x) {
     return 0.5f * (1.f + erff(x * 0.70710678118654752f)) + x * 0.3989422804014327f * __expf(-0.5f * x * x);
 }
@@ -716,6 +716,7 @@
     for (int i = 0; i < n; ++i) {
         const vmasr_cg_slot &s = slots[i];
         VMASR_REQUIRE(s.ah && s.bh && s.c0 && (ops || (s.al && s.bl)), VMASR_EINVAL, "%s: null tensor in slot %d", what, i);
+        VMASR_REQUIRE(!s.ch == !s.cl && (act || (!s.c1 && !s.ch)), VMASR_EINVAL, "%s: slot %d: ch / cl go together, c1 / ch / cl need act", what, i);
         VMASR_REQUIRE(!ops || (aligned_to(s.ah, 16) && aligned_to(s.bh, 16)), VMASR_EALIGN, "%s: slot %d: operands must be 16-byte aligned", what, i);
         const int64_t H1 = ((int64_t)s.H + 2 * pad - k) / stride + 1;
         const int64_t M = s.nseq * H1;
@@ -728,7 +729,7 @@
         p.hq_mul = stride; p.hq_add = -pad; p.crow_mul = 1; p.crow_add = 0;
         p.ntaps = k; p.tap0 = 0; p.tap_step = 1; p.dstep = 1;
         p.zero_rows = (int)rows_out;
-        bytes += (double)s.nseq * s.H * Cin * 4 + (double)Cout * k * Cin * 4 + (double)M * Cout * (act ? 12 : 4);
+        bytes += (double)s.nseq * s.H * Cin * 4 + (double)Cout * k * Cin * 4 + (double)M * Cout * (4 + (s.c1 ? 4 : 0) + (s.ch ? 4 : 0));
     }
     hipStream_t st = static_cast<hipStream_t>(stream);
     if (ops) VMASR_REQUIRE(Cout % 128 == 0, VMASR_EINVAL, "%s: Cout %% 128", what);
diff --git a/vm_asr_amd/csrc/featloss.hip b/vm_asr_amd/csrc/featloss.hip
--- a/vm_asr_amd/csrc/featloss.hip
+++ b/vm_asr_amd/csrc/featloss.hip
@@ -1,6 +1,7 @@
 #include <algorithm>
 
 #include "common.h"
+#include "gelu.h"
 
 namespace vmasr {
 namespace {
@@ -14,9 +15,11 @@
 
 __device__ __forceinline__ signed char sgn1(float d) { return (signed char)((d > 0.f) - (d < 0.f)); }
 
+template <bool PRE>
 __global__ __launch_bounds__(256) void masked_l1_fwd_kernel(const float *__restrict__ real, const float *__restrict__ gen,
                                                             signed char *__restrict__ sgn, double *__restrict__ partials,
                                                             const L1Slots t, const size_t stride_r, const size_t stride_g) {
+#pragma clang fp contract(off)
     const int s = blockIdx.y;
     const float *__restrict__ r = real + (size_t)s * stride_r;
     const float *__restrict__ g = gen + (size_t)s * stride_g;
@@ -24,7 +27,11 @@
     const long n = t.valid_elems[s], n4 = n / 4;
     double acc = 0.0;
     for (long i = (long)blockIdx.x * blockDim.x + threadIdx.x; i < n4; i += (long)gridDim.x * blockDim.x) {
-        const float4 a = reinterpret_cast<const float4 *>(g)[i], b = reinterpret_cast<const float4 *>(r)[i];
+        float4 a = reinterpret_cast<const float4 *>(g)[i], b = reinterpret_cast<const float4 *>(r)[i];
+        if constexpr (PRE) {
+            a = make_float4(cg_gelu(a.x), cg_gelu(a.y), cg_gelu(a.z), cg_gelu(a.w));
+            b = make_float4(cg_gelu(b.x), cg_gelu(b.y), cg_gelu(b.z), cg_gelu(b.w));
+        }
         const float d0 = a.x - b.x, d1 = a.y - b.y, d2 = a.z - b.z, d3 = a.w - b.w;
         acc += (double)((fabsf(d0) + fabsf(d1)) + (fabsf(d2) + fabsf(d3)));
         if (o) {
@@ -35,7 +42,7 @@
     }
     if (blockIdx.x == 0 && (int)threadIdx.x < (int)(n - n4 * 4)) {
         const long i = n4 * 4 + threadIdx.x;
-        const float d = g[i] - r[i];
+        const float d = PRE ? cg_gelu(g[i]) - cg_gelu(r[i]) : g[i] - r[i];
         acc += (double)fabsf(d);
         if (o) o[i] = sgn1(d);
     }
@@ -89,8 +96,9 @@
 
 VMASR_EXPORT int32_t vmasr_masked_l1_blocks(void) { return 256 * 4; }
 
-VMASR_EXPORT int vmasr_masked_l1_fwd(const float *real, const float *gen, void *sgn, double *partials, const int64_t *valid,
-                                     const float *scale, int32_t n, int64_t rows_r, int64_t rows_g, int32_t N, vmasr_stream_t stream) {
+namespace {
+int masked_l1_fwd(bool pre, const float *real, const float *gen, void *sgn, double *partials, const int64_t *valid, const float *scale, int32_t n,
+                  int64_t rows_r, int64_t rows_g, int32_t N, vmasr_stream_t stream) {
     VMASR_REQUIRE(real && gen && partials && valid && scale, VMASR_EINVAL, "masked_l1_fwd: null argument");
     VMASR_REQUIRE(n > 0 && n <= kMaxSlots && rows_r > 0 && rows_g > 0 && N > 0, VMASR_EINVAL, "masked_l1_fwd: bad shape");
     VMASR_REQUIRE(((size_t)rows_r * N) % 4 == 0 && ((size_t)rows_g * N) % 4 == 0 && aligned_to(real, 16) && aligned_to(gen, 16) &&
@@ -101,9 +109,43 @@
     double bytes = 0;
     for (int s = 0; s < n; ++s) bytes += (double)t.valid_elems[s] * (sgn ? 9.0 : 8.0);
     hipStream_t st = static_cast<hipStream_t>(stream);
-    VMASR_LAUNCH(VMASR_K_FEAT_L1, bytes, masked_l1_fwd_kernel, dim3(vmasr_masked_l1_blocks(), n), dim3(256), 0, st, real, gen,
-                 static_cast<signed char *>(sgn), partials, t, (size_t)rows_r * N, (size_t)rows_g * N);
+    if (pre)
+        VMASR_LAUNCH(VMASR_K_FEAT_L1, bytes, masked_l1_fwd_kernel<true>, dim3(vmasr_masked_l1_blocks(), n), dim3(256), 0, st, real, gen,
+                     static_cast<signed char *>(sgn), partials, t, (size_t)rows_r * N, (size_t)rows_g * N);
+    else
+        VMASR_LAUNCH(VMASR_K_FEAT_L1, bytes, masked_l1_fwd_kernel<false>, dim3(vmasr_masked_l1_blocks(), n), dim3(256), 0, st, real, gen,
+                     static_cast<signed char *>(sgn), partials, t, (size_t)rows_r * N, (size_t)rows_g * N);
     return check_launch("masked_l1_fwd");
+}
+}
+
+VMASR_EXPORT int vmasr_masked_l1_fwd(const float *real, const float *gen, void *sgn, double *partials, const int64_t *valid,
+                                     const float *scale, int32_t n, int64_t rows_r, int64_t rows_g, int32_t N, vmasr_stream_t stream) {
+    return masked_l1_fwd(false, real, gen, sgn, partials, valid, scale, n, rows_r, rows_g, N, stream);
+}
+
+VMASR_EXPORT int vmasr_masked_l1_fwd_pre(const float *real_pre, const float *gen_pre, void *sgn, double *partials, const int64_t *valid,
+                                         const float *scale, int32_t n, int64_t rows_r, int64_t rows_g, int32_t N, vmasr_stream_t stream) {
+    return masked_l1_fwd(true, real_pre, gen_pre, sgn, partials, valid, scale, n, rows_r, rows_g, N, stream);
+}
+
+namespace {
+__global__ __launch_bounds__(256) void mpd_gelu_fwd_kernel(const float4 *__restrict__ pre, float4 *__restrict__ y, const long n4) {
+    for (long i = (long)blockIdx.x * blockDim.x + threadIdx.x; i < n4; i += (long)gridDim.x * blockDim.x) {
+        const float4 p = pre[i];
+        y[i] = make_float4(cg_gelu(p.x), cg_gelu(p.y), cg_gelu(p.z), cg_gelu(p.w));
+    }
+}
+}
+
+VMASR_EXPORT int vmasr_mpd_gelu_fwd(const float *pre, float *y, int64_t count, vmasr_stream_t stream) {
+    VMASR_REQUIRE(pre && y && count > 0 && count % 4 == 0 && aligned_to(pre, 16) && aligned_to(y, 16), VMASR_EINVAL,
+                  "mpd_gelu_fwd: count %% 4 == 0, 16-byte aligned tensors");
+    const long n4 = (long)(count / 4);
+    const int blocks = (int)std::min<long>((n4 + 255) / 256, 256L * 8);
+    VMASR_LAUNCH(VMASR_K_FEAT_L1, 8.0 * count, mpd_gelu_fwd_kernel, dim3(blocks), dim3(256), 0, static_cast<hipStream_t>(stream),
+                 reinterpret_cast<const float4 *>(pre), reinterpret_cast<float4 *>(y), n4);
+    return check_launch("mpd_gelu_fwd");
 }
 
 VMASR_EXPORT int vmasr_masked_l1_bwd_add(const void *sgn, const float *gout, const float *add, float *dgen, const int64_t *valid,
diff --git a/vm_asr_amd/csrc/gelu.h b/vm_asr_amd/csrc/gelu.h
--- /dev/null
+++ b/vm_asr_amd/csrc/gelu.h
@@ -0,0 +1,4 @@
+#pragma once
+#include <hip/hip_runtime.h>
+
+__device__ __forceinline__ float cg_gelu(float x) { return 0.5f * x * (1.f + erff(x * 0.70710678118654752f)); }
diff --git a/vm_asr_amd/discriminator.py b/vm_asr_amd/discriminator.py
--- a/vm_asr_amd/discriminator.py
+++ b/vm_asr_amd/discriminator.py
@@ -10,8 +10,8 @@
 from .mpd_featloss import StackedFeatures, _FeatTapFn, _MaskedL1Fn, _masked_l1_ok, feature_loss_stacked
 from .mpd_layers import (_BatchedLinearFn, _BatchedLinearSplitFn, _StackedConvFirstFn, _StackedConvMfmaFn, _StackedConvPostFn,
                          _StackedConvSplitFn, _StackedIm2ColFn, _UnstackRowsFn, _bmm3, _dw3, _l1_mode, _poison, _round_up, _split_k,
-                         _split_mode, scores_only, skip_weight_grads)
-from .mpd_link import _Link, _Tap
+                         _split_mode, scores_only, skip_weight_grads, unstored)
+from .mpd_link import _Link, _Tap, forward_outputs
 from .mpd_ops import SpectralBatch, _slot_arrays, geom_of as _geom, split_bf16
 
 __all__ = ["PeriodDiscriminator", "MultiPeriodDiscriminator", "spectral_norm", "plain_torch_ops"]
@@ -344,7 +344,8 @@
             if T % p:
                 xp = F.pad(xp, (0, p - T % p), "reflect")
             cur.append(xp.view(B, 1, -1, p).permute(0, 3, 2, 1).to(cdt))
-        fmaps, stacks, valid, taps = [[] for _ in discs], [], [], []
+        fmaps, stacks, valid, taps, pres = [[] for _ in discs], [], [], [], []
+        n_act = len(discs[0].layers)
         next_pair = this_link = None
         for li in range(len(discs[0].layers) + 1):
             layers = [d.layers[li] if li < len(d.layers) else d.conv_post for d in discs]
@@ -362,6 +363,8 @@
             Cin = cur[0].shape[3]
             path = _layer_path(li, act, cdt, stacks[-1].dtype if stacks else None, sgeom is not None, k, stride, pad, Cin,
                                layers[0].out_channels, n, max(Ms), max(B * p * c.shape[2] for c, p in zip(cur, P)))
+            if stacks and unstored(stacks[-1]) and path != "mfma":
+                raise RuntimeError(f"MPD: layer {li} takes the {path!r} path, which reads the fp32 map the layer below did not store")
             wcache = wpair = None
             if path == "mfma" and self._frozen is not None:
                 wcache = self._frozen.setdefault(("mfma_ops", li), {})
@@ -392,7 +395,14 @@
             elif path == "mfma":
                 xh, xl = pair if pair is not None else (None, None)
                 this_link = _Link()
-                y = _StackedConvMfmaFn.apply(k, stride, pad, rows, sgeom, wcache, W, bstack, src[0], xh, xl, this_link, prev_link, wpair)
+                up = discs[0].layers[li + 1] if li + 1 < n_act else discs[0].conv_post
+                k2, s2, p2 = up.kernel_size[0], up.stride[0], up.padding[0]
+                M2 = max(B * p * ((h + 2 * p2 - k2) // s2 + 1) for p, h in zip(P, H1))
+                up_path = _layer_path(li + 1, li + 1 < n_act, cdt, torch.float32, bool(knobs.get("VMASR_STACK_INPUT")), k2, s2, p2,
+                                      layers[0].out_channels, up.out_channels, n, M2, max(Ms))
+                want_act, want_pair = forward_outputs(up_path)
+                y = _StackedConvMfmaFn.apply(k, stride, pad, rows, sgeom, wcache, W, bstack, src[0], xh, xl, this_link, prev_link, wpair,
+                                             want_act, want_pair)
                 next_pair, this_link.pair = this_link.pair, None
             elif path == "split":
                 y = _StackedConvSplitFn.apply(k, stride, pad, rows, act, sgeom, W, bstack, *src)
@@ -414,7 +424,8 @@
             stacks.append(y)
             valid.append(tuple(Ms))
             taps.append(tap)
-        return [torch.flatten(c, 1, -1) for c in cur], StackedFeatures(fmaps, stacks, valid, taps)
+            pres.append(this_link.pre if this_link is not None and unstored(y) else None)
+        return [torch.flatten(c, 1, -1) for c in cur], StackedFeatures(fmaps, stacks, valid, taps, pres)
 
     def _use_batched(self, x):
         return (x.is_cuda and not _PLAIN_OPS[0] and knobs.get("VMASR_MPD_BATCHED")
diff --git a/vm_asr_amd/knobs.py b/vm_asr_amd/knobs.py
--- a/vm_asr_amd/knobs.py
+++ b/vm_asr_amd/knobs.py
@@ -110,6 +110,9 @@
     _k("VMASR_MPD_SPLIT_MIN", "int", 1 << 18, "smallest K * N of a stacked layer that takes the split (hi, lo) GEMM path"),
     _k("VMASR_MPD_KCAT", "flag", 0, "the split GEMM's three products as one GEMM over a concatenated K"),
     _k("VMASR_MPD_FUSE_GELU_BWD", "flag", 1, "the activation backward inside the input-gradient epilogue"),
+    _k("VMASR_MPD_LEAN_FWD", "flag", 1, "a stacked MFMA layer's forward stores only what is read: no fp32 map under a next MFMA layer (the feature-matching "
+       "loss forms it from the pre-activation), no bf16 pair under conv_post; 0 = both always (mpd_link.forward_outputs; tests/test_mpd_lean_forward.py)",
+       reader="python:mpd"),
     _k("VMASR_SN_STACK", "flag", 1, "spectral normalisation, stack and permutation of a layer's weights in one launch"),
     _k("VMASR_STACK_INPUT", "flag", 1, "a layer reads the previous layer's stacked output directly"),
     _k("VMASR_CONV_POST", "flag", 1, "the 1-channel output convolution straight on the stacked maps"),
diff --git a/vm_asr_amd/mpd_featloss.py b/vm_asr_amd/mpd_featloss.py
--- a/vm_asr_amd/mpd_featloss.py
+++ b/vm_asr_amd/mpd_featloss.py
@@ -5,13 +5,51 @@
 
 class StackedFeatures(list):
 
-    def __init__(self, per_disc, stacks, valid, taps=None):
+    def __init__(self, per_disc, stacks, valid, taps=None, pres=None, rows=None):
         super().__init__(per_disc)
         self.stacks, self.valid = stacks, valid
         self.taps = taps if taps is not None else [None] * len(stacks)
+        self.pres = pres if pres is not None else [None] * len(stacks)
+        self.rows = rows if rows is not None else valid
+        if any(p is not None for p in self.pres):
+            for i, fs in enumerate(self):
+                if not isinstance(fs, _Maps):
+                    list.__setitem__(self, i, _Maps(fs))
+                list.__getitem__(self, i).owner = self
+
+    @property
+    def n_maps(self):
+        return sum(len(fs) for fs in list.__iter__(self))
+
+    def materialise(self):
+        from .mpd_layers import _StoredMapFn, _UnstackRowsFn
+        for l, pre in enumerate(self.pres):
+            if pre is None:
+                continue
+            y = _StoredMapFn.apply(self.stacks[l], pre)
+            self.stacks[l], self.pres[l] = y, None
+            for fs, v in zip(list.__iter__(self), _UnstackRowsFn.apply(y, *self.rows[l])):
+                list.__setitem__(fs, l, v.view(list.__getitem__(fs, l).shape))
 
     def detach(self):
-        return StackedFeatures([[f.detach() for f in fs] for fs in self], [y.detach() for y in self.stacks], self.valid)
+        return StackedFeatures([[f.detach() for f in list.__iter__(fs)] for fs in list.__iter__(self)], [y.detach() for y in self.stacks],
+                               self.valid, pres=list(self.pres), rows=self.rows)
+
+
+class _Maps(list):
+    owner = None
+
+    def _real(self):
+        if self.owner is not None and any(p is not None for p in self.owner.pres):
+            self.owner.materialise()
+
+    def __getitem__(self, i):
+        self._real()
+        return list.__getitem__(self, i)
+
+    def __iter__(self):
+        self._real()
+        return list.__iter__(self)
 
 
 class _FeatTapFn(torch.autograd.Function):
@@ -42,9 +80,9 @@
 class _MaskedL1Fn(torch.autograd.Function):
 
     @staticmethod
-    def forward(ctx, real, gen, valid, scale, token, tap):
+    def forward(ctx, real, gen, valid, scale, token, tap, from_pre=False):
         tapped = token is not None and ctx.needs_input_grad[4]
-        partials, sgn = bind.masked_l1_fwd(real, gen, valid, scale, ctx.needs_input_grad[1] or tapped)
+        partials, sgn = bind.masked_l1_fwd(real, gen, valid, scale, ctx.needs_input_grad[1] or tapped, from_pre=from_pre)
         ctx.meta = (valid, scale, gen.shape)
         ctx.tapped = tapped
         ctx.tap = tap if tapped else None
@@ -58,10 +96,10 @@
     def backward(ctx, g):
         if ctx.tapped:
             ctx.tap.gtok = g.detach().reshape(1).float().contiguous()
-            return None, None, None, None, g.reshape(1), None
+            return None, None, None, None, g.reshape(1), None, None
         (sgn,) = ctx.saved_tensors
         valid, scale, _ = ctx.meta
-        return None, bind.masked_l1_bwd(sgn, g.float().contiguous(), valid, scale), None, None, None, None
+        return None, bind.masked_l1_bwd(sgn, g.float().contiguous(), valid, scale), None, None, None, None, None
 
 
 def _masked_l1_ok(yr, yg):
@@ -74,15 +112,26 @@
 def feature_loss_stacked(real, gen):
     if not (isinstance(real, StackedFeatures) and isinstance(gen, StackedFeatures)) or real.valid != gen.valid:
         return None
-    n_maps = sum(len(fs) for fs in gen)
+    n_maps = gen.n_maps
     total = None
-    for yr, yg, valid, tap in zip(real.stacks, gen.stacks, real.valid, gen.taps):
+    for l, (valid, tap) in enumerate(zip(real.valid, gen.taps)):
+        yr, yg, pr, pg = real.stacks[l], gen.stacks[l], real.pres[l], gen.pres[l]
         R, N = min(yr.shape[1], yg.shape[1]), yg.shape[2]
         if max(valid) > R:
             return None
+        tapped = tap is not None and tap[0].requires_grad and not tap[1].fed
+        if pr is not None or pg is not None:
+            if pr is not None and pg is not None and _masked_l1_ok(pr, pg) and (tapped or not yg.requires_grad):
+                scale = tuple(1.0 / (m * N * n_maps) for m in valid)
+                term = _MaskedL1Fn.apply(pr, pg, tuple(valid), scale, *(tap if tapped else (None, None)), True)
+                total = term if total is None else total + term
+                continue
+            real.materialise()
+            gen.materialise()
+            yr, yg = real.stacks[l], gen.stacks[l]
         if _masked_l1_ok(yr, yg):
             scale = tuple(1.0 / (m * N * n_maps) for m in valid)
-            if tap is not None and tap[0].requires_grad and not tap[1].fed:
+            if tapped:
                 term = _MaskedL1Fn.apply(yr, yg.detach(), tuple(valid), scale, *tap)
             else:
                 term = _MaskedL1Fn.apply(yr, yg, tuple(valid), scale, None, None)
diff --git a/vm_asr_amd/mpd_layers.py b/vm_asr_amd/mpd_layers.py
--- a/vm_asr_amd/mpd_layers.py
+++ b/vm_asr_amd/mpd_layers.py
@@ -280,31 +280,37 @@
 class _StackedConvMfmaFn(torch.autograd.Function):
 
     @staticmethod
-    def forward(ctx, k, stride, pad, rows, geom, wcache, weight, bias, x, xh, xl, link, below=None, wpair=None):
+    def forward(ctx, k, stride, pad, rows, geom, wcache, weight, bias, x, xh, xl, link, below=None, wpair=None, want_act=True, want_pair=True):
         from . import convgemm as cg
         x_req = x.requires_grad
-        x = x.float().contiguous()
+        f32 = x.shape[2] < 128 and _l1_mode() == "f32"
+        if unstored(x):
+            if f32 or xh is None:
+                raise RuntimeError("MPD: a layer that reads its fp32 input was handed an unstored map")
+        else:
+            x = x.float().contiguous()
         w = weight.detach().float().contiguous()
-        f32 = x.shape[2] < 128 and _l1_mode() == "f32"
         ops = wcache.get("ops") if wcache is not None else None
         if ops is None:
             ops = {} if f32 else {"w": wpair if wpair is not None else split_bf16(w)}
             if wcache is not None:
                 wcache["ops"] = ops
         if f32:
-            pre, y, yh, yl = cg.conv_fwd_f32(x, w, bias.detach().float().contiguous(), geom, k, stride, pad, rows, act=True)
+            pre, y, yh, yl = cg.conv_fwd_f32(x, w, bias.detach().float().contiguous(), geom, k, stride, pad, rows, act=True,
+                                             want_pair=want_pair, want_act=want_act)
             xh = xl = x
         else:
             if xh is None:
                 xh, xl = split_bf16(x)
             wh, wl = ops["w"]
-            pre, y, yh, yl = cg.conv_fwd(xh, xl, wh, wl, bias.detach().float().contiguous(), geom, k, stride, pad, rows, act=True)
+            pre, y, yh, yl = cg.conv_fwd(xh, xl, wh, wl, bias.detach().float().contiguous(), geom, k, stride, pad, rows, act=True,
+                                         want_pair=want_pair, want_act=want_act)
         ctx.save_for_backward(xh, xl, pre, w)
         ctx.f32 = f32
         ctx.meta = (k, stride, pad, tuple(geom), ops, weight.dtype, bias.dtype, x.shape)
         ctx.link, ctx.below = link, below
-        link.fill(pre, x.shape[2], x_req, weight.requires_grad, bias.requires_grad, pair=(yh, yl))
-        return y
+        link.fill(pre, x.shape[2], x_req, weight.requires_grad, bias.requires_grad, pair=(yh, yl) if yh is not None else None)
+        return y if y is not None else _poison(pre.device).expand(pre.shape)
 
     @staticmethod
     def _fuse_below(ctx, gh, gl, wth, wtl, geom, k, stride, pad, rows_in, skip_w):
@@ -361,7 +367,7 @@
                 dw = cg.conv_wgrad(gh, gl, xh, xl, geom, k, stride, pad).to(wdt)
             if want_db:
                 db = db32.to(bdt)
-        return (None, None, None, None, None, None, dw, db, dx, None, None, None, None, None)
+        return (None, None, None, None, None, None, dw, db, dx, None, None, None, None, None, None, None)
 
 
 _POISON = {}
@@ -372,6 +378,21 @@
     if t is None:
         t = _POISON[device] = torch.full((), float("nan"), dtype=torch.float32, device=device)
     return t
+
+
+def unstored(t):
+    return t.dim() > 0 and t.numel() > 1 and not any(t.stride())
+
+
+class _StoredMapFn(torch.autograd.Function):
+
+    @staticmethod
+    def forward(ctx, y, pre):
+        return bind.gelu_of_pre(pre)
+
+    @staticmethod
+    def backward(ctx, g):
+        return g, None
 
 
 def _l1_mode():
diff --git a/vm_asr_amd/mpd_link.py b/vm_asr_amd/mpd_link.py
--- a/vm_asr_amd/mpd_link.py
+++ b/vm_asr_amd/mpd_link.py
@@ -1,6 +1,14 @@
 from collections import namedtuple
 
 Plan = namedtuple("Plan", "want_f32 want_pair want_db loss")
+
+
+def forward_outputs(next_path):
+    from . import knobs
+    if not knobs.get("VMASR_MPD_LEAN_FWD"):
+        return True, True
+    pair_read = next_path == "mfma"
+    return not pair_read, pair_read
 
 
 class _Tap:
diff --git a/vm_asr_amd/mpd_ops.py b/vm_asr_amd/mpd_ops.py
--- a/vm_asr_amd/mpd_ops.py
+++ b/vm_asr_amd/mpd_ops.py
@@ -204,13 +204,20 @@
     return (ctypes.c_int64 * n)(*valid), (ctypes.c_float * n)(*scale)
 
 
-def masked_l1_fwd(real, gen, valid, scale, want_sgn):
+def masked_l1_fwd(real, gen, valid, scale, want_sgn, from_pre=False):
     n, rows_g, N = gen.shape
     v, sc = _valid_scale(valid, scale)
     partials = _new(gen, n * _lib.lib().vmasr_masked_l1_blocks(), torch.float64)
     sgn = _new(gen, (n, rows_g, N), torch.int8) if want_sgn else None
-    _call(_lib.lib().vmasr_masked_l1_fwd, real, gen, sgn, partials, v, sc, n, real.shape[1], rows_g, N)
+    fn = _lib.lib().vmasr_masked_l1_fwd_pre if from_pre else _lib.lib().vmasr_masked_l1_fwd
+    _call(fn, real, gen, sgn, partials, v, sc, n, real.shape[1], rows_g, N)
     return partials, sgn
+
+
+def gelu_of_pre(pre):
+    y = _new(pre, pre.shape)
+    _call(_lib.lib().vmasr_mpd_gelu_fwd, pre, y, pre.numel())
+    return y
 
 
 def masked_l1_bwd(sgn, g, valid, scale, add=None, tap=False):
```

After: 201.7 clips/s (median of 6 runs). About the same (+0.8%).
